# MadNLP/MadNLP.jl

Hardware: AMD Instinct MI355X
Metric: IP iterations/sec + ms per factorize!/solve!, condensed KKT n≈1e4 (higher is better)
Workload: dtype f64; 1 GPU; BASELINE config C3: case1354pegase-shaped sparse-condensed KKT, one instance; N=11192, m=16646, nnz(K)=68688; step = compress_J+compress_H+build_kkt+factorize (n_f=1) + inertia fetch + 2 solve_linear_system per instance; algorithm=BUNCHKAUFMAN (device: static-pivot LDL^T), outer_block=0, batch_per_gpu=1, batch_api=n/a (one instance), parallelism=1 GPU(s) x 1 independent instance(s)

## Files before the change

### madnlp.jl_amd/csrc/dag.hip

```cpp
#include <algorithm>
#include <atomic>
#include <cfloat>
#include <climits>
#include <vector>

#include "gemm_tile.h"
#include "ls.h"

namespace mnk {


struct DagInst {
    double* F;
    int64_t ld;
    double* V;
    const double* dinv;
    const double* dblk;
    const double* inv16;
    int* front;
    int* af;
    int* tprog;
    int* info;
    unsigned long long* vmax;
    double* zfill;
// ... 973 lines not shown
        mnk::PpDag dag{front, inst.af, ntile, 0, 0, -1, spin_limit, trace ? trace + (size_t)ls->dag_ntasks * 8 + (size_t)js_begin * 8 * 16 : nullptr,
                  mnk_ls_growth_word(ls), ls->dag_debug ? ls->dag_dbg.p : nullptr};
        int rc = mnk_launch_pchain(ls, sp, dag, js_begin, js_end, strips);
        if (rc) return rc;
        const int ph = (int)(counter - qctr), nq = ls->dag_nq[ph];
        MNK_REQUIRE(nq == 0 || (ntask >= mnk_ctx_bulk_wgs(ctx, chain_cus, 3) && bulk_xcds(ctx, chain_cus) == nq),
                    "task-DAG schedule: the bulk grid does not cover the XCDs the task list was dealt for");
        rc = mnk::launch_dag_bulk(su, ldl, inst, nullptr, ls->dag_tasks.p + 4 * (size_t)task0, ntask, ntile, counter, spin_limit,
                                  std::min(ntask, mnk_ctx_bulk_wgs(ctx, chain_cus, 3)), trace ? trace + 8 * (size_t)task0 : nullptr,
                                  trace ? trace + (size_t)ls->dag_ntasks * 8 + 4096 * 8 + (task0 > 0 ? 512 * 8 : 0) : nullptr,
                                  ls->dag_qoff.p + 16 * ph, ls->dag_qheads.p + ph * mnk::DAG_QHEAD_WORDS, nq);
        if (rc) return rc;
        if (js_begin == 0 && js_end > 0) {
            const int64_t safe = std::min<int64_t>(js_end, std::max<int64_t>(0, (ntile - ls->dag_band / 2 - 1) / 2)) & ~(int64_t)1;
            if (strips == (unsigned)ls->dag_band && safe > 0) {
                rc = mnk_ls_invert_blocks(ls, su, 0, safe);
                if (rc) return rc;
                ls->inv_done = safe;
            }
        }
        if (small) {
            rc = mnk_ls_invert_blocks(ls, s, 0, nsc);
            if (rc) return rc;
            ls->inv_done = nsc;
        } else if (js_begin == 0 && js_end == nsc && js2 == 0) {
            hipLaunchKernelGGL(mnk::dag_gate_kernel, dim3(1), dim3(1), 0, su, front + (nblk - 1), ntile, ls->info_dev.p, spin_limit);
            rc = mnk_ls_invert_blocks(ls, su, 0, nsc);
            if (rc) return rc;
            ls->inv_done = nsc;
        }
        if (!small) MNK_HIP(hipEventRecord(ctx->ev_a, sp));
        MNK_HIP(hipEventRecord(ctx->ev_b, su));
        if (!small) MNK_HIP(hipStreamWaitEvent(s, ctx->ev_a, 0));
        MNK_HIP(hipStreamWaitEvent(s, ctx->ev_b, 0));
        return 0;
    };
    if (js2 > 0) {
        int rc = phase(ctx->sp_dag, ctx->su_dag, ctx->dag_cus, 0, ls->dag_ntasks1, qctr, 0, std::min(js2, nsc),
                       (unsigned)std::min<int64_t>(ls->dag_band, Np / NBI));
        if (rc) return rc;
    }
    if (js2 < nsc) {
        const int64_t rows2 = Np - 256 * (int64_t)js2;
        MNK_REQUIRE(ctx->sp_dag2 != nullptr, "task-DAG schedule: the deep-band streams are missing");
        int rc = phase(ctx->sp_dag2, ctx->su_dag2, ctx->dag_cus2, ls->dag_ntasks1, ls->dag_ntasks - ls->dag_ntasks1,
                       qctr + 1, js2, nsc, (unsigned)(rows2 / NBI));
        if (rc) return rc;
    }
    return 0;
}

namespace {
struct BatchState {
    int depth = 0;
    bool active = false;
    std::vector<mnk_ls*> pend;
};
thread_local BatchState t_batch;

struct BatchBuffers {
    mnk::DevBuf<int> tasks;
    mnk::DevBuf<int> qctr;
    mnk::DevBuf<char> insts, pcsys, aux;
    char* stage = nullptr;
    size_t stage_bytes = 0;
    hipEvent_t stage_ev = nullptr;
    int ntile = 0, ninst = 0, period = 0, chunk = 0, taper0 = 0, band = 0, ntasks = 0;
    bool fill = false;
    hipEvent_t ev[4] = {nullptr, nullptr, nullptr, nullptr};
};
BatchBuffers g_batch[64];
}

bool mnk_batch_active() { return t_batch.active; }

bool mnk_batch_defer(mnk_ls* ls) {
    if (!t_batch.active) return false;
    const int nsc = (int)((ls->Np + 255) / 256);
    if (ls->algo_now != 5 || (ls->dag_js2 != nsc && ls->dag_js2 != 0) || ls->dag_trace_on || ls->ctx->partitioned) return false;
    if (mnk_ctx_ensure_batch_streams(ls->ctx) != 0) (void)hipGetLastError();
    if (!ls->ctx->sp_dagB) return false;
    if (!ls->ev_defer && hipEventCreateWithFlags(&ls->ev_defer, hipEventDisableTiming) != hipSuccess) { (void)hipGetLastError(); return false; }
    if (hipEventRecord(ls->ev_defer, ls->ctx->stream) != hipSuccess) { (void)hipGetLastError(); return false; }
    ls->deferred = true;
    t_batch.pend.push_back(ls);
    return true;
}

static void batch_mark_done(mnk_ls* ls) {
    ls->factorized = true;
    ls->info_valid = false;
    ls->bk_active = false;
    ls->deferred = false;
}

static int batch_run_group(std::vector<mnk_ls*>& g) {
    mnk_ls* l0 = g[0];
    mnk_ctx* c0 = l0->ctx;
    hipStream_t h = c0->stream;
    MNK_HIP(hipSetDevice(c0->device));
    const int64_t Np = l0->Np;
    const bool ldl = l0->algo == MNK_LDL;
    const int ntile = (int)(Np / 128), nsc = (int)((Np + 255) / 256), ninst = (int)g.size();
    const size_t nflags = (size_t)2 + (size_t)(Np / NBI) + 2 * (size_t)ntile * ntile;
    for (mnk_ls* ls : g)
        if (ls->ctx->stream != h) MNK_HIP(hipStreamWaitEvent(h, ls->ev_defer, 0));
    int rc = mnk_persist_begin(c0, h);
    if (rc) return rc;
    auto body = [&]() -> int {
        BatchBuffers& B = g_batch[c0->device & 63];
        const int period = std::max((ntile + 1) / 2, l0->batch_period > 0 ? l0->batch_period : 0);
        if (B.ntile != ntile || B.ninst != ninst || B.period != period || B.chunk != l0->dag_chunk || B.taper0 != l0->dag_taper0 ||
            B.band != l0->dag_band || B.fill != l0->dag_has_fill || !B.tasks.p) {
            std::vector<int> merged;
            mnk::dag_merge_tasks(l0->dag_host_tasks, l0->dag_host_ready, ninst, period, merged);
            if (B.tasks.alloc(merged.size() + 4)) return -2;
            { mnk::H2DGuard h2d; MNK_HIP(hipMemcpy(B.tasks.p, merged.data(), merged.size() * sizeof(int), hipMemcpyHostToDevice)); }
            if (!B.qctr.p && B.qctr.alloc(4)) return -2;
            if (B.insts.alloc(sizeof(mnk::DagInst) * (size_t)ninst)) return -2;
            for (hipEvent_t& e : B.ev)
                if (!e) MNK_HIP(hipEventCreateWithFlags(&e, hipEventDisableTiming));
            B.ntile = ntile; B.ninst = ninst; B.period = period; B.chunk = l0->dag_chunk; B.taper0 = l0->dag_taper0;
            B.band = l0->dag_band; B.fill = l0->dag_has_fill; B.ntasks = (int)(merged.size() / 4);
        }
        std::vector<mnk::DagInst> hin;
        mnk::DagInst* insts_dev = reinterpret_cast<mnk::DagInst*>(B.insts.p);
        for (mnk_ls* ls : g) {
            hin.push_back(dag_instance(ls));
            ls->dag_filled = hin.back().zfill != nullptr;
            ls->env_used = hin.back().env != nullptr;
            hipLaunchKernelGGL(mnk::dag_reset_kernel, dim3((unsigned)std::min<size_t>((nflags + 1023) / 1024, 64)), dim3(256), 0, h,
                               ls->dag_flags.p, (int64_t)nflags, ls->info_dev.p, hin.back(), insts_dev + (hin.size() - 1),
                               (const mnk::SmallSysRec*)nullptr, ls->env_word.p);
            ls->env_armed = false;
        }
        MNK_HIP(hipMemsetAsync(B.qctr.p, 0, 4 * sizeof(int), h));
        hipStream_t sp[2] = {c0->sp_dag, c0->sp_dagB}, su = c0->su_dagB;
        MNK_HIP(hipEventRecord(B.ev[0], h));
        MNK_HIP(hipStreamWaitEvent(sp[0], B.ev[0], 0));
        MNK_HIP(hipStreamWaitEvent(sp[1], B.ev[0], 0));
        MNK_HIP(hipStreamWaitEvent(su, B.ev[0], 0));
        const unsigned strips = (unsigned)std::min<int64_t>(l0->dag_band, Np / NBI);
        const int bulk_wgs = mnk_ctx_bulk_wgs(c0, 2 * c0->dag_cus, 3);
        auto launch_chain = [&](int i) -> int {
            mnk_ls* ls = g[i];
            mnk::PpDag dag{hin[i].front, hin[i].af, ntile, 0, 0, -1, mnk_ls_dag_spin_limit(ls), nullptr, mnk_ls_growth_word(ls)};
            return mnk_launch_pchain(ls, sp[i & 1], dag, 0, nsc, strips);
        };
        auto launch_tail = [&](int i) -> int {
            mnk_ls* ls = g[i];
            int r = mnk_ls_invert_blocks(ls, sp[i & 1], 0, nsc);
            if (r) return r;
            ls->inv_done = nsc;
            return mnk_ls_launch_finish_info(ls, sp[i & 1]);
        };
        for (int i = 0; i < std::min(2, ninst); ++i) {
            int r = launch_chain(i);
            if (r) return r;
        }
        int r = mnk::launch_dag_bulk(su, ldl, hin[0], insts_dev, B.tasks.p, B.ntasks, ntile, B.qctr.p,
                                     mnk_ls_dag_spin_limit(l0), std::min(B.ntasks, bulk_wgs), nullptr, nullptr);
        if (r) return r;
        for (int i = 0; i < ninst; ++i) {
            r = launch_tail(i);
            if (r) return r;
            if (i + 2 < ninst) {
                r = launch_chain(i + 2);
                if (r) return r;
            }
        }
        MNK_HIP(hipEventRecord(B.ev[1], sp[0]));
        MNK_HIP(hipEventRecord(B.ev[2], sp[1]));
        MNK_HIP(hipEventRecord(B.ev[3], su));
        for (int e = 1; e < 4; ++e) MNK_HIP(hipStreamWaitEvent(h, B.ev[e], 0));
        return 0;
    };
    rc = body();
    rc = mnk_persist_end(c0, h, rc);
    if (rc) return rc;
    MNK_HIP(hipEventRecord(l0->ev_defer, h));
    for (mnk_ls* ls : g) {
        if (ls->ctx->stream != h) MNK_HIP(hipStreamWaitEvent(ls->ctx->stream, l0->ev_defer, 0));
        batch_mark_done(ls);
        int r = mnk_ls_prefill_spare(ls);
        if (r) return r;
    }
    return 0;
}

static int batch_run_group_small(std::vector<mnk_ls*>& g) {
    mnk_ls* l0 = g[0];
    mnk_ctx* c0 = l0->ctx;
    hipStream_t h = c0->stream;
    MNK_HIP(hipSetDevice(c0->device));
    const int64_t Np = l0->Np;
    const bool ldl = l0->algo == MNK_LDL;
    const int ntile = (int)(Np / 128), nsc = (int)((Np + 255) / 256), strips = (int)(Np / NBI);
    const size_t nflags = (size_t)2 + (size_t)(Np / NBI) + 2 * (size_t)ntile * ntile;
    const int ntasks1 = l0->dag_ntasks;
    const int bulk_min = ntasks1 > 0 ? std::max(32, c0->num_cu / 4) : 0;
    auto chain_cus_for = [&](int k) { return std::min(c0->num_cu, (k * strips + 63) / 64 * 64); };
    int kmax = std::min(32, (c0->num_cu - bulk_min) / strips);
    while (kmax > 1 && chain_cus_for(kmax) > c0->num_cu - bulk_min) --kmax;
    if (kmax < 2) {
        for (mnk_ls* ls : g) {
            ls->deferred = false;
            int rc = mnk_ls_run_factorization_now(ls);
            if (rc) return rc;
        }
        return 0;
    }
    for (mnk_ls* ls : g)
        if (ls->ctx->stream != h) MNK_HIP(hipStreamWaitEvent(h, ls->ev_defer, 0));
    BatchBuffers& B = g_batch[c0->device & 63];
    for (size_t r0 = 0; r0 < g.size(); r0 += (size_t)kmax) {
        const int k = (int)std::min<size_t>(kmax, g.size() - r0);
        hipStream_t sp = nullptr, su = nullptr;
        int rc = mnk_masked_stream_pair(c0, chain_cus_for(k), &sp, &su);
        if (rc) return rc;
        if (ntasks1 > 0 && su == nullptr) { set_error("factorize batch: no CUs left for the bulk kernel"); return -1; }
        rc = mnk_persist_begin(c0, h);
        if (rc) return rc;
        auto body = [&]() -> int {
            if (ntasks1 > 0 && (B.ntile != ntile || B.ninst != k || B.period != 0 || B.chunk != l0->dag_chunk || B.taper0 != l0->dag_taper0 ||
                                B.band != l0->dag_band || B.fill != l0->dag_has_fill || !B.tasks.p)) {
                std::vector<int> merged;
                mnk::dag_merge_tasks(l0->dag_host_tasks, l0->dag_host_ready, k, 0, merged);
                if (B.tasks.alloc(merged.size() + 4)) return -2;
                { mnk::H2DGuard h2d; MNK_HIP(hipMemcpy(B.tasks.p, merged.data(), merged.size() * sizeof(int), hipMemcpyHostToDevice)); }
                B.ntile = ntile; B.ninst = k; B.period = 0; B.chunk = l0->dag_chunk; B.taper0 = l0->dag_taper0;
                B.band = l0->dag_band; B.fill = l0->dag_has_fill; B.ntasks = (int)(merged.size() / 4);
            }
            if (!B.qctr.p && B.qctr.alloc(4)) return -2;
            if (B.insts.n < sizeof(mnk::DagInst) * (size_t)k && B.insts.alloc(sizeof(mnk::DagInst) * (size_t)std::max(k, 32))) return -2;
            if (B.pcsys.n < mnk_pchain_sys_bytes() * (size_t)k && B.pcsys.alloc(mnk_pchain_sys_bytes() * (size_t)std::max(k, 32))) return -2;
            for (hipEvent_t& e : B.ev)
                if (!e) MNK_HIP(hipEventCreateWithFlags(&e, hipEventDisableTiming));
            std::vector<mnk::DagInst> hin;
            std::vector<int*> fronts;
            std::vector<const int*> afs;
            mnk::DagInst* insts_dev = reinterpret_cast<mnk::DagInst*>(B.insts.p);
            const size_t pc_bytes = mnk_pchain_sys_bytes();
            const size_t need = (size_t)k * (sizeof(mnk::DagInst) + pc_bytes + sizeof(mnk::SmallSysRec));
            if (B.aux.n < sizeof(mnk::SmallSysRec) * (size_t)k && B.aux.alloc(sizeof(mnk::SmallSysRec) * (size_t)std::max(k, 32))) return -2;
            if (B.stage_ev == nullptr) MNK_HIP(hipEventCreateWithFlags(&B.stage_ev, hipEventDisableTiming));
            else MNK_HIP(hipEventSynchronize(B.stage_ev));
            if (B.stage_bytes < need) {
                mnk::LaunchLock lock;
                if (B.stage) { mnk::quiesce_persistent(); (void)hipHostFree(B.stage); B.stage = nullptr; }
                const size_t cap = (size_t)std::max(k, 32) * (sizeof(mnk::DagInst) + pc_bytes + sizeof(mnk::SmallSysRec));
                MNK_HIP(hipHostMalloc((void**)&B.stage, cap, hipHostMallocDefault));
                B.stage_bytes = cap;
            }
            mnk::DagInst* st_inst = reinterpret_cast<mnk::DagInst*>(B.stage);
            char* st_pc = B.stage + (size_t)k * sizeof(mnk::DagInst);
            mnk::SmallSysRec* st_aux = reinterpret_cast<mnk::SmallSysRec*>(st_pc + (size_t)k * pc_bytes);
            const bool batch_aux = l0->linv_mfma && !l0->solve512;
            for (int i = 0; i < k; ++i) {
                mnk_ls* ls = g[r0 + i];
                hin.push_back(dag_instance(ls));
                ls->dag_filled = hin.back().zfill != nullptr;
                hin.back().env = nullptr;
                hin.back().envgate = nullptr;
                ls->env_used = false;
                fronts.push_back(hin.back().front);
                afs.push_back(hin.back().af);
                st_inst[i] = hin.back();
                mnk_pchain_fill_sys(ls, st_pc + (size_t)i * pc_bytes, hin.back().front, hin.back().af);
                mnk_ls_fill_small_rec(ls, st_aux + i);
            }
            MNK_HIP(hipMemcpyAsync(B.insts.p, st_inst, (size_t)k * sizeof(mnk::DagInst), hipMemcpyHostToDevice, h));
            MNK_HIP(hipMemcpyAsync(B.pcsys.p, st_pc, (size_t)k * pc_bytes, hipMemcpyHostToDevice, h));
            MNK_HIP(hipMemcpyAsync(B.aux.p, st_aux, (size_t)k * sizeof(mnk::SmallSysRec), hipMemcpyHostToDevice, h));
            MNK_HIP(hipEventRecord(B.stage_ev, h));
            const mnk::SmallSysRec* aux_dev = reinterpret_cast<const mnk::SmallSysRec*>(B.aux.p);
            hipLaunchKernelGGL(mnk::dag_reset_kernel, dim3((unsigned)std::min<size_t>((nflags + 1023) / 1024, 64), (unsigned)k), dim3(256), 0, h,
                               (int*)nullptr, (int64_t)0, (int*)nullptr, hin[0], (mnk::DagInst*)nullptr, aux_dev);
            MNK_HIP(hipMemsetAsync(B.qctr.p, 0, 4 * sizeof(int), h));
            MNK_HIP(hipEventRecord(B.ev[0], h));
            MNK_HIP(hipStreamWaitEvent(sp, B.ev[0], 0));
            if (su != nullptr) MNK_HIP(hipStreamWaitEvent(su, B.ev[0], 0));
            int r = mnk_launch_pchain_multi(g.data() + r0, k, sp, nullptr, B.pcsys.p, fronts.data(), afs.data());
            if (r) return r;
            if (ntasks1 > 0) {
                const int bulk_wgs = mnk_ctx_bulk_wgs(c0, chain_cus_for(k), 3);
                r = mnk::launch_dag_bulk(su, ldl, hin[0], insts_dev, B.tasks.p, B.ntasks, ntile, B.qctr.p, mnk_ls_dag_spin_limit(l0),
                                         std::min(B.ntasks, bulk_wgs), nullptr, nullptr);
                if (r) return r;
                MNK_HIP(hipEventRecord(B.ev[2], su));
                MNK_HIP(hipStreamWaitEvent(h, B.ev[2], 0));
            }
            MNK_HIP(hipEventRecord(B.ev[1], sp));
            MNK_HIP(hipStreamWaitEvent(h, B.ev[1], 0));
            if (su != nullptr) MNK_HIP(hipStreamWaitEvent(su, B.ev[1], 0));
            if (su != nullptr) MNK_HIP(hipStreamWaitEvent(sp, B.ev[2], 0));
            if (batch_aux) {
                r = mnk_ls_invert_blocks_batch(h, ldl, aux_dev, k, Np);
                if (r) return r;
                r = mnk_ls_finish_info_batch(h, aux_dev, k, ldl ? (l0->N >= 4096 ? 1024 : 256) : 64);
                if (r) return r;
                for (int i = 0; i < k; ++i) {
                    mnk_ls* ls = g[r0 + i];
                    ls->inv_done = nsc;
                    if (!ls->ev_info) MNK_HIP(hipEventCreateWithFlags(&ls->ev_info, hipEventDisableTiming));
                    MNK_HIP(hipEventRecord(ls->ev_info, h));
                    ls->ev_info_recorded = true;
                }
                return 0;
            }
            hipStream_t inv_s[3] = {h, sp, su != nullptr ? su : sp};
            for (int i = 0; i < k; ++i) {
                mnk_ls* ls = g[r0 + i];
                hipStream_t si = inv_s[i % 3];
                r = mnk_ls_invert_blocks(ls, si, 0, nsc);
                if (r) return r;
                ls->inv_done = nsc;
                r = mnk_ls_launch_finish_info(ls, si);
                if (r) return r;
            }
            MNK_HIP(hipEventRecord(B.ev[1], sp));
            MNK_HIP(hipStreamWaitEvent(h, B.ev[1], 0));
            if (su != nullptr) {
                MNK_HIP(hipEventRecord(B.ev[2], su));
                MNK_HIP(hipStreamWaitEvent(h, B.ev[2], 0));
            }
            return 0;
        };
        rc = body();
        rc = mnk_persist_end(c0, h, rc);
        if (rc) return rc;
    }
    MNK_HIP(hipEventRecord(l0->ev_defer, h));
    for (mnk_ls* ls : g) {
        if (ls->ctx->stream != h) MNK_HIP(hipStreamWaitEvent(ls->ctx->stream, l0->ev_defer, 0));
        batch_mark_done(ls);
        int r = mnk_ls_prefill_spare(ls);
        if (r) return r;
    }
    return 0;
}

static int batch_flush() {
    std::vector<mnk_ls*> pend;
    pend.swap(t_batch.pend);
    int rc_all = 0;
    while (!pend.empty()) {
        mnk_ls* l0 = pend.front();
        std::vector<mnk_ls*> g, rest;
        for (mnk_ls* ls : pend) {
            const bool same = ls->ctx->device == l0->ctx->device && ls->Np == l0->Np && ls->algo == l0->algo && ls->dag_js2 == l0->dag_js2 && ls->dag_chunk == l0->dag_chunk &&
                              ls->dag_taper0 == l0->dag_taper0 && ls->dag_band == l0->dag_band && ls->dag_has_fill == l0->dag_has_fill;
            (same && std::find(g.begin(), g.end(), ls) == g.end() ? g : rest).push_back(ls);
        }
        pend.swap(rest);
        int rc;
        if (g.size() >= 2) {
            rc = l0->dag_js2 == 0 ? batch_run_group_small(g) : batch_run_group(g);
            if (rc)
                for (mnk_ls* ls : g) { ls->deferred = false; ls->factorized = false; ls->info_valid = false; }
        } else {
            g[0]->deferred = false;
            if (g[0]->Np < g[0]->dag_min_rows) g[0]->algo_now = 4;
            rc = mnk_ls_run_factorization_now(g[0]);
            if (rc) { g[0]->factorized = false; g[0]->info_valid = false; }
        }
        if (rc && !rc_all) rc_all = rc;
    }
    return rc_all;
}

int mnk_ls_sync_deferred(mnk_ls* ls) {
    {
        int rc_s = mnk_solve_sync_deferred(ls);
        if (rc_s) return rc_s;
    }
    return mnk_ls_sync_deferred_fact(ls);
}

bool mnk_ls_pending_elsewhere(const mnk_ls* ls) {
    return ls->deferred && std::find(t_batch.pend.begin(), t_batch.pend.end(), ls) == t_batch.pend.end();
}

int mnk_ls_sync_deferred_fact(mnk_ls* ls) {
    if (!ls->deferred) return 0;
    if (std::find(t_batch.pend.begin(), t_batch.pend.end(), ls) == t_batch.pend.end()) {
        set_error("a factorize! call of this solver is pending in a batch that another thread opened (mnk_factorize_batch_end must come first)");
        return -1;
    }
    return batch_flush();
}

extern "C" int mnk_factorize_batch_begin(void) {
    ++t_batch.depth;
    t_batch.active = true;
    return 0;
}

extern "C" int mnk_factorize_batch_end(void) {
    if (t_batch.depth <= 0) { set_error("mnk_factorize_batch_end: no batch is open on this thread"); return -1; }
    if (--t_batch.depth > 0) return 0;
    t_batch.active = false;
    return batch_flush();
}

extern "C" int mnk_debug_dag_tasks(int ntile, int chunk, int band_tiles, int js2, int taper0, int* out, int cap, int* first_phase) {
    if (ntile <= 0 || chunk <= 0 || band_tiles <= 0 || taper0 <= 0) return -1;
    std::vector<int> h;
    const int n1 = mnk::dag_build_tasks(ntile, chunk, band_tiles, js2, h, taper0, nullptr);
    const int n = (int)(h.size() / 4);
    if (first_phase != nullptr) *first_phase = n1;
    if (out != nullptr)
        for (int i = 0; i < std::min(n, cap) * 4; ++i) out[i] = h[i];
    return n;
}

extern "C" int mnk_debug_dag_merged_tasks(int ntile, int chunk, int band_tiles, int js2, int taper0, int fill, int ninst, int period,
                                          int* out, int cap) {
    if (ntile <= 0 || chunk <= 0 || band_tiles <= 0 || taper0 <= 0 || ninst <= 0 || period < 0) return -1;
    std::vector<int> h, ready, merged;
    int n1 = mnk::dag_build_tasks(ntile, chunk, band_tiles, js2, h, taper0, &ready);
    if (fill) n1 = mnk::dag_add_fill_tasks(ntile, h, ready, n1);
    mnk::dag_merge_tasks(h, ready, ninst, period, merged);
    const int n = (int)(merged.size() / 4);
    if (out != nullptr)
        for (int i = 0; i < std::min(n, cap) * 4; ++i) out[i] = merged[i];
    return n;
}

extern "C" int mnk_debug_dag_deal(int ntile, int chunk, int band_tiles, int js2, int taper0, int fill, int ninst, int period, int nq,
                                  int gang, int* tasks_out, int* order, int cap, int* off, int* first_phase) {
    if (ntile <= 0 || chunk <= 0 || band_tiles <= 0 || taper0 <= 0 || ninst <= 0 || period < 0 || nq <= 0 || nq > 64 || gang == 0) return -1;
    std::vector<int> h, ready;
    int n1 = mnk::dag_build_tasks(ntile, chunk, band_tiles, js2, h, taper0, &ready);
    if (fill) n1 = mnk::dag_add_fill_tasks(ntile, h, ready, n1);
    if (ninst > 1) {
        std::vector<int> merged, mready, pos(ninst, 0);
        mnk::dag_merge_tasks(h, ready, ninst, period, merged);
        for (size_t t = 0; t < merged.size() / 4; ++t) { const int i = merged[4 * t + 1] >> 16; mready.push_back(i * period + ready[pos[i]++]); }
        h.swap(merged);
        ready.swap(mready);
        n1 = (int)ready.size();
    }
    const int n = (int)ready.size();
    if (first_phase != nullptr) *first_phase = n1;
    const int part[3] = {0, n1, n};
    int written = 0;
    for (int ph = 0; ph < 2; ++ph) {
        std::vector<int> ord, o;
        mnk::dag_deal_tasks(h, ready, part[ph], part[ph + 1], nq, gang, ord, o);
        for (int x = 0; x <= nq; ++x)
            if (off != nullptr) off[ph * (nq + 1) + x] = part[ph] + o[x];
        for (int v : ord) {
            if (order != nullptr && written < cap) order[written] = v;
            ++written;
        }
    }
    if (tasks_out != nullptr)
        for (int i = 0; i < std::min(n, cap) * 4; ++i) tasks_out[i] = h[i];
    return n;
}
```

### madnlp.jl_amd/csrc/factor.hip

```cpp
#include <atomic>
#include <type_traits>
#include <atomic>
#include <cfloat>
#include <chrono>
#include <cmath>
#include <cstdlib>

#include "ls.h"
#include "leaf64.h"

namespace mnk {

template <bool LDL, int NS>
__device__ __forceinline__ void trsm64_mfma_body(double* __restrict__ F, int64_t ld, int64_t j0, int64_t Np,
                                                 const double* __restrict__ Dblk, const double* __restrict__ inv16,
                                                 const double* __restrict__ dinv, double* __restrict__ W, int64_t ldw,
                                                 int64_t wcol, const int* __restrict__ info,
                                                 unsigned long long* __restrict__ vmax) {
    if (*info != 0) return;
    const int lane = threadIdx.x & 63, wave = threadIdx.x >> 6;
    const int l15 = lane & 15, l4 = lane >> 4;
    const int64_t r0 = j0 + 64 + ((int64_t)blockIdx.x * 4 + wave) * (16 * NS);
    if (r0 >= Np) return;
    double Ln[6][4];
// ... 894 lines not shown
        hipLaunchKernelGGL(linv64_kernel<true>, dim3((unsigned)(b1 - b0)), dim3(256), 0, s, ls->fact.p, ls->ld, ls->dblk.p,
                           ls->linv.p, ls->info_dev.p, (int)b0);
    else
        hipLaunchKernelGGL(linv64_kernel<false>, dim3((unsigned)(b1 - b0)), dim3(256), 0, s, ls->fact.p, ls->ld, ls->dblk.p,
                           ls->linv.p, ls->info_dev.p, (int)b0);
    MNK_HIP(hipGetLastError());
    return mnk_ls_build_inverses(ls, s, sc0, sc1);
}

int mnk_launch_pchain(mnk_ls* ls, hipStream_t sp, const mnk::PpDag& dag, int js_begin, int js_end, unsigned strips) {
    {
        static std::atomic<uint64_t> attr_devs{0};
        int dev = 0;
        MNK_HIP(hipGetDevice(&dev));
        if (!(attr_devs.load(std::memory_order_relaxed) >> (dev & 63) & 1)) {
            MNK_HIP(hipFuncSetAttribute((const void*)pchain_kernel<true>, hipFuncAttributeMaxDynamicSharedMemorySize, PC_LDS_BYTES));
            MNK_HIP(hipFuncSetAttribute((const void*)pchain_kernel<false>, hipFuncAttributeMaxDynamicSharedMemorySize, PC_LDS_BYTES));
            attr_devs.fetch_or(1ull << (dev & 63), std::memory_order_relaxed);
        }
    }
    const bool ldl = ls->algo == MNK_LDL;
    const int epoch16 = ls->epoch * 16;
    double* V = ldl ? ls->vfull.p : nullptr;
    if (ldl)
        hipLaunchKernelGGL(pchain_kernel<true>, dim3(strips), dim3(256), PC_LDS_BYTES, sp, ls->fact.p, ls->ld, ls->Np, ls->dblk.p,
                           ls->inv16.p, ls->dvec.p, ls->dinv.p, V, ls->info_dev.p, ls->pivot_tol, ls->flag_p.p, epoch16,
                           ls->debug_pp_missing, dag, js_begin, js_end);
    else
        hipLaunchKernelGGL(pchain_kernel<false>, dim3(strips), dim3(256), PC_LDS_BYTES, sp, ls->fact.p, ls->ld, ls->Np, ls->dblk.p,
                           ls->inv16.p, ls->dvec.p, ls->dinv.p, V, ls->info_dev.p, ls->pivot_tol, ls->flag_p.p, epoch16,
                           ls->debug_pp_missing, dag, js_begin, js_end);
    MNK_HIP(hipGetLastError());
    return 0;
}

static int run_factorization_body(mnk_ls* ls);

size_t mnk_pchain_sys_bytes() { return sizeof(mnk::PcSys); }
void mnk_pchain_fill_sys(mnk_ls* ls, void* rec_host, int* front, const int* af) {
    const bool ldl = ls->algo == MNK_LDL;
    *static_cast<mnk::PcSys*>(rec_host) = mnk::PcSys{ls->fact.p, ls->ld, ls->Np, ls->dblk.p, ls->inv16.p, ls->dvec.p, ls->dinv.p,
                                                       ldl ? ls->vfull.p : nullptr, ls->info_dev.p, ls->pivot_tol, ls->flag_p.p,
                                                       ls->epoch * 16, front, af, (int)(ls->Np / 128), mnk_ls_dag_spin_limit(ls),
                                                       mnk_ls_growth_word(ls)};
}

int mnk_launch_pchain_multi(mnk_ls* const* v, int n, hipStream_t sp, hipStream_t fill_stream, void* table, int* const* front,
                            const int* const* af) {
    {
        static std::atomic<uint64_t> attr_devs{0};
        int dev = 0;
        MNK_HIP(hipGetDevice(&dev));
        if (!(attr_devs.load(std::memory_order_relaxed) >> (dev & 63) & 1)) {
            MNK_HIP(hipFuncSetAttribute((const void*)pchain_multi_kernel<true>, hipFuncAttributeMaxDynamicSharedMemorySize, PC_LDS_BYTES));
            MNK_HIP(hipFuncSetAttribute((const void*)pchain_multi_kernel<false>, hipFuncAttributeMaxDynamicSharedMemorySize, PC_LDS_BYTES));
            attr_devs.fetch_or(1ull << (dev & 63), std::memory_order_relaxed);
        }
    }
    mnk::PcSys* dst = static_cast<mnk::PcSys*>(table);
    const bool ldl = v[0]->algo == MNK_LDL;
    const int strips = (int)(v[0]->Np / NBI);
    for (int i = 0; i < n && fill_stream != nullptr; ++i) {
        mnk_ls* ls = v[i];
        mnk::PcSys rec{ls->fact.p, ls->ld, ls->Np, ls->dblk.p, ls->inv16.p, ls->dvec.p, ls->dinv.p, ldl ? ls->vfull.p : nullptr,
                       ls->info_dev.p, ls->pivot_tol, ls->flag_p.p, ls->epoch * 16, front[i], af[i], (int)(ls->Np / 128),
                       mnk_ls_dag_spin_limit(ls), mnk_ls_growth_word(ls)};
        hipLaunchKernelGGL(pc_set_sys_kernel, dim3(1), dim3(1), 0, fill_stream, rec, dst + i);
    }
    MNK_HIP(hipGetLastError());
    if (ldl)
        hipLaunchKernelGGL(pchain_multi_kernel<true>, dim3((unsigned)(n * strips)), dim3(256), PC_LDS_BYTES, sp, dst, strips);
    else
        hipLaunchKernelGGL(pchain_multi_kernel<false>, dim3((unsigned)(n * strips)), dim3(256), PC_LDS_BYTES, sp, dst, strips);
    MNK_HIP(hipGetLastError());
    return 0;
}

int mnk_ls_run_factorization(mnk_ls* ls) {
    if (ls->algo == MNK_QR) return mnk_qr_factor(ls);
    if (ls->algo == MNK_LU) return mnk_lu_factor(ls);
    if (ls->algo == MNK_EVD) return mnk_evd_factor(ls);
    mnk_ctx* ctx = ls->ctx;
    hipStream_t s = ctx->stream;
    const int64_t Np = ls->Np;
    if (ls->panel_algo >= 4 && !ls->flag_p.p) {
        if (ls->flag_p.alloc(Np / NBI + 1)) return -2;
        MNK_HIP(hipMemsetAsync(ls->flag_p.p, 0, (Np / NBI + 1) * sizeof(int), s));
    }
    ++ls->epoch;
    ls->inv_done = 0;
    ls->factor_invalid = false;
    ls->t_fact_launch_ms = mnk_host_ms();
    {
        const int want = (ls->early_reject && ls->accept_only_pd && ls->algo == MNK_LDL && ls->src_persistent) ? 1 : 0;
        if (want != ls->reject_on_device) {
            MNK_HIP(hipMemsetAsync(ls->info_dev.p + 2, want, sizeof(int), s));
            ls->reject_on_device = want;
        }
    }
    ls->algo_now = ls->panel_algo;
    ls->env_used = false;
    const int64_t min_rows = mnk_batch_active() ? std::min<int64_t>(ls->dag_min_rows, 256) : ls->dag_min_rows;
    if (ls->algo_now == 5 && (ctx->dag_cus < ls->dag_band || !ls->lookahead || Np < min_rows || Np > ls->dag_max_rows)) ls->algo_now = 4;
    if (ls->algo_now == 5 && ctx->sp_dag == nullptr && mnk_ctx_ensure_dag(ctx) != 0) { (void)hipGetLastError(); ls->algo_now = 4; }
    if (ls->algo_now == 5 && ctx->sp_dag == nullptr) ls->algo_now = 4;
    ++ls->fact_count;
    if (ls->pp_blocked && ls->fact_count >= ls->pp_retry_at) ls->pp_blocked = false;
    if (ls->algo_now >= 4 && ls->pp_blocked) ls->algo_now = 1;
    if (ls->algo_now == 5 && mnk_ls_dag_prepare(ls) != 0) ls->algo_now = 4;
    if (ls->algo_now == 5 && ls->dag_js2 < (Np + 255) / 256) {
        if (mnk_ctx_ensure_dag2(ctx) != 0) (void)hipGetLastError();
        if (ctx->sp_dag2 == nullptr) ls->algo_now = 4;
    }
    if (ls->algo_now == 5 && mnk_batch_defer(ls)) return 0;
    return mnk_ls_run_factorization_now(ls);
}

int mnk_ls_run_factorization_now(mnk_ls* ls) {
    mnk_ctx* ctx = ls->ctx;
    hipStream_t s = ctx->stream;
    const bool persistent = ls->algo_now >= 4;
    if (persistent) {
        int rc0 = mnk_persist_begin(ctx, s);
        if (rc0) return rc0;
    }
    const int rc_run = run_factorization_body(ls);
    return persistent ? mnk_persist_end(ctx, s, rc_run) : rc_run;
}

static int run_factorization_body(mnk_ls* ls) {
    mnk_ctx* ctx = ls->ctx;
    hipStream_t s = ctx->stream;
    const int64_t Np = ls->Np, ld = ls->ld;
    const bool ldl = ls->algo == MNK_LDL;
    double* F = ls->fact.p;
    const int64_t NBO = mnk_ls_effective_nbo(ls);
    if (ls->algo_now != 5) MNK_HIP(hipMemsetAsync(ls->info_dev.p, 0, 2 * sizeof(int), s));
    std::vector<int64_t> bnd{0};
    for (int64_t pos = 0; pos < Np;) {
        const bool tail = ls->lookahead && NBO < Np && ls->tail_rows > 0 && Np - pos <= ls->tail_rows && ls->tail_nbo < NBO;
        pos = std::min<int64_t>(pos + (tail ? ls->tail_nbo : NBO), Np);
        bnd.push_back(pos);
    }
    const int64_t npanel = (int64_t)bnd.size() - 1;
    const bool la = ls->lookahead && npanel > 1;

    if (ls->algo_now == 5) {
        int rc = mnk_ls_run_factorization_dag(ls);
        if (rc) return rc;
    } else if (!la) {
        for (int64_t ko = 0; ko < Np; ko += NBO) {
            const int64_t kend = std::min<int64_t>(ko + NBO, Np);
            int rc = factor_outer_panel(ls, s, ko, kend, ls->wbuf[0].p);
            if (rc) return rc;
            const int64_t Mt = Np - kend;
            if (Mt > 0) {
                const double* Wsrc = ldl ? ls->wbuf[0].p + kend : F + kend + ko * ld;
                rc = launch_gemm_nt(s, 2, Mt, Mt, kend - ko, Wsrc, ldl ? ls->ldw : ld, F + kend + ko * ld, ld,
                                    F + kend + kend * ld, ld, nullptr, nullptr, 0, ls->info_dev.p);
                if (rc) return rc;
            }
        }
    } else {
        { int rc_s = mnk_ctx_ensure_panel_streams(ctx); if (rc_s) return rc_s; }
        hipStream_t sp = ctx->sp, su = ctx->su;
        if ((int64_t)ctx->ev_panel.size() < npanel + 1) {
            const size_t old = ctx->ev_panel.size();
            ctx->ev_panel.resize(npanel + 1);
            ctx->ev_next.resize(npanel + 1);
            ctx->ev_next2.resize(npanel + 1);
            ctx->ev_bdone.resize(npanel + 1);
            for (size_t e = old; e < ctx->ev_panel.size(); ++e) {
                MNK_HIP(hipEventCreateWithFlags(&ctx->ev_panel[e], hipEventDisableTiming));
                MNK_HIP(hipEventCreateWithFlags(&ctx->ev_next[e], hipEventDisableTiming));
                MNK_HIP(hipEventCreateWithFlags(&ctx->ev_next2[e], hipEventDisableTiming));
                MNK_HIP(hipEventCreateWithFlags(&ctx->ev_bdone[e], hipEventDisableTiming));
            }
        }
        const int pcus = ctx->panel_cus;
        const int ucus = pcus > 0 ? ctx->num_cu - pcus : ctx->num_cu;
        const bool share = ls->share != 0;
        if (share) {
            if (ls->tile_ctr.n < 8 * ((size_t)npanel + 1)) {
                int rc0 = ls->tile_ctr.alloc(8 * ((size_t)npanel + 1));
                if (rc0) return rc0;
            }
            MNK_HIP(hipMemsetAsync(ls->tile_ctr.p, 0, 8 * ((size_t)npanel + 1) * sizeof(int), s));
        }
        int rc = 0;
        if (ls->panel0_whole) rc = factor_outer_panel(ls, s, 0, bnd[1], ls->wbuf[0].p);
        if (rc) return rc;
        MNK_HIP(hipEventRecord(ctx->ev_a, s));
        MNK_HIP(hipStreamWaitEvent(sp, ctx->ev_a, 0));
        MNK_HIP(hipStreamWaitEvent(su, ctx->ev_a, 0));
        if (!ls->panel0_whole) rc = factor_outer_panel(ls, sp, 0, bnd[1], ls->wbuf[0].p);
        if (rc) return rc;
        MNK_HIP(hipEventRecord(ctx->ev_panel[0], sp));
        for (int64_t k = 0; k + 1 < npanel; ++k) {
            const int64_t ko = bnd[k], kend = bnd[k + 1];
            const int64_t Mt = Np - kend;
            if (Mt <= 0) break;
            const int64_t nnext = bnd[k + 2] - kend;
            double* wk = ls->wbuf[k & 1].p;
            const double* Wsrc = ldl ? wk + kend : F + kend + ko * ld;
            const int64_t ldws = ldl ? ls->ldw : ld;
            const int64_t Kw = kend - ko;
            MNK_HIP(hipStreamWaitEvent(su, ctx->ev_panel[k], 0));
            auto update_a = [&](hipStream_t st, int64_t c0, int64_t c1) -> int {
                const int64_t Mp = Mt - c0, Nn = c1 - c0;
                double* Cp = F + (kend + c0) + (kend + c0) * ld;
                if (gemm_nt_lower_tiles(Mp, Nn) < ls->small_tiles)
                    return launch_gemm_nt_lower_small(st, Mp, Nn, Kw, Wsrc + c0, ldws, F + kend + c0 + ko * ld, ld, Cp,
                                                      ld, ls->info_dev.p);
                return launch_gemm_nt(st, 2, Mp, Nn, Kw, Wsrc + c0, ldws, F + kend + c0 + ko * ld, ld, Cp, ld, nullptr,
                                      nullptr, 0, ls->info_dev.p);
            };
            const bool fuse_a = ls->algo_now == 4 && ls->pp_fuse_rows > 0 && Mt <= ls->pp_fuse_rows && Kw <= 512;
            const bool own_first = !fuse_a && ls->split_a == 2 && nnext > NBI;
            const int64_t n1 = own_first ? std::min<int64_t>(ls->own_cols, nnext - NBI) : std::min<int64_t>(256, nnext);
            const bool split_a = (ls->split_a || fuse_a) && nnext > n1;
            if (fuse_a) {
                if (k > 0) MNK_HIP(hipStreamWaitEvent(sp, ctx->ev_bdone[k - 1], 0));
                if (split_a) {
                    rc = update_a(su, n1, nnext);
                    if (rc) return rc;
                    MNK_HIP(hipEventRecord(ctx->ev_next2[k], su));
                }
            } else if (own_first) {
                if (k > 0) MNK_HIP(hipStreamWaitEvent(sp, ctx->ev_bdone[k - 1], 0));
                rc = update_a(sp, 0, n1);
                if (rc) return rc;
                rc = update_a(su, n1, nnext);
                if (rc) return rc;
                MNK_HIP(hipEventRecord(ctx->ev_next2[k], su));
            } else {
                rc = update_a(su, 0, split_a ? n1 : nnext);
                if (rc) return rc;
                MNK_HIP(hipEventRecord(ctx->ev_next[k], su));
                if (split_a) {
                    rc = update_a(su, n1, nnext);
                    if (rc) return rc;
                    MNK_HIP(hipEventRecord(ctx->ev_next2[k], su));
                }
            }
            const int64_t Mb = Mt - nnext;
            const int64_t Nb = Mb;
            bool shared_b = false;
            if (Mb > 0 && Nb > 0) {
                const int ntiles = gemm_nt_lower_tiles(Mb, Nb);
                const double t_upd = ntiles * (68.0 * (double)Kw / 512.0) / ucus;
                const double t_pan = 55.0 * (double)nnext / 64.0 * (pcus > 0 ? 64.0 / pcus : 1.0);
                shared_b = share && pcus > 0 && (t_upd > t_pan || ls->share == 2);
                if (shared_b)
                    rc = launch_gemm_nt_queue(su, Mb, Nb, Kw, Wsrc + nnext, ldws, F + kend + nnext + ko * ld, ld,
                                              F + (kend + nnext) + (kend + nnext) * ld, ld, ls->tile_ctr.p + 8 * k,
                                              ucus, ls->info_dev.p);
                else
                    rc = launch_gemm_nt(su, 2, Mb, Nb, Kw, Wsrc + nnext, ldws, F + kend + nnext + ko * ld, ld,
                                        F + (kend + nnext) + (kend + nnext) * ld, ld, nullptr, nullptr, 0,
                                        ls->info_dev.p);
                if (rc) return rc;
            }
            MNK_HIP(hipEventRecord(ctx->ev_bdone[k], su));
            if (!own_first && !fuse_a) MNK_HIP(hipStreamWaitEvent(sp, ctx->ev_next[k], 0));
            rc = factor_outer_panel(ls, sp, kend, kend + nnext, ls->wbuf[(k + 1) & 1].p,
                                    split_a ? ctx->ev_next2[k] : nullptr, own_first ? n1 : 256,
                                    fuse_a ? (ldl ? wk : F + ko * ld) : nullptr, ldws, fuse_a ? Kw : 0);
            if (rc) return rc;
            if (shared_b) {
                rc = launch_gemm_nt_queue(sp, Mb, Nb, Kw, Wsrc + nnext, ldws, F + kend + nnext + ko * ld, ld,
                                          F + (kend + nnext) + (kend + nnext) * ld, ld, ls->tile_ctr.p + 8 * k,
                                          pcus, ls->info_dev.p);
                if (rc) return rc;
            }
            MNK_HIP(hipEventRecord(ctx->ev_panel[k + 1], sp));
        }
        MNK_HIP(hipEventRecord(ctx->ev_a, sp));
        MNK_HIP(hipEventRecord(ctx->ev_b, su));
        MNK_HIP(hipStreamWaitEvent(s, ctx->ev_a, 0));
        MNK_HIP(hipStreamWaitEvent(s, ctx->ev_b, 0));
    }
    {
        int rc = mnk_ls_invert_blocks(ls, s, ls->inv_done, (Np + 255) / 256);
        if (rc) return rc;
    }
    ls->factorized = true;
    ls->info_valid = false;
    ls->bk_active = false;
    {
        int rc = mnk_ls_launch_finish_info(ls, s);
        if (rc) return rc;
    }
    return mnk_ls_prefill_spare(ls);
}

void mnk_ls_fill_small_rec(mnk_ls* ls, mnk::SmallSysRec* rec) {
    const bool lmode = ls->algo == MNK_LDL;
    const int64_t ntile = ls->Np / 128;
    rec->flags = ls->dag_flags.p;
    rec->nflags = 2 + ls->Np / NBI + 2 * ntile * ntile;
    rec->info = ls->info_dev.p;
    rec->F = ls->fact.p; rec->ld = ls->ld; rec->dblk = ls->dblk.p; rec->linv = ls->linv.p;
    rec->linv256 = ls->linv256.p; rec->linv256t = ls->linv256t.p; rec->Np = ls->Np;
    rec->dvec = ls->dvec.p; rec->ninertia = lmode ? ls->N : 0; rec->pin_dev = ls->pin_dev;
    rec->amax = mnk_ls_growth_word(ls) != nullptr ? ls->amax_dev.p : nullptr;
}

int mnk_ls_invert_blocks_batch(hipStream_t s, bool ldl, const mnk::SmallSysRec* recs_dev, int n, int64_t Np) {
    const unsigned nb = (unsigned)(Np / NBI);
    if (ldl) hipLaunchKernelGGL(linv64_kernel<true>, dim3(nb, 1, (unsigned)n), dim3(256), 0, s, (double*)nullptr, (int64_t)0, (const double*)nullptr,
                                (double*)nullptr, (const int*)nullptr, 0, recs_dev);
    else hipLaunchKernelGGL(linv64_kernel<false>, dim3(nb, 1, (unsigned)n), dim3(256), 0, s, (double*)nullptr, (int64_t)0, (const double*)nullptr,
                            (double*)nullptr, (const int*)nullptr, 0, recs_dev);
    MNK_HIP(hipGetLastError());
    return mnk_ls_build_inverses_batch(s, recs_dev, n, Np);
}

int mnk_ls_finish_info_batch(hipStream_t s, const mnk::SmallSysRec* recs_dev, int n, int threads) {
    hipLaunchKernelGGL(finish_info_kernel, dim3((unsigned)n), dim3(threads), 0, s, (const double*)nullptr, (int64_t)0, (const int*)nullptr,
                       (unsigned long long*)nullptr, (const unsigned long long*)nullptr, recs_dev);
    MNK_HIP(hipGetLastError());
    return 0;
}

int mnk_ls_launch_finish_info(mnk_ls* ls, hipStream_t s) {
    const bool lmode = ls->algo == MNK_LDL;
    const int threads = lmode ? (ls->N >= 4096 ? 1024 : 256) : 64;
    hipLaunchKernelGGL(finish_info_kernel, dim3(1), dim3(threads), 0, s, ls->dvec.p, lmode ? ls->N : (int64_t)0, ls->info_dev.p, ls->pin_dev,
                       mnk_ls_growth_word(ls) != nullptr ? ls->amax_dev.p : (const unsigned long long*)nullptr);
    MNK_HIP(hipGetLastError());
    if (!ls->ev_info) MNK_HIP(hipEventCreateWithFlags(&ls->ev_info, hipEventDisableTiming));
    MNK_HIP(hipEventRecord(ls->ev_info, s));
    ls->ev_info_recorded = true;
    return 0;
}

int mnk_ls_right_trsm_rows(mnk_ls* ls, hipStream_t s, int64_t j0, double* Xrows, double* Vrows, int64_t ldr, int64_t nrows) {
    MNK_REQUIRE(ls->factorized && !ls->bk_active && nrows % 16 == 0 && j0 % NBI == 0 && j0 < ls->Np,
                "mnk_ls_right_trsm_rows: needs a static-pivot factor, 16-row multiples and a block-aligned column");
    double* Fp = Xrows - (j0 + NBI);
    double* Wp = Vrows ? Vrows - (j0 + NBI) : nullptr;
    const unsigned grid = (unsigned)((nrows / 16 + 3) / 4);
    const double* dblk = ls->dblk.p + (j0 / NBI) * 4096;
    const double* inv16 = ls->inv16.p + (j0 / NBI) * 1024;
    if (ls->algo == MNK_LDL)
        hipLaunchKernelGGL((trsm64_mfma_kernel<true, 1>), dim3(grid), dim3(256), 0, s, Fp, ldr, j0, j0 + NBI + nrows, dblk,
                           inv16, ls->dinv.p, Wp, ldr, (int64_t)j0, ls->info_dev.p);
    else
        hipLaunchKernelGGL((trsm64_mfma_kernel<false, 1>), dim3(grid), dim3(256), 0, s, Fp, ldr, j0, j0 + NBI + nrows, dblk,
                           inv16, ls->dinv.p, (double*)nullptr, (int64_t)0, (int64_t)0, ls->info_dev.p);
    MNK_HIP(hipGetLastError());
    return 0;
}

int mnk_launch_trsm64_batch(hipStream_t s, bool ldl, const mnk::TrsmBatchRec* recs_dev, int nbatch, int64_t j0, int64_t nrows,
                            int64_t ldr) {
    if (nbatch <= 0 || nrows <= 0) return 0;
    MNK_REQUIRE(nrows % 16 == 0 && j0 % NBI == 0, "mnk_launch_trsm64_batch: 16-row multiples and a block-aligned column");
    const dim3 grid((unsigned)((nrows / 16 + 3) / 4), (unsigned)nbatch);
    if (ldl) hipLaunchKernelGGL(trsm64_mfma_batch_kernel<true>, grid, dim3(256), 0, s, recs_dev, ldr, j0, nrows);
    else hipLaunchKernelGGL(trsm64_mfma_batch_kernel<false>, grid, dim3(256), 0, s, recs_dev, ldr, j0, nrows);
    MNK_HIP(hipGetLastError());
    return 0;
}

static int bk_fallback(mnk_ls* ls) {
    hipStream_t s = ls->ctx->stream;
    int rc = ls->retransfer();
    if (rc) return rc;
    rc = mnk_ls_run_bunchkaufman(ls);
    if (rc) return rc;
    rc = mnk_ls_invert_blocks(ls, s, 0, (ls->Np + 255) / 256);
    if (rc) return rc;
    ++ls->bk_count;
    return mnk_ls_prefill_spare(ls);
}

int mnk_ls_fetch_info(mnk_ls* ls) {
    { int rc_d = mnk_ls_sync_deferred(ls); if (rc_d) return rc_d; }
    if (ls->info_valid) return 0;
    if (ls->algo == MNK_QR) {
        MNK_HIP(mnk::stream_wait(ls->ctx->stream));
        ls->info = 0;
        ls->info_valid = true;
        return 0;
    }
    if (ls->algo == MNK_LU) return mnk_lu_fetch_info(ls);
    if (ls->algo == MNK_EVD) return mnk_evd_fetch_info(ls);
    hipStream_t s = ls->ctx->stream;
    if (ls->bk_active) {
        MNK_HIP(hipMemsetAsync(ls->inertia_dev.p, 0, 3 * sizeof(unsigned long long), s));
        int rc = mnk_ls_bk_inertia(ls, ls->inertia_dev.p);
        if (rc) return rc;
        hipLaunchKernelGGL(publish_info_kernel, dim3(1), dim3(64), 0, s, ls->inertia_dev.p, ls->info_dev.p, ls->pin_dev);
        MNK_HIP(hipGetLastError());
        MNK_HIP(mnk::stream_wait(s));
        volatile unsigned long long* pw = ls->pin;
        unsigned long long h[3] = {pw[0], pw[1], pw[2]};
        int hinfo = (int)(long long)pw[3];
        ls->info = hinfo;
        ls->nneg = h[1] > 0 ? -1 : (int64_t)h[0];
        ls->nzero = hinfo > 0 ? 1 : 0;
        ls->npos = ls->N - ls->nneg - ls->nzero;
        ls->info_valid = true;
        return 0;
    }
    const bool guard = ls->algo == MNK_LDL && ls->bk_requested && ls->bk_fallback && ls->retransfer && ls->amax_dev.p != nullptr;
    if (ls->ev_info_recorded) MNK_HIP(hipEventSynchronize(ls->ev_info));
    else MNK_HIP(mnk::stream_wait(s));
    volatile unsigned long long* pw = ls->pin;
    unsigned long long h[3] = {pw[0], pw[1], pw[2]};
    int hinfo = (int)(long long)pw[3];
    if (guard) {
        double am, dm;
        const unsigned long long wa = pw[4], wd = pw[5];
        memcpy(&am, &wa, sizeof am);
        memcpy(&dm, &wd, sizeof dm);
        ls->last_growth = am > 0.0 ? dm / am : (dm > 0.0 ? HUGE_VAL : 0.0);
        ls->last_sign_changes = (int64_t)pw[6];
    }
    if (hinfo == -7) ls->last_timeout_site = (int)(long long)pw[7];
    if (hinfo == -7 && ls->dag_debug && ls->dag_flags.p && ls->dag_dbg.p) {
        MNK_HIP(mnk::stream_wait(s));
        const int64_t ntile = ls->Np / 128;
        ls->dbg_flags.resize((size_t)(2 + ls->Np / NBI + 2 * ntile * ntile));
        ls->dbg_chain.resize(ls->dag_dbg.n);
        MNK_HIP(mnk::d2h_copy(ls->dbg_flags.data(), ls->dag_flags.p, ls->dbg_flags.size() * sizeof(int), s));
        MNK_HIP(mnk::d2h_copy(ls->dbg_chain.data(), ls->dag_dbg.p, ls->dbg_chain.size() * sizeof(int), s));
    }
    if (hinfo != 0 && ls->spare_by_dag) {
        ls->spare_zeroed = false;
        ls->spare_by_dag = false;
    }
    if (hinfo == -7 && ls->algo_now >= 4 && ls->retransfer) {
        ls->pp_blocked = true;
        ls->pp_retry_at = ls->fact_count + ls->pp_backoff + 1;
        ls->pp_backoff *= 4;
        ++ls->pp_fallbacks;
        {
            const double lost = std::max(0.0, mnk_host_ms() - ls->t_fact_launch_ms);
            ls->stall_ms_total += lost;
            mnk_add_process_stall_ms(lost);
        }
        int rc = ls->retransfer();
        if (rc) return rc;
        rc = mnk_ls_run_factorization(ls);
        if (rc) return rc;
        return mnk_ls_fetch_info(ls);
    }
    ls->factor_invalid = false;
    if (hinfo == -9) {
        ls->info = 1;
        ls->npos = (int64_t)h[0];
        ls->nzero = (int64_t)h[1];
        ls->nneg = ls->N - ls->npos - ls->nzero;
        ls->factor_invalid = true;
        ++ls->early_rejects;
        ls->early_reject_col = (int64_t)(long long)pw[7];
        ls->info_valid = true;
        ls->probe_last_rejected = true;
        if (2 * ls->early_reject_col < ls->N) { ls->probe_hint_col = ls->early_reject_col; ls->probe_since_hint = 0; }
        else if (ls->probe_since_hint < (1 << 20)) ++ls->probe_since_hint;
        return 0;
    }
    if (hinfo < 0) {
        set_error("factorize!: a device-side hand-off timed out (info = %d) and the matrix cannot be transferred again; the "
                  "factor is invalid -- set panel_algo = 1", hinfo);
        return -4;
    }
    ls->info = hinfo;
    if (ls->algo == MNK_LDL) {
        ls->npos = (int64_t)h[0];
        ls->nzero = (int64_t)h[1];
        ls->nneg = (int64_t)h[2];
        if (ls->nzero > 0 && ls->info == 0) ls->info = 1;
        const double gtol = ls->last_sign_changes <= 1 ? ls->bk_growth_tol_qd : ls->bk_growth_tol;
        const bool verdict_final = ls->accept_only_pd && (ls->nzero > 0 || ls->nneg > 0);
        if (!verdict_final && (ls->nzero > 0 || (guard && !(ls->last_growth <= gtol))) && ls->bk_requested && ls->bk_fallback && ls->retransfer) {
            int rc = bk_fallback(ls);
            if (rc) return rc;
            return mnk_ls_fetch_info(ls);
        }
    } else {
        if (hinfo == 0) { ls->npos = ls->N; ls->nzero = 0; ls->nneg = 0; }
        else { ls->npos = 0; ls->nzero = ls->N; ls->nneg = 0; }
    }
    ls->probe_last_rejected = false;
    if (ls->probe_since_hint < (1 << 20)) ++ls->probe_since_hint;
    ls->info_valid = true;
    return 0;
}
```

### madnlp.jl_amd/csrc/ls.h

```cpp
#pragma once
#include <algorithm>
#include <functional>
#include <memory>
#include <string>
#include <vector>

#include "common.h"

struct mnk_sc {
    mnk_ctx* ctx = nullptr;
    int64_t n = 0, m = 0, nnzj = 0, nnzh = 0;
    int64_t nnz_jt = 0, nnz_hess = 0, nnz_aug = 0, len_jptr = 0;
    std::vector<int32_t> jt_colptr, jt_rowval, h_colptr, h_rowval, aug_colptr, aug_rowval;
    std::vector<int32_t> tile_env;
    mnk::DevBuf<int32_t> d_tile_env;
    std::vector<int64_t> jt_map, h_map;
    std::vector<int32_t> d_dst, d_src, hp_dst, hp_src, j_dst, j_c, j_k, j_l;
    mnk::DevBuf<int32_t> jt_seg_ptr, jt_seg_src, h_seg_ptr, h_seg_src;
    mnk::DevBuf<int32_t> aug_hptr, aug_hsrc;
    mnk::DevBuf<int32_t> aug_dsrc;
    mnk::DevBuf<int32_t> aug_jptr, aug_jc, aug_jk, aug_jl;
    mnk::DevBuf<int32_t> aug_row, aug_col;
    mnk::DevBuf<int32_t> d_jt_colptr, d_jt_rowval, d_jt_colidx, d_h_colptr, d_h_rowval, d_h_colidx;
    mnk::DevBuf<double> jac_coo, hess_coo, jt_nz, h_nz, aug_nz, diag_buffer, pr_diag, du_diag;
    void* extra = nullptr;
    std::shared_ptr<int> alive = std::make_shared<int>(0);
};

inline std::vector<int32_t> mnk_tile_envelope(int64_t n, const int32_t* row, const int32_t* col, int64_t nnz) {
    std::vector<int32_t> fnz(n);
    for (int64_t i = 0; i < n; ++i) fnz[i] = (int32_t)i;
    for (int64_t k = 0; k < nnz; ++k)
        if (row[k] >= 0 && row[k] < n && col[k] < fnz[row[k]]) fnz[row[k]] = col[k];
    const int64_t ntile = (n + 127) / 128;
    std::vector<int32_t> env(ntile);
    for (int64_t I = 0; I < ntile; ++I) {
        int32_t f = (int32_t)(128 * I);
        for (int64_t i = 128 * I; i < std::min<int64_t>(n, 128 * I + 128); ++i) f = std::min(f, fnz[i]);
        env[I] = f / 128;
    }
    return env;
}

struct mnk_dc {
    mnk_ctx* ctx = nullptr;
    int condensed = 1;
    bool mirror_pending = false;
    int64_t n = 0, m = 0, ns = 0, n_eq = 0, order = 0;
    std::vector<int64_t> ind_ineq, ind_eq;
    mnk::DevBuf<int64_t> d_ind_ineq, d_ind_eq;
    mnk::DevBuf<double> hess, jac, aug, pr_diag, du_diag, diag_buffer;
    mnk::DevBuf<double> jis;
    int64_t ld_jis = 0, kpad = 0, npad = 0;
    void* extra = nullptr;
    void* qn = nullptr;
    std::shared_ptr<int> alive = std::make_shared<int>(0);
};
void mnk_dc_qn_release(mnk_dc* dc);

constexpr int EVD_BLOCK = 32;

struct mnk_ls {
    mnk_ctx* ctx = nullptr;
    int64_t N = 0, Np = 0, ld = 0, ldw = 0, nbo = 512;
    bool nbo_auto = true;
    int algo = MNK_LDL;
    double pivot_tol = 0.0;
    int lookahead = 1;
    int share = 1;
    int small_tiles = 400;
    int split_a = 2;
    int64_t single_rows = 2560;
    int64_t tail_rows = 4096;
    int64_t tail_nbo = 256;
    int small_tiles_mid = 1000;
    mnk::DevBuf<int> tile_ctr;
    mnk::DevBuf<double> fact, wbuf[2], linv, dblk, inv16, linv256, linv256t, dvec, dinv, xwork;
    mnk::DevBuf<double> fact_spare;
    hipEvent_t ev_spare = nullptr, ev_free = nullptr;
    bool spare_zeroed = false, spare_pending = false;
    int prefill = 1;
    int64_t prefill_max_rows = 24576;
    int epoch = 0;
    mnk::DevBuf<int> flag_p;
    int panel0_whole = 1;
    int algo_now = 1;
    bool pp_blocked = false;
    int64_t fact_count = 0, pp_retry_at = 0, pp_backoff = 16;
    int pp_fallbacks = 0;
    int last_timeout_site = 0;
    double stall_ms_total = 0.0;
    double t_fact_launch_ms = 0.0;
    int64_t pp_fuse_rows = 4096;
    int64_t own_cols = 128;
    mnk::DevBuf<int> dag_tasks;
    int dag_ntasks = 0, dag_ntasks1 = 0, dag_js2 = 0;
    std::vector<int> dag_host_tasks, dag_host_ready;
    int dag_fill = 1;
    bool dag_has_fill = false;
    bool dag_filled = false;
    int batch_period = 0;
    hipEvent_t ev_info = nullptr;
    bool ev_info_recorded = false;
    hipEvent_t ev_defer = nullptr;
    bool deferred = false;
    int dag_xcd_queues = 1;
    int dag_gang = 4;
    int dag_nq[2] = {0, 0};
    mnk::DevBuf<int> dag_qoff;
    mnk::DevBuf<int> dag_qheads;
    mnk::DevBuf<int> dag_flags;
    mnk::DevBuf<double> vfull;
    mnk::DevBuf<unsigned long long> dag_trace;
    bool dag_trace_on = false;
    int64_t inv_done = 0;
    int dag_band = 16;
    int dag_taper0 = 2;
    long dag_spin_limit = 0;
    int dag_chunk = 64;
    int64_t dag_min_rows = 1280;
    int64_t dag_deep_rows = 5376;
    int envelope = 1;
    const int32_t* env_dev = nullptr;
    std::vector<int32_t> env_host;
    mnk::DevBuf<int32_t> env_own;
    mnk::DevBuf<int> env_word;
    bool env_used = false;
    bool env_armed = false;
    int64_t dag_max_rows = 30720;
    int panel_algo = 5;
    int persistent_solve = 1;
    int solve512 = 0;
    int64_t solve512_min_rows = 4096;
    int dag_chain_inline = 1;
    std::vector<std::string> env_keys;
    int dag_js2_override = -1;
    int linv_mfma = 1;
    mnk::DevBuf<double> linv512, linv512t, linv512tmp;
    int pub_next = 0;
    bool pub_clean[2] = {false, false};
    int* solve_abort = nullptr;
    long ps_spin_limit = 6000000;
    int debug_pp_missing = -1;
    int debug_ps_missing = -1;
    mnk::DevBuf<unsigned long long> solve_trace;
    mnk::DevBuf<int> info_dev;
    mnk::DevBuf<unsigned long long> inertia_dev;
    unsigned long long* pin = nullptr;
    unsigned long long* pin_dev = nullptr;
    bool bk_requested = false;
    int bk_fallback = 1;
    int early_reject = 0;
    int reject_on_device = -1;
    bool src_persistent = false;
    bool factor_invalid = false;
    int64_t early_rejects = 0, early_reject_col = -1, early_reject_redone = 0;
    int probe = 1;
    mnk_ls* probe_ls = nullptr;
    int64_t probe_order = 0;
    int64_t probe_hint_col = -1;
    int probe_since_hint = 1 << 20;
    bool probe_last_rejected = false;
    int64_t probe_hits = 0, probe_misses = 0;
    int accept_only_pd = 0;
    double bk_growth_tol = 64.0, bk_growth_tol_qd = 1e8;
    double last_growth = 0.0;
    int64_t last_sign_changes = 0;
    mnk::DevBuf<unsigned long long> amax_dev;
    bool bk_active = false;
    int bk_count = 0;
    std::function<int()> retransfer;
    mnk::DevBuf<int> bk_perm, bk_ptype;
    mnk::DevBuf<double> bk_doff, bk_dcoup, bk_work;
    mnk::DevBuf<char> bk_state;
    mnk::DevBuf<double> bk_wv, bk_tmp;
    mnk::DevBuf<unsigned long long> bk_msg;
    mnk::DevBuf<int> bk_aux;
    int bk_panel_wgs = 0;
    int bk_max_wgs = 0;
    long bk_spin_limit = 1L << 21;
    int debug_bk_missing = -1;
    bool bk_multi_last = false, bk_mw_blocked = false;
    int bk_mw_fallbacks = 0;
    bool factorized = false, info_valid = false;
    int dag_debug = 0;
    mnk::DevBuf<int> dag_dbg;
    std::vector<int> dbg_flags, dbg_chain;
    bool spare_by_dag = false;
    int info = 0;
    int64_t npos = 0, nzero = 0, nneg = 0;
    mnk::DevBuf<double> qr_v, qr_t, qr_w, qr_p;
    mnk::DevBuf<double> lu_ut, lu_p;
    mnk::DevBuf<int> lu_cand, lu_ipiv, lu_perm, lu_info;
    mnk::DevBuf<double> evd_a, evd_v, evd_rt, evd_colsum, evd_lam, evd_part;
    mnk::DevBuf<int> evd_ident, evd_rank;
    int evd_sweep_cap = 60;
    int evd_sweeps = 0;
};

int64_t mnk_ls_effective_nbo(const mnk_ls* ls);
int mnk_qr_alloc(mnk_ls* ls);
int mnk_qr_factor(mnk_ls* ls);
int mnk_qr_solve(mnk_ls* ls, double* x, int64_t nrhs, int64_t ldx, int loc);
int mnk_launch_tril_to_full(hipStream_t s, double* F, int64_t ld, int64_t N, int64_t Np);
int mnk_launch_upper_bsolve(hipStream_t s, const double* F, int64_t ld, int64_t Np, double* y, double* x);
int mnk_lu_alloc(mnk_ls* ls);
int mnk_lu_factor(mnk_ls* ls);
int mnk_lu_fetch_info(mnk_ls* ls);
int mnk_lu_solve(mnk_ls* ls, double* x, int64_t nrhs, int64_t ldx, int loc);
int mnk_evd_alloc(mnk_ls* ls);
int mnk_evd_factor(mnk_ls* ls);
int mnk_evd_fetch_info(mnk_ls* ls);
int mnk_evd_solve(mnk_ls* ls, double* x, int64_t nrhs, int64_t ldx, int loc);
int mnk_ls_run_factorization(mnk_ls* ls);
int mnk_ls_run_factorization_now(mnk_ls* ls);
int mnk_ls_launch_finish_info(mnk_ls* ls, hipStream_t s);
bool mnk_solve_defer(mnk_ls* ls, double* xuser);
int mnk_solve_sync_deferred(mnk_ls* ls);
int mnk_solve_batch_flush_pending(void);
int mnk_ls_factorize_dense_dev_async(mnk_ls* ls, const double* Adev, int64_t lda);
double mnk_host_ms();
void mnk_add_process_stall_ms(double ms);
double mnk_process_stall_ms();
bool mnk_ls_pending_elsewhere(const mnk_ls* ls);
bool mnk_batch_active();
size_t mnk_pchain_sys_bytes();
int mnk_launch_pchain_multi(mnk_ls* const* v, int n, hipStream_t sp, hipStream_t fill_stream, void* table, int* const* front,
                            const int* const* af);
bool mnk_batch_defer(mnk_ls* ls);
int mnk_ls_sync_deferred(mnk_ls* ls);
int mnk_ls_sync_deferred_fact(mnk_ls* ls);
int mnk_ls_prefill_spare(mnk_ls* ls);
int mnk_ls_fetch_info(mnk_ls* ls);
int mnk_ls_run_factorization_dag(mnk_ls* ls);
int mnk_ls_dag_prepare(mnk_ls* ls);
int mnk_launch_pchain(mnk_ls* ls, hipStream_t sp, const mnk::PpDag& dag, int js_begin, int js_end, unsigned strips);
unsigned long long* mnk_ls_growth_word(mnk_ls* ls);
int mnk_ls_run_solve(mnk_ls* ls, double* xdev , double* xuser = nullptr );
int mnk_ls_build_inverses(mnk_ls* ls, hipStream_t s, int64_t sc0, int64_t sc1);
int mnk_ls_invert_blocks(mnk_ls* ls, hipStream_t s, int64_t sc0, int64_t sc1);
int mnk_ls_right_trsm_rows(mnk_ls* ls, hipStream_t s, int64_t j0, double* Xrows, double* Vrows, int64_t ldr, int64_t nrows);
int mnk_ls_run_bunchkaufman(mnk_ls* ls);
long mnk_ls_dag_spin_limit(const mnk_ls* ls);
namespace mnk {
struct SmallSysRec {
    int* flags; int64_t nflags; int* info;
    double* F; int64_t ld; const double* dblk; double* linv; double* linv256; double* linv256t; int64_t Np;
    const double* dvec; int64_t ninertia; unsigned long long* pin_dev; const unsigned long long* amax;
};
}
int mnk_ls_invert_blocks_batch(hipStream_t s, bool ldl, const mnk::SmallSysRec* recs_dev, int n, int64_t Np);
int mnk_ls_build_inverses_batch(hipStream_t s, const mnk::SmallSysRec* recs_dev, int n, int64_t Np);
int mnk_ls_finish_info_batch(hipStream_t s, const mnk::SmallSysRec* recs_dev, int n, int threads);
void mnk_ls_fill_small_rec(mnk_ls* ls, mnk::SmallSysRec* rec);
void mnk_pchain_fill_sys(mnk_ls* ls, void* rec_host, int* front, const int* af);
int mnk_launch_trsm64_batch(hipStream_t s, bool ldl, const mnk::TrsmBatchRec* recs_dev, int nbatch, int64_t j0, int64_t nrows,
                            int64_t ldr);
int mnk_ls_bk_permute(mnk_ls* ls, double* x, double* tmp, bool forward);
int mnk_ls_bk_dsolve(mnk_ls* ls, double* y);
int mnk_ls_bk_inertia(mnk_ls* ls, unsigned long long* out_dev);
bool mnk_ls_take_solve_abort(mnk_ls* ls);
```

### madnlp.jl_amd/csrc/ls.hip

```cpp
#include <cstdarg>
#include <cstdlib>
#include <atomic>
#include <map>
#include <mutex>

#include <cfloat>
#include "ls.h"

namespace mnk {

static thread_local std::string g_err;
void set_error(const char* fmt, ...) {
    char buf[1024];
    va_list ap;
    va_start(ap, fmt);
    vsnprintf(buf, sizeof(buf), fmt, ap);
    va_end(ap);
    g_err = buf;
}

__global__ __launch_bounds__(256) void fill_lower_kernel(double* __restrict__ F, int64_t ld, int64_t N, int64_t Np) {
    const int64_t col = blockIdx.x;
    const int64_t first = (col / PAD) * PAD;
    const int64_t r = first + ((int64_t)blockIdx.y * 256 + threadIdx.x) * 2;
// ... 431 lines not shown
        }
        if (!part) g_ctx_list[device & 63].push_back(c);
        c->sp_dag = d.sp; c->su_dag = d.su; c->dag_cus = d.cus;
        c->dag_cus2 = d.cus > 0 ? (getenv("MNK_DAG_CUS2") ? atoi(getenv("MNK_DAG_CUS2")) : 96) : 0;
        if (c->dag_cus2 <= 0 || c->dag_cus2 >= c->num_cu) c->dag_cus2 = 0;
        c->shared_dag_streams = !part;
        if (part) {
            if (c->dag_cus2 > 0 && !make_pair(c->dag_cus2, c->sp_dag2, c->su_dag2)) c->dag_cus2 = 0;
        }
    }
    MNK_HIP(hipEventCreateWithFlags(&c->ev_a, hipEventDisableTiming));
    MNK_HIP(hipEventCreateWithFlags(&c->ev_b, hipEventDisableTiming));
    if (mnk_solve_warmup(c->stream) != 0) (void)hipGetLastError();
    g_live_ctx[device & 63].fetch_add(1, std::memory_order_relaxed);
    *out = c;
    return 0;
}

int mnk_ctx_create(int device, void* stream, mnk_ctx** out) { return ctx_create_common(device, stream, 0, 0, out); }

}
int mnk_masked_stream_pair(mnk_ctx* ctx, int chain_cus, hipStream_t* sp, hipStream_t* su) {
    mnk::LaunchLock lock;
    MNK_REQUIRE(!ctx->partitioned && chain_cus > 0 && chain_cus <= ctx->total_cu, "mnk_masked_stream_pair: bad size");
    MaskedPair& p = g_pair_cache[{ctx->device, chain_cus}];
    if (p.sp == nullptr) {
        std::vector<int> bits;
        for (int b = 0; b < ctx->total_cu; ++b) bits.push_back(b);
        if (!make_masked_stream(ctx->total_cu, bits.data(), chain_cus, p.sp)) { set_error("mnk_masked_stream_pair: CU-masked streams are not available"); return -2; }
        if (chain_cus < ctx->total_cu && !make_masked_stream(ctx->total_cu, bits.data() + chain_cus, ctx->total_cu - chain_cus, p.su)) {
            (void)hipStreamDestroy(p.sp);
            p.sp = nullptr;
            set_error("mnk_masked_stream_pair: CU-masked streams are not available");
            return -2;
        }
        if (p.su != nullptr) {
            hipStream_t w[1] = {p.su};
            if (mnk_dag_warmup(w, 1, 3 * ctx->num_cu) != 0) (void)hipGetLastError();
        }
    }
    *sp = p.sp;
    *su = p.su;
    return 0;
}
extern "C" {

int mnk_ctx_destroy(mnk_ctx* c) {
    if (!c) return 0;
    {
        std::lock_guard<std::mutex> lock(g_ctx_mutex);
        if (c->children > 0) {
            c->released = true;
            return 0;
        }
    }
    ctx_free(c);
    return 0;
}


int mnk_ctx_synchronize(mnk_ctx* c) {
    MNK_REQUIRE(c != nullptr, "ctx is NULL");
    MNK_HIP(mnk::stream_wait(c->stream));
    return 0;
}

void* mnk_ctx_stream(mnk_ctx* c) { return c ? (void*)c->stream : nullptr; }

int mnk_ls_create(mnk_ctx* ctx, int64_t N, int algo, mnk_ls** out) {
    MNK_REQUIRE(ctx && out, "mnk_ls_create: NULL argument");
    mnk::LaunchLock lock;
    MNK_REQUIRE(N > 0, "mnk_ls_create: N must be positive");
    const bool bk_requested = algo == MNK_BUNCHKAUFMAN;
    if (bk_requested) algo = MNK_LDL;
    MNK_REQUIRE(algo == MNK_CHOLESKY || algo == MNK_LDL || algo == MNK_QR || algo == MNK_LU || algo == MNK_EVD,
                "mnk_ls_create: unknown algorithm (BUNCHKAUFMAN, LU, QR, CHOLESKY, LDL and EVD are implemented on device)");
    MNK_HIP(hipSetDevice(ctx->device));
    mnk_ls* ls = new mnk_ls();
    ls->ctx = ctx;
    ls->N = N;
    ls->algo = algo;
    ls->bk_requested = bk_requested;
    {
        auto from_env = [&](const std::string& key, double v) {
            if (mnk_ls_set_option(ls, key.c_str(), v) == 0) ls->env_keys.push_back(key);
            else fprintf(stderr, "madnlp_hip: ignoring environment override '%s': %s\n", key.c_str(), mnk_last_error_string());
        };
        if (const char* e = getenv("MNK_PANEL_ALGO")) from_env("panel_algo", atof(e));
        if (const char* e = getenv("MNK_PERSISTENT_SOLVE")) from_env("persistent_solve", atof(e));
        if (const char* e = getenv("MNK_OPTIONS")) {
            std::string all(e);
            size_t pos = 0;
            while (pos < all.size()) {
                size_t end = all.find(',', pos);
                if (end == std::string::npos) end = all.size();
                const std::string item = all.substr(pos, end - pos);
                const size_t eq = item.find('=');
                if (eq != std::string::npos && eq > 0) from_env(item.substr(0, eq), atof(item.c_str() + eq + 1));
                pos = end + 1;
            }
        }
    }
    ls->Np = round_up(N, PAD);
    ls->ld = ls->Np;
    ls->ldw = ls->Np;
    int rc = 0;
    rc |= ls->fact.alloc((size_t)ls->ld * ls->Np + SLACK);
    rc |= ls->linv.alloc((size_t)(ls->Np / NBI) * NBI * NBI);
    rc |= ls->dblk.alloc((size_t)(ls->Np / NBI) * NBI * NBI);
    rc |= ls->inv16.alloc((size_t)(ls->Np / NBI) * 1024);
    rc |= ls->linv256.alloc((size_t)((ls->Np + 255) / 256) * 65536);
    rc |= ls->linv256t.alloc((size_t)((ls->Np + 255) / 256) * 65536);
    rc |= ls->dvec.alloc(ls->Np);
    rc |= ls->dinv.alloc(ls->Np);
    rc |= ls->xwork.alloc(10 * ls->Np);
    if (hipHostMalloc((void**)&ls->solve_abort, sizeof(int), hipHostMallocDefault) != hipSuccess) {
        (void)hipGetLastError();
        ls->solve_abort = nullptr;
        rc |= -2;
    } else {
        *ls->solve_abort = 0;
    }
    if (hipHostMalloc((void**)&ls->pin, 8 * sizeof(unsigned long long), hipHostMallocMapped) != hipSuccess ||
        hipHostGetDevicePointer((void**)&ls->pin_dev, ls->pin, 0) != hipSuccess) {
        (void)hipGetLastError();
        rc |= -2;
    }
    rc |= ls->info_dev.alloc(4);
    rc |= ls->inertia_dev.alloc(3);
    if (algo == MNK_QR) {
        rc |= mnk_qr_alloc(ls);
        ls->prefill = 0;
    }
    if (algo == MNK_LU) {
        rc |= mnk_lu_alloc(ls);
        ls->prefill = 0;
    }
    if (algo == MNK_EVD) {
        rc |= mnk_evd_alloc(ls);
        ls->prefill = 0;
    }
    if (rc) { delete ls; return -2; }
    MNK_HIP(hipMemsetAsync(ls->fact.p, 0, ((size_t)ls->ld * ls->Np + SLACK) * sizeof(double), ctx->stream));
    mnk_ctx_child_added(ctx);
    *out = ls;
    return 0;
}

int mnk_ls_destroy(mnk_ls* ls) {
    if (!ls) return 0;
    (void)hipSetDevice(ls->ctx->device);
    if (mnk_ls_pending_elsewhere(ls)) {
        set_error("mnk_ls_destroy: a factorize! call of this solver is pending in a batch that another thread opened "
                  "(that thread's mnk_factorize_batch_end must come first); the solver was NOT destroyed");
        return -1;
    }
    (void)mnk_ls_sync_deferred(ls);
    (void)mnk::stream_wait(ls->ctx->stream);
    if (ls->probe_ls) { (void)mnk_ls_destroy(ls->probe_ls); ls->probe_ls = nullptr; }
    mnk::LaunchLock lock;
    mnk::quiesce_persistent();
    if (ls->solve_abort) (void)hipHostFree(ls->solve_abort);
    if (ls->pin) (void)hipHostFree(ls->pin);
    if (ls->ctx->s_fill) (void)mnk::stream_wait(ls->ctx->s_fill);
    if (ls->ev_spare) (void)hipEventDestroy(ls->ev_spare);
    if (ls->ev_free) (void)hipEventDestroy(ls->ev_free);
    if (ls->ev_defer) (void)hipEventDestroy(ls->ev_defer);
    if (ls->ev_info) (void)hipEventDestroy(ls->ev_info);
    mnk_ctx* ctx = ls->ctx;
    delete ls;
    mnk_ctx_child_gone(ctx);
    return 0;
}

int mnk_ls_set_option(mnk_ls* ls, const char* key, double value) {
    MNK_REQUIRE(ls && key, "mnk_ls_set_option: NULL argument");
    { int rc_d = mnk_ls_sync_deferred(ls); if (rc_d) return rc_d; }
    for (const std::string& k : ls->env_keys)
        if (k == key) {
            static std::mutex warn_mutex;
            static std::vector<std::string> warned;
            std::lock_guard<std::mutex> lock(warn_mutex);
            if (std::find(warned.begin(), warned.end(), k) == warned.end()) {
                warned.push_back(k);
                fprintf(stderr, "madnlp_hip: set_option('%s', %g) ignored: the option is pinned by MNK_OPTIONS / MNK_PANEL_ALGO / "
                                "MNK_PERSISTENT_SOLVE for this process (query: get_stat(\"pinned:%s\"))\n", key, value, key);
            }
            return 0;
        }
    if (!strcmp(key, "pivot_tol")) { ls->pivot_tol = value; return 0; }
    if (!strcmp(key, "envelope")) { ls->envelope = value != 0.0; return 0; }
    if (!strcmp(key, "split_a")) { ls->split_a = (int)value; return 0; }
    if (!strcmp(key, "tail_rows")) { ls->tail_rows = (int64_t)value; return 0; }
    if (!strcmp(key, "tail_nbo")) { ls->tail_nbo = (int64_t)value; return 0; }
    if (!strcmp(key, "own_cols")) { ls->own_cols = std::max<long>(64, (long)value / 64 * 64); return 0; }
    if (!strcmp(key, "panel0_whole")) { ls->panel0_whole = (int)value; return 0; }
    if (!strcmp(key, "dag_js2")) { ls->dag_js2_override = (int)value; return 0; }
    if (!strcmp(key, "outer_block")) {
        int64_t v = (int64_t)value;
        MNK_REQUIRE(v == 0 || (v >= NBI && v % NBI == 0), "outer_block must be 0 (by size) or a positive multiple of 64");
        ls->nbo_auto = v == 0;
        if (v > 0) ls->nbo = v;
        ls->wbuf[0].release();
        ls->wbuf[1].release();
        return 0;
    }
    if (!strcmp(key, "solve512")) { ls->solve512 = value != 0; return 0; }
    if (!strcmp(key, "solve512_min_rows")) { ls->solve512_min_rows = (int64_t)value; return 0; }
    if (!strcmp(key, "linv_mfma")) { ls->linv_mfma = value != 0.0; return 0; }
    if (!strcmp(key, "dag_chain_inline")) { ls->dag_chain_inline = value != 0.0; return 0; }
    if (!strcmp(key, "prefill")) { ls->prefill = value != 0; return 0; }
    if (!strcmp(key, "prefill_max_rows")) { ls->prefill_max_rows = (int64_t)value; return 0; }
    if (!strcmp(key, "single_rows")) {
        ls->single_rows = (int64_t)value;
        ls->wbuf[0].release();
        ls->wbuf[1].release();
        return 0;
    }
    if (!strcmp(key, "lookahead")) { ls->lookahead = value != 0.0; return 0; }
    if (!strcmp(key, "share")) { ls->share = (int)value; return 0; }
    if (!strcmp(key, "small_tiles")) { ls->small_tiles = (int)value; return 0; }
    if (!strcmp(key, "small_tiles_mid")) { ls->small_tiles_mid = (int)value; return 0; }
    if (!strcmp(key, "panel_algo")) {
        MNK_REQUIRE((int)value == 1 || (int)value == 4 || (int)value == 5, "panel_algo must be 1, 4 or 5");
        ls->panel_algo = (int)value;
        return 0;
    }
    if (!strcmp(key, "pp_fuse_rows")) { ls->pp_fuse_rows = (int64_t)value; return 0; }
    if (!strcmp(key, "dag_min_rows")) { ls->dag_min_rows = (int64_t)value; return 0; }
    if (!strcmp(key, "dag_taper0")) {
        MNK_REQUIRE(value >= 1.0 && value <= 16.0, "dag_taper0 must be in 1..16");
        ls->dag_taper0 = (int)value;
        ls->dag_tasks.release();
        return 0;
    }
    if (!strcmp(key, "dag_chunk")) {
        MNK_REQUIRE(value >= 1.0 && value <= 64.0, "dag_chunk must be in 1..64");
        ls->dag_chunk = (int)value;
        ls->dag_tasks.release();
        return 0;
    }
    if (!strcmp(key, "dag_band")) {
        MNK_REQUIRE(value >= 8.0 && value <= 64.0 && (int)value % 4 == 0 && (double)(int)value == value, "dag_band must be a multiple of 4 in 8..64");
        ls->dag_band = (int)value;
        ls->dag_tasks.release();
        return 0;
    }
    if (!strcmp(key, "dag_spin_limit")) {
        MNK_REQUIRE(value >= 1024.0, "dag_spin_limit must be at least 1024");
        ls->dag_spin_limit = (long)value;
        return 0;
    }
    if (!strcmp(key, "dag_fill")) { ls->dag_fill = value != 0.0; ls->dag_tasks.release(); return 0; }
    if (!strcmp(key, "dag_xcd_queues")) { ls->dag_xcd_queues = value != 0.0; ls->dag_tasks.release(); return 0; }
    if (!strcmp(key, "dag_gang")) {
        MNK_REQUIRE(value <= 64.0 && value != 0.0 && (double)(int)value == value, "dag_gang must be an integer in 1..64 (or negative)");
        ls->dag_gang = (int)value;
        ls->dag_tasks.release();
        return 0;
    }
    if (!strcmp(key, "batch_period")) { ls->batch_period = (int)value; return 0; }
    if (!strcmp(key, "dag_trace")) { ls->dag_trace_on = value != 0.0; return 0; }
    if (!strcmp(key, "dag_max_rows")) { ls->dag_max_rows = (int64_t)value; return 0; }
    if (!strcmp(key, "dag_deep_rows")) { ls->dag_deep_rows = (int64_t)value; ls->dag_tasks.release(); return 0; }
    if (!strcmp(key, "bk_fallback")) { ls->bk_fallback = (int)value; return 0; }
    if (!strcmp(key, "bk_panel_wgs")) {
        MNK_REQUIRE(value == 0.0 || value == 1.0, "bk_panel_wgs must be 0 or 1");
        ls->bk_panel_wgs = (int)value;
        return 0;
    }
    if (!strcmp(key, "accept_only_pd")) { ls->accept_only_pd = value != 0; return 0; }
    if (!strcmp(key, "probe")) { ls->probe = value != 0; return 0; }
    if (!strcmp(key, "early_reject")) { ls->early_reject = value != 0; return 0; }
    if (!strcmp(key, "dag_debug")) {
        ls->dag_debug = value != 0.0;
        if (ls->dag_debug && !ls->dag_dbg.p) {
            if (ls->dag_dbg.alloc(8 * 128 + 16 * 1024)) return -2;
            MNK_HIP(hipMemset(ls->dag_dbg.p, 0, (8 * 128 + 16 * 1024) * sizeof(int)));
        }
        return 0;
    }
    if (!strcmp(key, "bk_max_wgs")) {
        MNK_REQUIRE(value >= 0.0 && value <= 256.0, "bk_max_wgs must be in 0..256");
        ls->bk_max_wgs = (int)value;
        return 0;
    }
    if (!strcmp(key, "bk_spin_limit")) {
        MNK_REQUIRE(value >= 1024.0, "bk_spin_limit must be at least 1024");
        ls->bk_spin_limit = (long)value;
        return 0;
    }
    if (!strcmp(key, "debug_bk_missing")) { ls->debug_bk_missing = (int)value; return 0; }
    if (!strcmp(key, "bk_growth_tol")) {
        MNK_REQUIRE(value > 1.0, "bk_growth_tol must be > 1");
        ls->bk_growth_tol = value;
        return 0;
    }
    if (!strcmp(key, "bk_growth_tol_qd")) {
        MNK_REQUIRE(value > 1.0, "bk_growth_tol_qd must be > 1");
        ls->bk_growth_tol_qd = value;
        return 0;
    }
    if (!strcmp(key, "persistent_solve")) { ls->persistent_solve = value != 0.0; return 0; }
    if (!strcmp(key, "ps_spin_limit")) {
        MNK_REQUIRE(value >= 1024.0, "ps_spin_limit must be at least 1024");
        ls->ps_spin_limit = (long)value;
        return 0;
    }
    if (!strcmp(key, "debug_pp_missing")) { ls->debug_pp_missing = (int)value; return 0; }
    if (!strcmp(key, "debug_ps_missing")) { ls->debug_ps_missing = (int)value; return 0; }
    if (!strcmp(key, "solve_trace")) {
        if (value != 0.0) {
            int rc = ls->solve_trace.alloc((size_t)(ls->Np / 64) * 8);
            if (rc) return rc;
            MNK_HIP(hipMemset(ls->solve_trace.p, 0, (size_t)(ls->Np / 64) * 8 * sizeof(unsigned long long)));
        } else {
            ls->solve_trace.release();
        }
        return 0;
    }
    set_error("mnk_ls_set_option: unknown option '%s'", key);
    return -1;
}

static int ensure_wbuf(mnk_ls* ls) {
    if (ls->algo != MNK_LDL || ls->wbuf[0].p) return 0;
    const size_t cnt = (size_t)ls->ldw * std::min<int64_t>(mnk_ls_effective_nbo(ls), ls->Np) + SLACK;
    int rc = ls->wbuf[0].alloc(cnt);
    if (!rc && mnk_ls_effective_nbo(ls) < ls->Np) rc = ls->wbuf[1].alloc(cnt);
    return rc;
}

static unsigned long long* amax_word(mnk_ls* ls) {
    if (!(ls->bk_requested && ls->bk_fallback && ls->algo == MNK_LDL)) return nullptr;
    if (!ls->amax_dev.p && ls->amax_dev.alloc(AMAX_WORDS)) return nullptr;
    (void)hipMemsetAsync(ls->amax_dev.p, 0, AMAX_WORDS * sizeof(unsigned long long), ls->ctx->stream);
    return ls->amax_dev.p;
}

static int prepare_fill(mnk_ls* ls) {
    mnk_ctx* ctx = ls->ctx;
    hipStream_t s = ctx->stream;
    dim3 grid((unsigned)ls->Np, (unsigned)((ls->Np / 2 + 255) / 256));
    bool pre = ls->prefill && ls->Np <= ls->prefill_max_rows;
    if (pre && !ls->fact_spare.p) {
        if (ls->fact_spare.alloc(ls->fact.n) != 0) { (void)hipGetLastError(); ls->prefill = 0; pre = false; }
        if (pre && !ctx->s_fill && hipStreamCreateWithFlags(&ctx->s_fill, hipStreamNonBlocking) != hipSuccess) { ls->prefill = 0; pre = false; }
        if (pre && (hipEventCreateWithFlags(&ls->ev_spare, hipEventDisableTiming) != hipSuccess ||
                    hipEventCreateWithFlags(&ls->ev_free, hipEventDisableTiming) != hipSuccess)) { ls->prefill = 0; pre = false; }
        if (pre) MNK_HIP(hipMemsetAsync(ls->fact_spare.p, 0, ls->fact_spare.n * sizeof(double), s));
    }
    if (pre && ls->spare_zeroed && ls->spare_by_dag && !ls->info_valid) {
        ls->spare_zeroed = false;
        ls->spare_by_dag = false;
    }
    if (pre && ls->spare_zeroed) {
        std::swap(ls->fact.p, ls->fact_spare.p);
        MNK_HIP(hipStreamWaitEvent(s, ls->ev_spare, 0));
        ls->spare_zeroed = false;
    } else {
        hipLaunchKernelGGL(fill_lower_kernel, grid, dim3(256), 0, s, ls->fact.p, ls->ld, ls->N, ls->Np);
    }
    ls->spare_pending = pre;
    MNK_HIP(hipGetLastError());
    return 0;
}

}
int mnk_ls_prefill_spare(mnk_ls* ls) {
    if (!ls->spare_pending) return 0;
    ls->spare_pending = false;
    if (ls->dag_filled) {
        ls->dag_filled = false;
        MNK_HIP(hipEventRecord(ls->ev_spare, ls->ctx->stream));
        ls->spare_zeroed = true;
        ls->spare_by_dag = true;
        return 0;
    }
    ls->spare_by_dag = false;
    mnk_ctx* ctx = ls->ctx;
    dim3 grid((unsigned)ls->Np, (unsigned)((ls->Np / 2 + 255) / 256));
    MNK_HIP(hipEventRecord(ls->ev_free, ctx->stream));
    MNK_HIP(hipStreamWaitEvent(ctx->s_fill, ls->ev_free, 0));
    hipLaunchKernelGGL(fill_lower_kernel, grid, dim3(256), 0, ctx->s_fill, ls->fact_spare.p, ls->ld, ls->N, ls->Np);
    MNK_HIP(hipGetLastError());
    MNK_HIP(hipEventRecord(ls->ev_spare, ctx->s_fill));
    ls->spare_zeroed = true;
    return 0;
}
extern "C" {

static int* set_envelope(mnk_ls* ls, const int32_t* env_dev, const std::vector<int32_t>& env_host) {
    ls->env_dev = nullptr;
    if (!ls->envelope || env_dev == nullptr || ls->algo == MNK_QR || ls->algo == MNK_LU || ls->algo == MNK_EVD) return nullptr;
    if (!ls->env_word.p) {
        if (ls->env_word.alloc(2) || hipMemsetAsync(ls->env_word.p, 0, 2 * sizeof(int), ls->ctx->stream) != hipSuccess) {
            (void)hipGetLastError();
            ls->env_word.release();
            return nullptr;
        }
    }
    if (ls->env_armed && hipMemsetAsync(ls->env_word.p, 0, sizeof(int), ls->ctx->stream) != hipSuccess) { (void)hipGetLastError(); return nullptr; }
    ls->env_armed = true;
    ls->env_dev = env_dev;
    ls->env_host.assign(env_host.begin(), env_host.begin() + std::min<size_t>(env_host.size(), (size_t)(ls->Np / 128)));
    return ls->env_word.p;
}

static int transfer_sc(mnk_ls* ls, mnk_sc* sc) {
    int rc = prepare_fill(ls);
    if (rc) return rc;
    const int64_t nnz = sc->nnz_aug;
    int* nonfinite = set_envelope(ls, sc->d_tile_env.p, sc->tile_env);
    hipLaunchKernelGGL(scatter_csc_kernel, dim3((unsigned)((nnz + 255) / 256)), dim3(256), 0, ls->ctx->stream,
                       ls->fact.p, ls->ld, sc->aug_row.p, sc->aug_col.p, sc->aug_nz.p, nnz, amax_word(ls),
                       ls->N < sc->n ? (int32_t)ls->N : INT32_MAX, nonfinite);
    MNK_HIP(hipGetLastError());
    return 0;
}

static int probe_leading_block(mnk_ls* ls, mnk_sc* sc, bool* rejected) {
    *rejected = false;
    if (!(ls->probe && ls->early_reject && ls->accept_only_pd && ls->algo == MNK_LDL && ls->N == sc->n && !mnk_batch_active())) return 0;
    if (ls->probe_last_rejected || ls->probe_hint_col < 0 || ls->probe_since_hint > 3) return 0;
    const int64_t m = (ls->probe_hint_col + 256) / 256 * 256;
    if (m < 512 || 2 * m > ls->N) return 0;
    if (ls->probe_ls == nullptr || ls->probe_order != m) {
        if (ls->probe_ls) { (void)mnk_ls_destroy(ls->probe_ls); ls->probe_ls = nullptr; }
        mnk_ls* child = nullptr;
        if (mnk_ls_create(ls->ctx, m, ls->algo, &child) != 0) { (void)hipGetLastError(); return 0; }
        child->probe = 0;
        child->accept_only_pd = 1;
        child->early_reject = 1;
        ls->probe_ls = child;
        ls->probe_order = m;
    }
    mnk_ls* c = ls->probe_ls;
    c->pivot_tol = ls->pivot_tol;
    c->envelope = ls->envelope;
    if (c->dag_xcd_queues != ls->dag_xcd_queues || c->dag_gang != ls->dag_gang) {
        c->dag_xcd_queues = ls->dag_xcd_queues;
        c->dag_gang = ls->dag_gang;
        c->dag_tasks.release();
    }
    int rc = mnk_ls_factorize_sc_async(c, sc);
    if (!rc) rc = mnk_ls_fetch_info(c);
    if (rc) return rc;
    if (c->npos == m && c->nzero == 0 && c->nneg == 0) { ++ls->probe_misses; return 0; }
    ++ls->probe_hits;
    ++ls->early_rejects;
    ls->early_reject_col = c->factor_invalid ? c->early_reject_col : m - 1;
    ls->info = 1;
    ls->npos = c->npos;
    ls->nzero = c->nzero;
    ls->nneg = ls->N - ls->npos - ls->nzero;
    ls->factor_invalid = true;
    ls->info_valid = true;
    ls->factorized = true;
    ls->bk_active = false;
    ls->probe_last_rejected = true;
    if (2 * ls->early_reject_col < ls->N) { ls->probe_hint_col = ls->early_reject_col; ls->probe_since_hint = 0; }
    *rejected = true;
    return 0;
}

int mnk_ls_factorize_sc_async(mnk_ls* ls, mnk_sc* sc) {
    MNK_REQUIRE(ls && sc && sc->ctx, "mnk_ls_factorize_sc: NULL argument or host-only handle");
    MNK_REQUIRE(sc->n >= ls->N, "mnk_ls_factorize_sc: the solver's order exceeds the KKT system's");
    MNK_HIP(hipSetDevice(ls->ctx->device));
    { int rc_d = mnk_ls_sync_deferred(ls); if (rc_d) return rc_d; }
    int rc = ensure_wbuf(ls);
    if (rc) return rc;
    bool probe_rejected = false;
    rc = probe_leading_block(ls, sc, &probe_rejected);
    if (rc) return rc;
    if (!probe_rejected) {
        rc = transfer_sc(ls, sc);
        if (rc) return rc;
    }
    ls->src_persistent = true;
    ls->retransfer = [ls, sc, w = std::weak_ptr<int>(sc->alive)]() {
        if (w.expired()) {
            set_error("factorize!: the KKT handle of the last factorize! call was destroyed before its inertia was fetched; the "
                      "matrix cannot be transferred again for the fall-back tier");
            return -5;
        }
        return transfer_sc(ls, sc);
    };
    if (probe_rejected) return 0;
    return mnk_ls_run_factorization(ls);
}

static int transfer_dense(mnk_ls* ls, const double* Adev, int64_t lda) {
    ls->env_dev = nullptr;
    dim3 grid((unsigned)ls->Np, (unsigned)((ls->Np + 1023) / 1024));
    hipLaunchKernelGGL(copy_lower_kernel, grid, dim3(256), 0, ls->ctx->stream, ls->fact.p, ls->ld, Adev, lda,
                       ls->N, ls->Np, amax_word(ls));
    MNK_HIP(hipGetLastError());
    return 0;
}

static int factorize_dense_dev(mnk_ls* ls, const double* Adev, int64_t lda, bool src_persistent = false) {
    int rc = ensure_wbuf(ls);
    if (rc) return rc;
    rc = transfer_dense(ls, Adev, lda);
    if (rc) return rc;
    ls->src_persistent = src_persistent;
    ls->retransfer = [ls, Adev, lda]() { return transfer_dense(ls, Adev, lda); };
    return mnk_ls_run_factorization(ls);
}

}
int mnk_ls_factorize_dense_dev_async(mnk_ls* ls, const double* Adev, int64_t lda) {
    MNK_REQUIRE(ls && Adev && lda >= ls->N, "mnk_ls_factorize_dense_dev_async: bad argument");
    MNK_HIP(hipSetDevice(ls->ctx->device));
    { int rc_d = mnk_ls_sync_deferred(ls); if (rc_d) return rc_d; }
    return factorize_dense_dev(ls, Adev, lda);
}
extern "C" {

int mnk_ls_factorize_dc_async(mnk_ls* ls, mnk_dc* dc) {
    MNK_REQUIRE(ls && dc, "mnk_ls_factorize_dc: NULL argument");
    MNK_REQUIRE(dc->order == ls->N, "mnk_ls_factorize_dc: order mismatch");
    MNK_HIP(hipSetDevice(ls->ctx->device));
    { int rc_d = mnk_ls_sync_deferred(ls); if (rc_d) return rc_d; }
    int rc = factorize_dense_dev(ls, dc->aug.p, round_up(dc->order, PAD), true);
    ls->retransfer = [ls, dc, w = std::weak_ptr<int>(dc->alive)]() {
        if (w.expired()) {
            set_error("factorize!: the KKT handle of the last factorize! call was destroyed before its inertia was fetched; the "
                      "matrix cannot be transferred again for the fall-back tier");
            return -5;
        }
        return transfer_dense(ls, dc->aug.p, round_up(dc->order, PAD));
    };
    return rc;
}

static int finish_info(mnk_ls* ls, int* info) {
    int rc = mnk_ls_fetch_info(ls);
    if (rc) return rc;
    if (info) *info = ls->info;
    return 0;
}

int mnk_ls_factorize_sc(mnk_ls* ls, mnk_sc* sc, int* info) {
    int rc = mnk_ls_factorize_sc_async(ls, sc);
    return rc ? rc : finish_info(ls, info);
}

int mnk_ls_factorize_dc(mnk_ls* ls, mnk_dc* dc, int* info) {
    int rc = mnk_ls_factorize_dc_async(ls, dc);
    return rc ? rc : finish_info(ls, info);
}

int mnk_ls_factorize_dense(mnk_ls* ls, const double* A, int64_t lda, int loc, int* info) {
    MNK_REQUIRE(ls && A, "mnk_ls_factorize_dense: NULL argument");
    MNK_REQUIRE(lda >= ls->N, "mnk_ls_factorize_dense: lda < N");
    MNK_HIP(hipSetDevice(ls->ctx->device));
    { int rc_d = mnk_ls_sync_deferred(ls); if (rc_d) return rc_d; }
    int rc;
    if (loc == MNK_DEVICE) {
        rc = factorize_dense_dev(ls, A, lda);
    } else {
        DevBuf<double> tmp;
        rc = tmp.alloc((size_t)ls->N * ls->N);
        if (rc) return rc;
        MNK_HIP(mnk::h2d_copy_2d(tmp.p, ls->N * sizeof(double), A, lda * sizeof(double), ls->N * sizeof(double), ls->N,
                                 ls->ctx->stream));
        rc = factorize_dense_dev(ls, tmp.p, ls->N);
        MNK_HIP(mnk::stream_wait(ls->ctx->stream));
        if (!rc) rc = finish_info(ls, info);
        ls->retransfer = nullptr;
        return rc;
    }
    rc = rc ? rc : finish_info(ls, info);
    ls->retransfer = nullptr;
    return rc;
}

int mnk_ls_factorize_csc(mnk_ls* ls, const int32_t* colptr, const int32_t* rowval, const double* nzval,
                         int index_base, int* info) {
    MNK_REQUIRE(ls && colptr && rowval && nzval, "mnk_ls_factorize_csc: NULL argument");
    MNK_HIP(hipSetDevice(ls->ctx->device));
    { int rc_d = mnk_ls_sync_deferred(ls); if (rc_d) return rc_d; }
    const int64_t N = ls->N;
    const int64_t nnz = colptr[N] - index_base;
    std::vector<int32_t> row(nnz), col(nnz);
    for (int64_t c = 0; c < N; ++c)
        for (int64_t k = colptr[c] - index_base; k < colptr[c + 1] - index_base; ++k) {
            row[k] = rowval[k] - index_base;
            col[k] = (int32_t)c;
            MNK_REQUIRE(row[k] >= c && row[k] < N, "mnk_ls_factorize_csc: matrix must be lower triangular");
        }
    DevBuf<int32_t> drow, dcol;
    DevBuf<double> dnz;
    std::vector<double> nzv(nzval, nzval + nnz);
    int rc = drow.upload(row, ls->ctx->stream);
    rc |= dcol.upload(col, ls->ctx->stream);
    rc |= dnz.upload(nzv, ls->ctx->stream);
    const std::vector<int32_t> env = ls->envelope ? mnk_tile_envelope(N, row.data(), col.data(), nnz) : std::vector<int32_t>();
    if (ls->envelope) rc |= ls->env_own.upload(env, ls->ctx->stream);
    if (rc) return -2;
    rc = ensure_wbuf(ls);
    if (rc) return rc;
    auto transfer = [ls, nnz, &drow, &dcol, &dnz, &env]() -> int {
        int r = prepare_fill(ls);
// ... 387 lines not shown
```

### madnlp.jl_amd/csrc/solve.hip

```cpp
#include <mutex>

#include <atomic>

#include "gemm_tile.h"
#include "ls.h"

namespace mnk {

constexpr int SB = 256;
typedef double v2d __attribute__((ext_vector_type(2)));

__device__ __forceinline__ void mm64x16_acc(const double* As, const double* Bs, double (&c)[4], int ty, int tx) {
#pragma unroll 8
    for (int k = 0; k < 64; ++k) {
        const double b = Bs[tx * 64 + k];
#pragma unroll
        for (int i = 0; i < 4; ++i) c[i] = fma(As[k * 64 + 4 * ty + i], b, c[i]);
    }
}

template <int S>
__global__ __launch_bounds__(256) void linv_tri_kernel(const double* __restrict__ F, int64_t ld,
                                                      const double* __restrict__ Linv64, double* __restrict__ Inv,
                                                      double* __restrict__ InvT, int64_t Np,
                                                      const int* __restrict__ info, int blk0) {
    __shared__ double As[64 * 64];
    __shared__ double Bs[16 * 64];
    if (*info != 0) return;
    const int64_t blk = (int64_t)blockIdx.x + blk0;
    const int q = blockIdx.y;
    const int cs = blockIdx.z;
    const int64_t j0 = blk * S;
    const int nb = (int)((Np - j0 < S ? Np - j0 : S) / 64);
    double* out = Inv + blk * (int64_t)(S * S);
    double* outT = InvT + blk * (int64_t)(S * S);
    const int t = threadIdx.x, ty = t & 15, tx = t >> 4;
    const int col = 64 * q + 16 * cs + tx;
    for (int e = t; e < 64 * q * 16; e += 256) {
        const int r = e % (64 * q), c = 64 * q + 16 * cs + e / (64 * q);
        out[r + (int64_t)c * S] = 0.0;
        outT[c + (int64_t)r * S] = 0.0;
    }
    if (q >= nb) {
        for (int e = t; e < 16 * S; e += 256) {
            const int r = e % S, c = 64 * q + 16 * cs + e / S;
            out[r + (int64_t)c * S] = 0.0;
            outT[c + (int64_t)r * S] = 0.0;
        }
        return;
    }
    for (int b = q; b < S / 64; ++b) {
        double c[4] = {0.0, 0.0, 0.0, 0.0};
        if (b < nb) {
            if (b == q) {
                const double* Li = Linv64 + ((j0 >> 6) + q) * 4096;
#pragma unroll
                for (int i = 0; i < 4; ++i) c[i] = Li[(4 * ty + i) + 64 * (16 * cs + tx)];
            } else {
                for (int bp = q; bp < b; ++bp) {
                    __syncthreads();
                    for (int e = t; e < 4096; e += 256) {
                        const int r = e & 63, k = e >> 6;
                        As[k * 64 + r] = F[(j0 + 64 * b + r) + (j0 + 64 * bp + k) * ld];
                    }
                    for (int e = t; e < 1024; e += 256) {
                        const int k = e & 63, j = e >> 6;
                        Bs[j * 64 + k] = out[(64 * bp + k) + (int64_t)(64 * q + 16 * cs + j) * S];
                    }
                    __syncthreads();
                    mm64x16_acc(As, Bs, c, ty, tx);
                }
                __syncthreads();
#pragma unroll
                for (int i = 0; i < 4; ++i) Bs[tx * 64 + 4 * ty + i] = c[i];
                const double* Li = Linv64 + ((j0 >> 6) + b) * 4096;
                for (int e = t; e < 4096; e += 256) As[e] = Li[e];
                __syncthreads();
#pragma unroll
                for (int i = 0; i < 4; ++i) c[i] = 0.0;
                mm64x16_acc(As, Bs, c, ty, tx);
#pragma unroll
                for (int i = 0; i < 4; ++i) c[i] = -c[i];
            }
        }
#pragma unroll
        for (int i = 0; i < 4; ++i) {
            const int r = 64 * b + 4 * ty + i;
            out[r + (int64_t)col * S] = c[i];
            outT[col + (int64_t)r * S] = c[i];
        }
        __threadfence_block();
        __syncthreads();
    }
}

__global__ __launch_bounds__(256) void linv256_mfma_kernel(const double* __restrict__ F, int64_t ld, const double* __restrict__ Linv64,
                                                           double* __restrict__ Inv,
                                                           double* __restrict__ InvT, int64_t Np, const int* __restrict__ info,
                                                           int blk0, const mnk::SmallSysRec* __restrict__ recs = nullptr) {
    __shared__ v4f64 tile[1024];
    if (recs != nullptr) {
        const mnk::SmallSysRec r = recs[blockIdx.z];
        F = r.F; ld = r.ld; Linv64 = r.linv; Inv = r.linv256; InvT = r.linv256t; Np = r.Np; info = r.info;
    }
    if (*info != 0) return;
    const int64_t blk = (int64_t)blockIdx.x + blk0;
    const int q = blockIdx.y;
    const int64_t j0 = blk * SB;
    const int nb = (int)((Np - j0 < SB ? Np - j0 : SB) / 64);
    double* out = Inv + blk * (int64_t)(SB * SB);
    double* outT = InvT + blk * (int64_t)(SB * SB);
    const int tid = threadIdx.x, lane = tid & 63, w = __builtin_amdgcn_readfirstlane(tid >> 6);
    const int l15 = lane & 15, l4 = lane >> 4;
    const int row = 64 * q + 16 * w + l15;
    v4f64 X[16];
#pragma unroll
    for (int g = 0; g < 16; ++g)
#pragma unroll
        for (int r = 0; r < 4; ++r) X[g][r] = (q < nb && 16 * g + l4 + 4 * r == row) ? 1.0 : 0.0;
    auto step = [&](auto Jc) __attribute__((always_inline)) {
        constexpr int j = decltype(Jc)::value;
        if (j >= q && j < nb && q < nb) {
            const double* Li = Linv64 + ((j0 >> 6) + j) * 4096;
#pragma unroll
            for (int cb = 3; cb >= 0; --cb) {
                v4f64 x = {0.0, 0.0, 0.0, 0.0};
#pragma unroll
                for (int ib = 0; ib <= cb; ++ib)
#pragma unroll
                    for (int s = 0; s < 4; ++s)
                        x = __builtin_amdgcn_mfma_f64_16x16x4f64(Li[(16 * cb + l15) + 64 * (16 * ib + 4 * s + l4)], X[4 * j + ib][s], x, 0, 0, 0);
                X[4 * j + cb] = x;
            }
#pragma unroll
            for (int c = j + 1; c < 4; ++c) {
                if (c >= nb) break;
                __syncthreads();
                {
                    const double* src = F + (j0 + 64 * c + lane) + (j0 + 64 * j + w) * ld;
#pragma unroll
                    for (int ib = 0; ib < 4; ++ib) {
                        v4f64 pre;
#pragma unroll
                        for (int s = 0; s < 4; ++s) pre[s] = src[(16 * ib + 4 * s) * ld];
                        tile[((lane >> 4) * 4 + ib) * 64 + (lane & 15) + 16 * w] = pre;
                    }
                }
                __syncthreads();
#pragma unroll
                for (int cb2 = 0; cb2 < 4; ++cb2)
#pragma unroll
                    for (int ib = 0; ib < 4; ++ib) {
                        const v4f64 a = tile[(cb2 * 4 + ib) * 64 + lane];
#pragma unroll
                        for (int s = 0; s < 4; ++s)
                            X[4 * c + cb2] = __builtin_amdgcn_mfma_f64_16x16x4f64(-a[s], X[4 * j + ib][s], X[4 * c + cb2], 0, 0, 0);
                    }
            }
        }
    };
    step(std::integral_constant<int, 0>{});
    step(std::integral_constant<int, 1>{});
    step(std::integral_constant<int, 2>{});
    step(std::integral_constant<int, 3>{});
#pragma unroll
    for (int g = 0; g < 16; ++g)
#pragma unroll
        for (int r = 0; r < 4; ++r) {
            const int c = 16 * g + l4 + 4 * r;
            const double v = (c >= row && c < 64 * nb) ? X[g][r] : 0.0;
            outT[row + (int64_t)c * SB] = v;
            out[c + (int64_t)row * SB] = v;
        }
}

__global__ __launch_bounds__(1024) void diag256_kernel(const double* __restrict__ M, const double* __restrict__ b,
                                                       double* __restrict__ x, int upper, int nrow) {
    __shared__ double bs[SB];
    __shared__ double part[4][SB];
    const int t = threadIdx.x, r = t & 255, p = t >> 8;
    if (t < SB) bs[t] = t < nrow ? b[t] : 0.0;
    __syncthreads();
    double a0 = 0.0, a1 = 0.0, a2 = 0.0, a3 = 0.0;
    const int rb = r >> 6;
    if (upper ? p >= rb : p <= rb) {
        const double* Mr = M + r + (int64_t)(64 * p) * SB;
        const double* bp = bs + 64 * p;
#pragma unroll 8
        for (int c = 0; c < 64; c += 4) {
            a0 += Mr[(int64_t)(c + 0) * SB] * bp[c + 0];
            a1 += Mr[(int64_t)(c + 1) * SB] * bp[c + 1];
            a2 += Mr[(int64_t)(c + 2) * SB] * bp[c + 2];
            a3 += Mr[(int64_t)(c + 3) * SB] * bp[c + 3];
        }
    }
    part[p][r] = (a0 + a1) + (a2 + a3);
    __syncthreads();
    if (p == 0 && r < nrow) x[r] = (part[0][r] + part[1][r]) + (part[2][r] + part[3][r]);
}

__global__ void scale_vec_kernel(double* __restrict__ y, const double* __restrict__ dinv, int64_t n) {
    const int64_t i = blockIdx.x * (int64_t)blockDim.x + threadIdx.x;
    if (i < n) y[i] *= dinv[i];
}

__global__ __launch_bounds__(256) void fwd_panel_kernel(const double* __restrict__ F, int64_t ld,
                                                        const double* __restrict__ x, double* __restrict__ b,
                                                        int64_t j0, int ncol, int64_t Np) {
    __shared__ double xs[SB];
    __shared__ double part[4][64];
    const int t = threadIdx.x, row = t & 63, p = t >> 6;
    xs[t] = t < ncol ? x[j0 + t] : 0.0;
    __syncthreads();
    const int64_t r = j0 + ncol + (int64_t)blockIdx.x * 64 + row;
    double s0 = 0.0, s1 = 0.0;
    if (r < Np) {
        const int c0 = p * (ncol / 4), c1 = c0 + ncol / 4;
        const double* Fr = F + r + j0 * ld;
#pragma unroll 8
        for (int c = c0; c < c1; c += 2) {
            s0 += Fr[(int64_t)c * ld] * xs[c];
            s1 += Fr[(int64_t)(c + 1) * ld] * xs[c + 1];
        }
    }
    part[p][row] = s0 + s1;
    __syncthreads();
    if (p == 0 && r < Np) b[r] -= (part[0][row] + part[1][row]) + (part[2][row] + part[3][row]);
}

__global__ __launch_bounds__(256) void bwd_panel_kernel(const double* __restrict__ F, int64_t ld,
                                                        const double* __restrict__ x, double* __restrict__ z,
                                                        int64_t j0, int nrow) {
    __shared__ double xs[SB];
    const int t = threadIdx.x;
    xs[t] = t < nrow ? x[j0 + t] : 0.0;
    __syncthreads();
    const int64_t cb = (int64_t)blockIdx.x * 64;
    const int lane = t & 63, w = t >> 6;
    const int sub = lane & 15, colq = lane >> 4;
    double acc[4] = {0.0, 0.0, 0.0, 0.0};
    for (int rb = 0; rb < nrow; rb += 64) {
        const double x0 = xs[rb + 4 * sub], x1 = xs[rb + 4 * sub + 1], x2 = xs[rb + 4 * sub + 2],
                     x3 = xs[rb + 4 * sub + 3];
#pragma unroll
        for (int pass = 0; pass < 4; ++pass) {
            const int64_t col = cb + pass * 16 + w * 4 + colq;
            const double* Fp = F + j0 + rb + 4 * sub + col * ld;
            acc[pass] += (Fp[0] * x0 + Fp[1] * x1) + (Fp[2] * x2 + Fp[3] * x3);
        }
    }
#pragma unroll
    for (int pass = 0; pass < 4; ++pass) {
        double s = acc[pass];
        s += __shfl_xor(s, 1);
        s += __shfl_xor(s, 2);
        s += __shfl_xor(s, 4);
        s += __shfl_xor(s, 8);
        const int64_t col = cb + pass * 16 + w * 4 + colq;
        if (sub == 0) z[col] -= s;
    }
}


constexpr int PS_MAXOWN = 12;
constexpr int PS_NEAR = 3;
constexpr int PS_DAHEAD = 3;

__device__ __forceinline__ void ps_publish(double* p, double v) {
    __hip_atomic_store(reinterpret_cast<unsigned long long*>(p), (unsigned long long)__double_as_longlong(v),
                       __ATOMIC_RELAXED, __HIP_MEMORY_SCOPE_AGENT);
}

__device__ __forceinline__ void ps_barrier() { asm volatile("s_waitcnt lgkmcnt(0)\n\ts_barrier" ::: "memory"); }

__device__ __forceinline__ bool ps_gather(const double* src, int n, double* dst, int* abort_flag, long spin_limit,
                                          bool relaxed = false, int nap = 6, int* s_bad = nullptr) {
    const int t = threadIdx.x;
    int bad = 0;
    if (t < n) {
        const unsigned long long* p = reinterpret_cast<const unsigned long long*>(src + t);
        unsigned long long u = __hip_atomic_load(p, __ATOMIC_RELAXED, __HIP_MEMORY_SCOPE_AGENT);
        long spins = 0;
        while (u == ~0ull) {
            if (relaxed) { for (int z = 0; z < nap; ++z) __builtin_amdgcn_s_sleep(8); }
            else if (spins < 256) __builtin_amdgcn_s_sleep(1);
            else __builtin_amdgcn_s_sleep(24);
            if ((++spins & 1023) == 0) {
                if (__hip_atomic_load(abort_flag, __ATOMIC_RELAXED, __HIP_MEMORY_SCOPE_AGENT) != 0) { bad = 1; break; }
                if (spins > spin_limit) {
                    __hip_atomic_store(abort_flag, 1, __ATOMIC_RELAXED, __HIP_MEMORY_SCOPE_AGENT);
                    bad = 1;
                    break;
                }
            }
            u = __hip_atomic_load(p, __ATOMIC_RELAXED, __HIP_MEMORY_SCOPE_AGENT);
        }
        dst[t] = __longlong_as_double((long long)u);
    }
    if (s_bad != nullptr) {
        if (bad) *s_bad = 1;
        ps_barrier();
        return *s_bad == 0;
    }
    return __syncthreads_or(bad) == 0;
}

__global__ void pad_copy_kernel(double* __restrict__ dst, const double* __restrict__ src, int64_t N, int64_t Np) {
    const int64_t k = blockIdx.x * (int64_t)blockDim.x + threadIdx.x;
    if (k < Np) dst[k] = k < N ? src[k] : 0.0;
}

__global__ void ps_reset_kernel(unsigned long long* pub, int64_t n) {
    const int64_t i = blockIdx.x * (int64_t)blockDim.x + threadIdx.x;
    if (i < n) pub[i] = ~0ull;
}

constexpr int PS_NT = 1024;
constexpr int PS_NQ = PS_NT / 64;
constexpr int PS_CW = 256 / PS_NQ;

template <bool LDL>
__device__ __forceinline__ void persistent_solve_body(
    const double* __restrict__ F, int64_t ld, const double* __restrict__ Inv, const double* __restrict__ InvT,
    const double* __restrict__ dinv, const double* xin ,
    double* xout , int64_t N,
    double* __restrict__ pub ,
    double* __restrict__ pub_other ,
    int64_t Np, int* abort_flag,
    const int* __restrict__ info, unsigned long long* __restrict__ trace ,
    int near_steps, int nap, long spin_limit, int missing_wg, const int G, const int g) {
#define PS_STAMP(blk, slot) do { if (trace != nullptr && t == 0) trace[(int64_t)(blk) * 8 + (slot)] = wall_clock64(); } while (0)
    __shared__ double run[PS_MAXOWN][64];
    __shared__ double ysol[PS_MAXOWN][64];
    __shared__ double xs[256];
    __shared__ double part[PS_NQ][64];
    __shared__ int s_bad;
    const int t = threadIdx.x, r = t & 63, q = t >> 6;
    const int nb = (int)(Np / 64);
    const int nsteps = (nb + 3) / 4;
    const int nown = g < nb ? (nb - g + G - 1) / G : 0;
    if (pub_other != nullptr)
        for (int e = t; e < nown * 256; e += PS_NT) {
            const int m = e >> 8, arr = (e >> 6) & 3;
            reinterpret_cast<unsigned long long*>(pub_other)[(int64_t)arr * Np + (int64_t)(g + m * G) * 64 + (e & 63)] = ~0ull;
        }
    if (*info != 0) return;
    if (nown == 0) return;
    if (g == missing_wg) return;
    double* bfin = pub;
    double* ypub = pub + Np;
    double* zfin = pub + 2 * Np;
    double* xpub = pub + 3 * Np;
    for (int e = t; e < nown * 64; e += PS_NT) {
        const int64_t row = (int64_t)(g + (e >> 6) * G) * 64 + (e & 63);
        run[e >> 6][e & 63] = row < N ? xin[row] : 0.0;
    }
    if (t == 0) s_bad = 0;
    __syncthreads();

    double a[PS_CW];
    double d[PS_CW];
    auto dot_chunk = [&](const double (&v)[PS_CW], bool active) {
        double s0 = 0.0, s1 = 0.0, s2 = 0.0, s3 = 0.0;
        if (active) {
            const double* xq = xs + q * PS_CW;
#pragma unroll
            for (int j = 0; j < PS_CW; j += 4) {
                s0 = fma(v[j], xq[j], s0);
                s1 = fma(v[j + 1], xq[j + 1], s1);
                s2 = fma(v[j + 2], xq[j + 2], s2);
                s3 = fma(v[j + 3], xq[j + 3], s3);
            }
        }
        part[q][r] = (s0 + s1) + (s2 + s3);
    };
    auto reduce_parts = [&](int c) {
        double sm = 0.0;
#pragma unroll
        for (int u = 0; u < PS_NQ; ++u) sm += part[u][c];
        return sm;
    };
    const int qb = (q * PS_CW) >> 6;

    int m0 = 0;
    bool have_d = false;
    bool pub_b = false;
    for (int k = 0; k < nsteps && m0 < nown; ++k) {
        const int b0 = 4 * k, nbk = nb - b0 < 4 ? nb - b0 : 4;
        int i = g + m0 * G;
        if (i < b0 + nbk) {
            const int li = i - b0;
            if (!have_d) {
                const double* Mk = Inv + (int64_t)k * (SB * SB) + (li * 64 + r) + (int64_t)(q * PS_CW) * SB;
                if (qb <= li) {
#pragma unroll
                    for (int j = 0; j < PS_CW; ++j) d[j] = Mk[(int64_t)j * SB];
                }
            }
            if (!pub_b && t < 64) ps_publish(bfin + (int64_t)i * 64 + t, run[m0][t]);
            if (t < 64) xs[li * 64 + t] = run[m0][t];
            if (!ps_gather(bfin + (int64_t)b0 * 64, li * 64, xs, abort_flag, spin_limit, false, 6, &s_bad)) return;
            PS_STAMP(i, 3);
            dot_chunk(d, qb <= li);
            ps_barrier();
            if (t < 64) {
                const double v = reduce_parts(t);
                ps_publish(ypub + (int64_t)i * 64 + t, v);
                ysol[m0][t] = v;
            }
            PS_STAMP(i, 4);
            have_d = false;
            pub_b = false;
            ++m0;
            if (m0 >= nown) break;
            i = g + m0 * G;
        }
        const bool diag_next = i < b0 + nbk + 4;
        {
            const double* Fs = F + ((int64_t)i * 64 + r) + ((int64_t)b0 * 64 + q * PS_CW) * ld;
            if (qb < nbk) {
#pragma unroll
                for (int j = 0; j < PS_CW; ++j) a[j] = Fs[(int64_t)j * ld];
            }
            if (!have_d && i < b0 + nbk + 4 * PS_DAHEAD) {
                const int li = i & 3;
                const double* Mk = Inv + (int64_t)(i >> 2) * (SB * SB) + (li * 64 + r) + (int64_t)(q * PS_CW) * SB;
                if (qb <= li) {
#pragma unroll
                    for (int j = 0; j < PS_CW; ++j) d[j] = Mk[(int64_t)j * SB];
                }
                have_d = true;
            }
        }
        if (diag_next) PS_STAMP(i, 0);
        if (!ps_gather(ypub + (int64_t)b0 * 64, nbk * 64, xs, abort_flag, spin_limit, i >= b0 + nbk + 4 * near_steps, nap, &s_bad)) return;
        if (diag_next) PS_STAMP(i, 1);
        for (int m = m0; m < nown; ++m) {
            const int im = g + m * G;
            if (m > m0 && qb < nbk) {
                const double* Fs = F + ((int64_t)im * 64 + r) + ((int64_t)b0 * 64 + q * PS_CW) * ld;
#pragma unroll
                for (int j = 0; j < PS_CW; ++j) a[j] = Fs[(int64_t)j * ld];
            }
            dot_chunk(a, qb < nbk);
            ps_barrier();
            if (t < 64) {
                const double v = run[m][t] - reduce_parts(t);
                run[m][t] = v;
                if (m == m0 && diag_next) ps_publish(bfin + (int64_t)im * 64 + t, v);
            }
            if (m == m0 && diag_next) PS_STAMP(im, 2);
            if (m + 1 < nown) ps_barrier();
        }
        pub_b = diag_next;
    }

    __syncthreads();
    for (int e = t; e < nown * 64; e += PS_NT) {
        const int m = e >> 6, c = e & 63;
        const double y = ysol[m][c];
        run[m][c] = LDL ? y * dinv[(int64_t)(g + m * G) * 64 + c] : y;
    }
    __syncthreads();
    const int lane = t & 63, sub = lane & 15, colq = lane >> 4, rc = q & 3, cg = q >> 2;
    int m1 = nown - 1;
    have_d = false;
    pub_b = false;
    for (int k = nsteps - 1; k >= 0 && m1 >= 0; --k) {
        const int b0 = 4 * k, nbk = nb - b0 < 4 ? nb - b0 : 4;
        int i = g + m1 * G;
        if (i >= b0) {
            const int li = i - b0;
            const bool act = qb >= li && qb < nbk;
            if (!have_d) {
                const double* Mk = InvT + (int64_t)k * (SB * SB) + (li * 64 + r) + (int64_t)(q * PS_CW) * SB;
                if (act) {
#pragma unroll
                    for (int j = 0; j < PS_CW; ++j) d[j] = Mk[(int64_t)j * SB];
                }
            }
            if (!pub_b && t < 64) ps_publish(zfin + (int64_t)i * 64 + t, run[m1][t]);
            if (t < 64) xs[li * 64 + t] = run[m1][t];
            if (!ps_gather(zfin + (int64_t)(i + 1) * 64, (nbk - 1 - li) * 64, xs + (li + 1) * 64, abort_flag, spin_limit, false, 6, &s_bad)) return;
            dot_chunk(d, act);
            ps_barrier();
            if (t < 64) {
                const double v = reduce_parts(t);
                ps_publish(xpub + (int64_t)i * 64 + t, v);
                if ((int64_t)i * 64 + t < N) xout[(int64_t)i * 64 + t] = v;
            }
            have_d = false;
            pub_b = false;
            --m1;
            if (m1 < 0) break;
            i = g + m1 * G;
        }
        auto load_slice = [&](int im, double (&dst)[PS_CW], int bs) {
            const double* Fs = F + ((int64_t)bs * 64 + 64 * rc + 4 * sub) + ((int64_t)im * 64 + cg * 16 + colq) * ld;
#pragma unroll
            for (int p = 0; p < 4; ++p) {
                const v2d lo = *reinterpret_cast<const v2d*>(Fs + (int64_t)(4 * p) * ld);
                const v2d hi = *reinterpret_cast<const v2d*>(Fs + (int64_t)(4 * p) * ld + 2);
                dst[4 * p] = lo[0];
                dst[4 * p + 1] = lo[1];
                dst[4 * p + 2] = hi[0];
                dst[4 * p + 3] = hi[1];
            }
        };
        const bool diag_next = i >= b0 - 4;
        if (rc < nbk) load_slice(i, a, b0);
        if (!have_d && i >= b0 - 4 * PS_DAHEAD) {
            const int li = i & 3;
            const double* Mk = InvT + (int64_t)(i >> 2) * (SB * SB) + (li * 64 + r) + (int64_t)(q * PS_CW) * SB;
            if (qb >= li) {
#pragma unroll
                for (int j = 0; j < PS_CW; ++j) d[j] = Mk[(int64_t)j * SB];
            }
            have_d = true;
        }
        if (!ps_gather(xpub + (int64_t)b0 * 64, nbk * 64, xs, abort_flag, spin_limit, i < b0 - 4 * near_steps, nap, &s_bad)) return;
        for (int m = m1; m >= 0; --m) {
            const int im = g + m * G;
            if (m < m1 && rc < nbk) load_slice(im, a, b0);
            if (rc < nbk) {
                const double x0 = xs[64 * rc + 4 * sub], x1 = xs[64 * rc + 4 * sub + 1],
                             x2 = xs[64 * rc + 4 * sub + 2], x3 = xs[64 * rc + 4 * sub + 3];
#pragma unroll
                for (int p = 0; p < 4; ++p) {
                    double sp = (a[4 * p] * x0 + a[4 * p + 1] * x1) + (a[4 * p + 2] * x2 + a[4 * p + 3] * x3);
                    sp += __shfl_xor(sp, 1);
                    sp += __shfl_xor(sp, 2);
                    if ((sub & 3) == 0) part[rc * 4 + (sub >> 2)][cg * 16 + 4 * p + colq] = sp;
                }
            } else if (lane < 16) {
#pragma unroll
                for (int u = 0; u < 4; ++u) part[rc * 4 + u][cg * 16 + lane] = 0.0;
            }
            ps_barrier();
            if (t < 64) {
                const double v = run[m][t] - reduce_parts(t);
                run[m][t] = v;
                if (m == m1 && diag_next) ps_publish(zfin + (int64_t)im * 64 + t, v);
            }
            if (m > 0) ps_barrier();
        }
        pub_b = diag_next;
    }
#undef PS_STAMP
}

template <bool LDL>
__global__ __launch_bounds__(PS_NT) void persistent_solve_kernel(
    const double* __restrict__ F, int64_t ld, const double* __restrict__ Inv, const double* __restrict__ InvT,
    const double* __restrict__ dinv, const double* xin, double* xout, int64_t N, double* __restrict__ pub,
    double* __restrict__ pub_other, int64_t Np, int* abort_flag, const int* __restrict__ info,
    unsigned long long* __restrict__ trace, int near_steps, int nap, long spin_limit, int missing_wg) {
    persistent_solve_body<LDL>(F, ld, Inv, InvT, dinv, xin, xout, N, pub, pub_other, Np, abort_flag, info, trace, near_steps, nap,
                               spin_limit, missing_wg, (int)gridDim.x, (int)blockIdx.x);
}

struct PsSys {
    const double* F;
    int64_t ld;
    const double* Inv;
    const double* InvT;
    const double* dinv;
    const double* xin;
    double* xout;
    int64_t N;
    double* pub;
    double* pub_other;
    int* abort_flag;
    const int* info;
};
typedef const PsSys __attribute__((address_space(4))) * PsSysP;

template <bool LDL>
__global__ __launch_bounds__(PS_NT) void persistent_solve_multi_kernel(const PsSys* __restrict__ sys, int G, int64_t Np, int near_steps,
                                                                      int nap, long spin_limit) {
    const int isys = (int)blockIdx.x / G, g = (int)blockIdx.x % G;
    const PsSysP y = (PsSysP)(uintptr_t)(sys + isys);
    persistent_solve_body<LDL>(y->F, y->ld, y->Inv, y->InvT, y->dinv, y->xin, y->xout, y->N, y->pub, y->pub_other, Np, y->abort_flag,
                               y->info, nullptr, near_steps, nap, spin_limit, -1, G, g);
}

__global__ void ps_set_sys_kernel(PsSys rec, PsSys* __restrict__ dst) { *dst = rec; }


constexpr int P5_RB = 32, P5_NBS = 16, P5_STEP = 512, P5_NQ = 32, P5_CW = 16;

template <bool LDL>
__global__ __launch_bounds__(PS_NT) void persistent_solve512_kernel(
    const double* __restrict__ F, int64_t ld, const double* __restrict__ Inv, const double* __restrict__ InvT,
    const double* __restrict__ dinv, double* __restrict__ xio, double* __restrict__ pub, int64_t Np, int* abort_flag,
    const int* __restrict__ info, int near_steps, int nap, long spin_limit, int missing_wg) {
    __shared__ double run[PS_MAXOWN][P5_RB];
    __shared__ double ysol[PS_MAXOWN][P5_RB];
    __shared__ double xs[P5_STEP];
    __shared__ double part[P5_NQ][P5_RB];
    if (*info != 0) return;
    const int t = threadIdx.x, r = t & 31, q = t >> 5;
    const int G = gridDim.x, g = blockIdx.x;
    const int nb = (int)(Np / P5_RB);
    const int nsteps = (nb + P5_NBS - 1) / P5_NBS;
    const int nown = g < nb ? (nb - g + G - 1) / G : 0;
    if (nown == 0) return;
    if (g == missing_wg) return;
    double* bfin = pub;
    double* ypub = pub + Np;
    double* zfin = pub + 2 * Np;
    double* xpub = pub + 3 * Np;
    for (int e = t; e < nown * P5_RB; e += PS_NT) run[e >> 5][e & 31] = xio[(int64_t)(g + (e >> 5) * G) * P5_RB + (e & 31)];
    __syncthreads();

    double a[P5_CW], d[P5_CW];
    auto dot_chunk = [&](const double (&v)[P5_CW], bool active) {
        double s0 = 0.0, s1 = 0.0, s2 = 0.0, s3 = 0.0;
        if (active) {
            const double* xq = xs + q * P5_CW;
#pragma unroll
            for (int j = 0; j < P5_CW; j += 4) {
                s0 = fma(v[j], xq[j], s0);
                s1 = fma(v[j + 1], xq[j + 1], s1);
                s2 = fma(v[j + 2], xq[j + 2], s2);
                s3 = fma(v[j + 3], xq[j + 3], s3);
            }
        }
        part[q][r] = (s0 + s1) + (s2 + s3);
    };
    auto reduce_parts = [&](int c, int n) {
        double sm = 0.0;
        for (int u = 0; u < n; ++u) sm += part[u][c];
        return sm;
    };
    const int qb = q >> 1;

    int m0 = 0;
    bool have_d = false;
    for (int k = 0; k < nsteps && m0 < nown; ++k) {
        const int b0 = P5_NBS * k, nbk = nb - b0 < P5_NBS ? nb - b0 : P5_NBS;
        int i = g + m0 * G;
        if (i < b0 + nbk) {
            const int li = i - b0;
            if (!have_d) {
                const double* Mk = Inv + (int64_t)k * (P5_STEP * P5_STEP) + (li * P5_RB + r) + (int64_t)(q * P5_CW) * P5_STEP;
                if (qb <= li) {
#pragma unroll
                    for (int j = 0; j < P5_CW; ++j) d[j] = Mk[(int64_t)j * P5_STEP];
                }
                if (t < P5_RB) ps_publish(bfin + (int64_t)i * P5_RB + t, run[m0][t]);
            }
            if (t < P5_RB) xs[li * P5_RB + t] = run[m0][t];
            if (!ps_gather(bfin + (int64_t)b0 * P5_RB, li * P5_RB, xs, abort_flag, spin_limit)) return;
            dot_chunk(d, qb <= li);
            __syncthreads();
            if (t < P5_RB) {
                const double v = reduce_parts(t, P5_NQ);
                ps_publish(ypub + (int64_t)i * P5_RB + t, v);
                ysol[m0][t] = v;
            }
            have_d = false;
            ++m0;
            if (m0 >= nown) break;
            i = g + m0 * G;
        }
        const bool diag_next = i < b0 + nbk + P5_NBS;
        {
            const double* Fs = F + ((int64_t)i * P5_RB + r) + ((int64_t)b0 * P5_RB + q * P5_CW) * ld;
            if (qb < nbk) {
#pragma unroll
                for (int j = 0; j < P5_CW; ++j) a[j] = Fs[(int64_t)j * ld];
            }
            if (diag_next) {
                const int li = i - (b0 + nbk);
                const double* Mk = Inv + (int64_t)(k + 1) * (P5_STEP * P5_STEP) + (li * P5_RB + r) + (int64_t)(q * P5_CW) * P5_STEP;
                if (qb <= li) {
#pragma unroll
                    for (int j = 0; j < P5_CW; ++j) d[j] = Mk[(int64_t)j * P5_STEP];
                }
            }
        }
        if (!ps_gather(ypub + (int64_t)b0 * P5_RB, nbk * P5_RB, xs, abort_flag, spin_limit, i >= b0 + nbk + P5_NBS * near_steps, nap)) return;
        for (int m = m0; m < nown; ++m) {
            const int im = g + m * G;
            if (m > m0 && qb < nbk) {
                const double* Fs = F + ((int64_t)im * P5_RB + r) + ((int64_t)b0 * P5_RB + q * P5_CW) * ld;
#pragma unroll
                for (int j = 0; j < P5_CW; ++j) a[j] = Fs[(int64_t)j * ld];
            }
            dot_chunk(a, qb < nbk);
            __syncthreads();
            if (t < P5_RB) {
                const double v = run[m][t] - reduce_parts(t, P5_NQ);
                run[m][t] = v;
                if (m == m0 && diag_next) ps_publish(bfin + (int64_t)im * P5_RB + t, v);
            }
            if (m + 1 < nown) __syncthreads();
        }
        have_d = diag_next;
    }

    __syncthreads();
    for (int e = t; e < nown * P5_RB; e += PS_NT) {
        const int m = e >> 5, c = e & 31;
        const double y = ysol[m][c];
        run[m][c] = LDL ? y * dinv[(int64_t)(g + m * G) * P5_RB + c] : y;
    }
    __syncthreads();
    const int lane = t & 63, sub = lane & 7, colq = lane >> 3, rc = t >> 6;
    int m1 = nown - 1;
    have_d = false;
    for (int k = nsteps - 1; k >= 0 && m1 >= 0; --k) {
        const int b0 = P5_NBS * k, nbk = nb - b0 < P5_NBS ? nb - b0 : P5_NBS;
        int i = g + m1 * G;
        if (i >= b0) {
            const int li = i - b0;
            const bool act = qb >= li && qb < nbk;
            if (!have_d) {
                const double* Mk = InvT + (int64_t)k * (P5_STEP * P5_STEP) + (li * P5_RB + r) + (int64_t)(q * P5_CW) * P5_STEP;
                if (act) {
#pragma unroll
                    for (int j = 0; j < P5_CW; ++j) d[j] = Mk[(int64_t)j * P5_STEP];
                }
                if (t < P5_RB) ps_publish(zfin + (int64_t)i * P5_RB + t, run[m1][t]);
            }
            if (t < P5_RB) xs[li * P5_RB + t] = run[m1][t];
            if (!ps_gather(zfin + (int64_t)(i + 1) * P5_RB, (nbk - 1 - li) * P5_RB, xs + (li + 1) * P5_RB, abort_flag, spin_limit)) return;
            dot_chunk(d, act);
            __syncthreads();
            if (t < P5_RB) {
                const double v = reduce_parts(t, P5_NQ);
                ps_publish(xpub + (int64_t)i * P5_RB + t, v);
                xio[(int64_t)i * P5_RB + t] = v;
            }
            have_d = false;
            --m1;
            if (m1 < 0) break;
            i = g + m1 * G;
        }
        auto load_slice = [&](int im) {
            const double* Fs = F + ((int64_t)b0 * P5_RB + 32 * rc + 4 * sub) + ((int64_t)im * P5_RB + colq) * ld;
#pragma unroll
            for (int p = 0; p < 4; ++p) {
                const v2d lo = *reinterpret_cast<const v2d*>(Fs + (int64_t)(8 * p) * ld);
                const v2d hi = *reinterpret_cast<const v2d*>(Fs + (int64_t)(8 * p) * ld + 2);
                a[4 * p] = lo[0];
                a[4 * p + 1] = lo[1];
                a[4 * p + 2] = hi[0];
                a[4 * p + 3] = hi[1];
            }
        };
        const bool diag_next = i >= b0 - P5_NBS;
        if (rc < nbk) load_slice(i);
        if (diag_next) {
            const int li = i - (b0 - P5_NBS);
            const double* Mk = InvT + (int64_t)(k - 1) * (P5_STEP * P5_STEP) + (li * P5_RB + r) + (int64_t)(q * P5_CW) * P5_STEP;
            if (qb >= li) {
#pragma unroll
                for (int j = 0; j < P5_CW; ++j) d[j] = Mk[(int64_t)j * P5_STEP];
            }
        }
        if (!ps_gather(xpub + (int64_t)b0 * P5_RB, nbk * P5_RB, xs, abort_flag, spin_limit, i < b0 - P5_NBS * near_steps, nap)) return;
        for (int m = m1; m >= 0; --m) {
            const int im = g + m * G;
            if (m < m1 && rc < nbk) load_slice(im);
            if (rc < nbk) {
                const double x0 = xs[32 * rc + 4 * sub], x1 = xs[32 * rc + 4 * sub + 1], x2 = xs[32 * rc + 4 * sub + 2],
                             x3 = xs[32 * rc + 4 * sub + 3];
#pragma unroll
                for (int p = 0; p < 4; ++p) {
                    double sp = (a[4 * p] * x0 + a[4 * p + 1] * x1) + (a[4 * p + 2] * x2 + a[4 * p + 3] * x3);
                    sp += __shfl_xor(sp, 1);
                    sp += __shfl_xor(sp, 2);
                    sp += __shfl_xor(sp, 4);
                    if (sub == 0) part[rc][colq + 8 * p] = sp;
                }
            } else if (lane < P5_RB) {
                part[rc][lane] = 0.0;
            }
            __syncthreads();
            if (t < P5_RB) {
                const double v = run[m][t] - reduce_parts(t, P5_NBS);
                run[m][t] = v;
                if (m == m1 && diag_next) ps_publish(zfin + (int64_t)im * P5_RB + t, v);
            }
            if (m > 0) __syncthreads();
        }
        have_d = diag_next;
    }
}


__global__ __launch_bounds__(512) void inv512_assemble_kernel(const double* __restrict__ Inv256, const double* __restrict__ InvT256,
                                                              double* __restrict__ Inv512, double* __restrict__ InvT512, int64_t Np,
                                                              int t0, const int* __restrict__ info) {
    if (*info != 0) return;
    const int64_t t = (int64_t)blockIdx.x + t0;
    const int col = blockIdx.y, row = threadIdx.x;
    const int64_t nblk256 = (Np + 255) / 256;
    double v = 0.0, vt = 0.0;
    const int qr = row >> 8, qc = col >> 8;
    if (qr == qc && 2 * t + qr < nblk256) {
        const int64_t off = (2 * t + qr) * 65536 + (row & 255) + (int64_t)(col & 255) * 256;
        v = Inv256[off];
        vt = InvT256[off];
    }
    Inv512[t * 262144 + row + (int64_t)col * 512] = v;
    InvT512[t * 262144 + row + (int64_t)col * 512] = vt;
}
template <int STAGE>
__global__ __launch_bounds__(256, 3) void inv512_gemm_kernel(const double* __restrict__ F, int64_t ld, const double* __restrict__ Inv256,
                                                             const double* __restrict__ InvT256, double* __restrict__ Tt,
                                                             double* __restrict__ Inv512, double* __restrict__ InvT512, int64_t Np,
                                                             int t0, const int* __restrict__ info) {
    extern __shared__ __attribute__((aligned(16))) char smem_raw[];
    if (*info != 0) return;
    const int64_t t = (int64_t)blockIdx.x + t0;
    if ((2 * t + 1) * 256 >= Np) return;
    const int tm = blockIdx.y & 1, tn = blockIdx.y >> 1;
    const double* IA_t = InvT256 + (2 * t) * 65536;
    const double* ID = Inv256 + (2 * t + 1) * 65536;
    double* T = Tt + t * 65536;
    if (STAGE == 1) {
        const double* C = F + (512 * t + 256) + (512 * t) * ld;
        gemm_nt_tile<2, 2, 4, 1, false, 0, 8>(tm, tn, 256, 256, 256, IA_t, 256, C, ld, T, 256, nullptr, nullptr, 0, smem_raw);
    } else if (blockIdx.z == 0) {
        gemm_nt_tile<2, 2, 4, 0, false, 0, 8>(tm, tn, 256, 256, 256, ID, 256, T, 256, Inv512 + t * 262144 + 256, 512, nullptr, nullptr, 0, smem_raw);
    } else {
        gemm_nt_tile<2, 2, 4, 0, false, 0, 8>(tm, tn, 256, 256, 256, T, 256, ID, 256, InvT512 + t * 262144 + (int64_t)256 * 512, 512, nullptr, nullptr, 0, smem_raw);
    }
}

}

using namespace mnk;

int mnk_ls_build_inverses(mnk_ls* ls, hipStream_t s, int64_t sc0, int64_t sc1) {
    const int64_t nblk = std::min<int64_t>(sc1, (ls->Np + SB - 1) / SB) - sc0;
    if (nblk <= 0) return 0;
    if (!ls->linv_mfma)
        hipLaunchKernelGGL(linv_tri_kernel<256>, dim3((unsigned)nblk, 4, 4), dim3(256), 0, s, ls->fact.p, ls->ld, ls->linv.p,
                           ls->linv256.p, ls->linv256t.p, ls->Np, ls->info_dev.p, (int)sc0);
    else
        hipLaunchKernelGGL(linv256_mfma_kernel, dim3((unsigned)nblk, 4), dim3(256), 0, s, ls->fact.p, ls->ld, ls->linv.p,
                           ls->linv256.p, ls->linv256t.p, ls->Np, ls->info_dev.p, (int)sc0);
    if (ls->solve512 && ls->Np >= ls->solve512_min_rows && ls->Np % 512 != 384 && !ls->linv512.p) {
        const size_t ntri = (size_t)((ls->Np + 511) / 512);
        if (ls->linv512.alloc(ntri * 512 * 512) || ls->linv512t.alloc(ntri * 512 * 512) || ls->linv512tmp.alloc(ntri * 256 * 256)) {
            (void)hipGetLastError();
            ls->linv512.release(); ls->linv512t.release(); ls->linv512tmp.release();
            ls->solve512 = 0;
        }
    }
    if (ls->solve512 && ls->linv512.p) {
        const int64_t nsc = (ls->Np + SB - 1) / SB;
        const int64_t t0 = (sc0 + 1) / 2, t1 = std::min<int64_t>(sc1, nsc) == nsc ? (ls->Np + 511) / 512 : sc1 / 2;
        if (t1 > t0) {
            const unsigned nt = (unsigned)(t1 - t0);
            static std::atomic<uint64_t> attr_devs{0};
            int dev = 0;
            MNK_HIP(hipGetDevice(&dev));
            const int smem = 2 * 8 * ((128 + 16) + (128 + 16)) * (int)sizeof(double);
            if (!(attr_devs.load(std::memory_order_relaxed) >> (dev & 63) & 1)) {
                MNK_HIP(hipFuncSetAttribute((const void*)inv512_gemm_kernel<1>, hipFuncAttributeMaxDynamicSharedMemorySize, smem));
                MNK_HIP(hipFuncSetAttribute((const void*)inv512_gemm_kernel<2>, hipFuncAttributeMaxDynamicSharedMemorySize, smem));
                attr_devs.fetch_or(1ull << (dev & 63), std::memory_order_relaxed);
            }
            hipLaunchKernelGGL(inv512_assemble_kernel, dim3(nt, 512), dim3(512), 0, s, ls->linv256.p, ls->linv256t.p, ls->linv512.p,
                               ls->linv512t.p, ls->Np, (int)t0, ls->info_dev.p);
            hipLaunchKernelGGL(inv512_gemm_kernel<1>, dim3(nt, 4, 1), dim3(256), smem, s, ls->fact.p, ls->ld, ls->linv256.p, ls->linv256t.p,
                               ls->linv512tmp.p, ls->linv512.p, ls->linv512t.p, ls->Np, (int)t0, ls->info_dev.p);
            hipLaunchKernelGGL(inv512_gemm_kernel<2>, dim3(nt, 4, 2), dim3(256), smem, s, ls->fact.p, ls->ld, ls->linv256.p, ls->linv256t.p,
                               ls->linv512tmp.p, ls->linv512.p, ls->linv512t.p, ls->Np, (int)t0, ls->info_dev.p);
        }
    }
    MNK_HIP(hipGetLastError());
    return 0;
}

int mnk_ls_build_inverses_batch(hipStream_t s, const mnk::SmallSysRec* recs_dev, int n, int64_t Np) {
    const unsigned nblk = (unsigned)((Np + SB - 1) / SB);
    hipLaunchKernelGGL(linv256_mfma_kernel, dim3(nblk, 4, (unsigned)n), dim3(256), 0, s, (const double*)nullptr, (int64_t)0,
                       (const double*)nullptr, (double*)nullptr, (double*)nullptr, (int64_t)0, (const int*)nullptr, 0, recs_dev);
    MNK_HIP(hipGetLastError());
    return 0;
}

int mnk_solve_warmup(hipStream_t s) {
    static mnk::DevBuf<int> one;
    if (!one.p) {
        if (one.alloc(1)) return -2;
        const int v = 1;
        { mnk::H2DGuard h2d; MNK_HIP(hipMemcpy(one.p, &v, sizeof(int), hipMemcpyHostToDevice)); }
    }
    hipLaunchKernelGGL(linv256_mfma_kernel, dim3(1, 4), dim3(256), 0, s, (const double*)nullptr, (int64_t)0, (const double*)nullptr,
                       (double*)nullptr, (double*)nullptr, (int64_t)256, one.p, 0);
    MNK_HIP(hipGetLastError());
    return 0;
}

int mnk_ls_run_solve(mnk_ls* ls, double* xdev, double* xuser) {
    hipStream_t s = ls->ctx->stream;
    const int64_t Np = ls->Np, ld = ls->ld, N = ls->N;
    const int ldl = ls->algo == MNK_LDL;
    const int64_t nb64 = Np / 64;
    const int G = (int)std::min<int64_t>(nb64, ls->ctx->num_cu);
    const bool bk = ls->bk_active;
    const bool persistent = !bk && ls->persistent_solve && G >= 1 && (nb64 + G - 1) / G <= PS_MAXOWN && (G >= 4 || nb64 <= G);
    const int64_t nb32 = Np / P5_RB;
    const int G5 = (int)std::min<int64_t>(nb32, ls->ctx->num_cu);
    const bool use512 = persistent && ls->solve512 && ls->linv512.p && (nb32 + G5 - 1) / G5 <= PS_MAXOWN && (G5 >= P5_NBS || nb32 <= G5);
    const bool direct = persistent && !use512;
    auto stage_in = [&]() -> int {
        if (xuser != nullptr) hipLaunchKernelGGL(pad_copy_kernel, dim3((unsigned)((Np + 255) / 256)), dim3(256), 0, s, xdev, xuser, N, Np);
        MNK_HIP(hipGetLastError());
        return 0;
    };
    auto stage_out = [&]() -> int {
        if (xuser != nullptr) MNK_HIP(hipMemcpyAsync(xuser, xdev, N * sizeof(double), hipMemcpyDeviceToDevice, s));
        return 0;
    };
    if (!direct) {
        int rc = stage_in();
        if (rc) return rc;
    }
    if (bk) {
        ls->pub_clean[0] = false;
        int rc = mnk_ls_bk_permute(ls, xdev, xdev + 2 * Np, true);
        if (rc) return rc;
    }
    if (persistent) {
        int rc = mnk_persist_begin(ls->ctx, s);
        if (rc) return rc;
        const int ps_near = PS_NEAR, ps_nap = 6;
        double* pubs[2] = {xdev + 2 * Np, xdev + 6 * Np};
        auto ensure_clean = [&](int b) {
            if (!ls->pub_clean[b])
                hipLaunchKernelGGL(ps_reset_kernel, dim3((unsigned)((4 * Np + 255) / 256)), dim3(256), 0, s,
                                   reinterpret_cast<unsigned long long*>(pubs[b]), 4 * Np);
            ls->pub_clean[b] = true;
        };
        if (use512) {
            ls->pub_clean[0] = false;
            ensure_clean(0);
            double* pub = pubs[0];
            if (ldl)
                hipLaunchKernelGGL(persistent_solve512_kernel<true>, dim3(G5), dim3(PS_NT), 0, s, ls->fact.p, ld, ls->linv512.p,
                                   ls->linv512t.p, ls->dinv.p, xdev, pub, Np, ls->solve_abort, ls->info_dev.p, ps_near, ps_nap,
                                   ls->ps_spin_limit, ls->debug_ps_missing);
            else
                hipLaunchKernelGGL(persistent_solve512_kernel<false>, dim3(G5), dim3(PS_NT), 0, s, ls->fact.p, ld, ls->linv512.p,
                                   ls->linv512t.p, ls->dinv.p, xdev, pub, Np, ls->solve_abort, ls->info_dev.p, ps_near, ps_nap,
                                   ls->ps_spin_limit, ls->debug_ps_missing);
            ls->pub_clean[0] = false;
            rc = hipGetLastError() == hipSuccess ? 0 : -2;
            rc = mnk_persist_end(ls->ctx, s, rc);
            return rc ? rc : stage_out();
        }
        const int cur = ls->pub_next, oth = cur ^ 1;
        ensure_clean(cur);
        const double* xin = xuser != nullptr ? xuser : xdev;
        double* xout = xuser != nullptr ? xuser : xdev;
        const int64_t nio = xuser != nullptr ? N : Np;
        if (ldl)
            hipLaunchKernelGGL(persistent_solve_kernel<true>, dim3(G), dim3(PS_NT), 0, s, ls->fact.p, ld, ls->linv256.p,
                               ls->linv256t.p, ls->dinv.p, xin, xout, nio, pubs[cur], pubs[oth], Np, ls->solve_abort, ls->info_dev.p,
                               ls->solve_trace.p, ps_near, ps_nap, ls->ps_spin_limit, ls->debug_ps_missing);
        else
            hipLaunchKernelGGL(persistent_solve_kernel<false>, dim3(G), dim3(PS_NT), 0, s, ls->fact.p, ld,
                               ls->linv256.p, ls->linv256t.p, ls->dinv.p, xin, xout, nio, pubs[cur], pubs[oth], Np, ls->solve_abort,
                               ls->info_dev.p, ls->solve_trace.p, ps_near, ps_nap, ls->ps_spin_limit,
                               ls->debug_ps_missing);
        ls->pub_clean[cur] = false;
        ls->pub_clean[oth] = ls->debug_ps_missing < 0;
        ls->pub_next = oth;
        rc = hipGetLastError() == hipSuccess ? 0 : -2;
        return mnk_persist_end(ls->ctx, s, rc);
    }
    double* b = xdev;
    double* y = xdev + Np;
    const int64_t nsteps = (Np + SB - 1) / SB;
    for (int64_t k = 0; k < nsteps; ++k) {
        const int64_t j0 = k * SB;
        const int ncol = (int)std::min<int64_t>(SB, Np - j0);
        hipLaunchKernelGGL(diag256_kernel, dim3(1), dim3(1024), 0, s, ls->linv256.p + k * (int64_t)(SB * SB), b + j0,
                           y + j0, 0, ncol);
        const int64_t below = Np - j0 - ncol;
        if (below > 0)
            hipLaunchKernelGGL(fwd_panel_kernel, dim3((unsigned)((below + 63) / 64)), dim3(256), 0, s, ls->fact.p, ld,
                               y, b, j0, ncol, Np);
    }
    if (bk) {
        int rc = mnk_ls_bk_dsolve(ls, y);
        if (rc) return rc;
    } else if (ldl)
        hipLaunchKernelGGL(scale_vec_kernel, dim3((unsigned)((Np + 255) / 256)), dim3(256), 0, s, y, ls->dinv.p, Np);
    for (int64_t k = nsteps - 1; k >= 0; --k) {
        const int64_t j0 = k * SB;
        const int nrow = (int)std::min<int64_t>(SB, Np - j0);
        hipLaunchKernelGGL(diag256_kernel, dim3(1), dim3(1024), 0, s, ls->linv256t.p + k * (int64_t)(SB * SB), y + j0,
                           b + j0, 1, nrow);
        if (j0 > 0)
            hipLaunchKernelGGL(bwd_panel_kernel, dim3((unsigned)(j0 / 64)), dim3(256), 0, s, ls->fact.p, ld, b, y, j0,
                               nrow);
    }
    MNK_HIP(hipGetLastError());
    if (bk) {
        ls->pub_clean[0] = false;
        int rc = mnk_ls_bk_permute(ls, xdev, xdev + 2 * Np, false);
        if (rc) return rc;
    }
    return stage_out();
}

namespace {
struct SolveReq { mnk_ls* ls; double* x; };
struct SolveBatchState { int depth = 0; bool active = false; std::vector<SolveReq> pend; };
thread_local SolveBatchState t_sbatch;
struct SolveBatchBuffers { mnk::DevBuf<char> sys; hipEvent_t ev = nullptr; };
SolveBatchBuffers g_sbatch[64];
constexpr int PS_BATCH_MAXQ = 32;
}

static bool solve_eligible(const mnk_ls* ls) {
    const int64_t nb64 = ls->Np / 64;
    const int G = (int)std::min<int64_t>(nb64, ls->ctx->num_cu);
    return !ls->bk_active && ls->persistent_solve && !(ls->solve512 && ls->linv512.p) && !ls->ctx->partitioned &&
           (nb64 + G - 1) / G <= PS_MAXOWN && (G >= 4 || nb64 <= G) && !(ls->solve_abort && *ls->solve_abort != 0) &&
           ls->debug_ps_missing < 0 && !ls->solve_trace.p;
}

bool mnk_solve_defer(mnk_ls* ls, double* xuser) {
    if (!t_sbatch.active || !solve_eligible(ls)) return false;
    if (!ls->ev_defer && hipEventCreateWithFlags(&ls->ev_defer, hipEventDisableTiming) != hipSuccess) { (void)hipGetLastError(); return false; }
    if (hipEventRecord(ls->ev_defer, ls->ctx->stream) != hipSuccess) { (void)hipGetLastError(); return false; }
    t_sbatch.pend.push_back({ls, xuser});
    return true;
}

static int solve_batch_launch(const std::vector<SolveReq>& v) {
    const int q = (int)v.size();
    mnk_ls* l0 = v[0].ls;
    mnk_ctx* c0 = l0->ctx;
    hipStream_t h = c0->stream;
    MNK_HIP(hipSetDevice(c0->device));
    const int64_t Np = l0->Np, nb64 = Np / 64;
    const int G = (int)std::min<int64_t>(nb64, c0->num_cu / q);
    SolveBatchBuffers& B = g_sbatch[c0->device & 63];
    for (const SolveReq& r : v)
        if (r.ls->ctx->stream != h) MNK_HIP(hipStreamWaitEvent(h, r.ls->ev_defer, 0));
    int rc = mnk_persist_begin(c0, h);
    if (rc) return rc;
    auto body = [&]() -> int {
        if (B.sys.n < sizeof(PsSys) * PS_BATCH_MAXQ && B.sys.alloc(sizeof(PsSys) * PS_BATCH_MAXQ)) return -2;
        if (!B.ev) MNK_HIP(hipEventCreateWithFlags(&B.ev, hipEventDisableTiming));
        PsSys* dsys = reinterpret_cast<PsSys*>(B.sys.p);
        for (int i = 0; i < q; ++i) {
            mnk_ls* ls = v[i].ls;
            double* pubs[2] = {ls->xwork.p + 2 * Np, ls->xwork.p + 6 * Np};
            const int cur = ls->pub_next, oth = cur ^ 1;
            if (!ls->pub_clean[cur])
                hipLaunchKernelGGL(ps_reset_kernel, dim3((unsigned)((4 * Np + 255) / 256)), dim3(256), 0, h,
                                   reinterpret_cast<unsigned long long*>(pubs[cur]), 4 * Np);
            PsSys rec{ls->fact.p, ls->ld, ls->linv256.p, ls->linv256t.p, ls->dinv.p, v[i].x, v[i].x, ls->N, pubs[cur], pubs[oth],
                      ls->solve_abort, ls->info_dev.p};
            hipLaunchKernelGGL(ps_set_sys_kernel, dim3(1), dim3(1), 0, h, rec, dsys + i);
            ls->pub_clean[cur] = false;
            ls->pub_clean[oth] = true;
            ls->pub_next = oth;
        }
        const bool ldl = l0->algo == MNK_LDL;
        if (ldl)
            hipLaunchKernelGGL(persistent_solve_multi_kernel<true>, dim3((unsigned)(q * G)), dim3(PS_NT), 0, h, dsys, G, Np, PS_NEAR, 6, l0->ps_spin_limit);
        else
            hipLaunchKernelGGL(persistent_solve_multi_kernel<false>, dim3((unsigned)(q * G)), dim3(PS_NT), 0, h, dsys, G, Np, PS_NEAR, 6, l0->ps_spin_limit);
        MNK_HIP(hipGetLastError());
        return 0;
    };
    rc = body();
    rc = mnk_persist_end(c0, h, rc);
    if (rc) return rc;
    bool other = false;
    for (const SolveReq& r : v) other = other || r.ls->ctx->stream != h;
    if (other) {
        MNK_HIP(hipEventRecord(B.ev, h));
        for (const SolveReq& r : v)
            if (r.ls->ctx->stream != h) MNK_HIP(hipStreamWaitEvent(r.ls->ctx->stream, B.ev, 0));
    }
    return 0;
}

static int solve_batch_flush() {
    std::vector<SolveReq> pend;
    pend.swap(t_sbatch.pend);
    static const int envq = []() { const char* e = getenv("MNK_SOLVE_BATCH_Q"); return e ? std::max(1, std::min(PS_BATCH_MAXQ, atoi(e))) : 0; }();
    int rc_all = 0;
    while (!pend.empty()) {
        mnk_ls* l0 = pend.front().ls;
        const int64_t nb64 = l0->Np / 64;
        const int g4 = (int)std::max<int64_t>(1, std::min<int64_t>(nb64, l0->ctx->num_cu / 4));
        const int maxq = envq > 0 ? envq : std::max(1, std::min(PS_BATCH_MAXQ, l0->ctx->num_cu / g4));
        std::vector<SolveReq> g, rest;
        for (const SolveReq& r : pend) {
            bool take = (int)g.size() < maxq && r.ls->ctx->device == l0->ctx->device && r.ls->Np == l0->Np && r.ls->algo == l0->algo;
            for (const SolveReq& t : g) take = take && t.ls != r.ls;
            for (const SolveReq& t : rest) take = take && t.ls != r.ls;
            if (take) {
                const int Gq = (int)std::min<int64_t>(nb64, l0->ctx->num_cu / ((int)g.size() + 1));
                take = (Gq >= 4 || nb64 <= Gq) && (nb64 + Gq - 1) / Gq <= PS_MAXOWN;
                take = take || g.empty();
            }
            (take ? g : rest).push_back(r);
        }
        pend.swap(rest);
        int rc;
        if (g.size() >= 2) rc = solve_batch_launch(g);
        else rc = mnk_ls_run_solve(g[0].ls, g[0].ls->xwork.p, g[0].x);
        if (rc && !rc_all) rc_all = rc;
    }
    return rc_all;
}

extern "C" int mnk_solve_batch_begin(void) {
    ++t_sbatch.depth;
    t_sbatch.active = true;
    return 0;
}

extern "C" int mnk_solve_batch_end(void) {
    if (t_sbatch.depth <= 0) { mnk::set_error("mnk_solve_batch_end: no batch is open on this thread"); return -1; }
    if (--t_sbatch.depth > 0) return 0;
    t_sbatch.active = false;
    return solve_batch_flush();
}

int mnk_solve_batch_flush_pending(void) { return t_sbatch.pend.empty() ? 0 : solve_batch_flush(); }

int mnk_solve_sync_deferred(mnk_ls* ls) {
    for (const SolveReq& r : t_sbatch.pend)
        if (r.ls == ls) return solve_batch_flush();
    return 0;
}
```

### madnlp.jl_amd/linear_solver.py

```python
from __future__ import annotations

import atexit
import ctypes as C
import weakref
from dataclasses import dataclass

import numpy as np

from . import _lib as L

BUNCHKAUFMAN, LU, QR, CHOLESKY, LDL, EVD = "BUNCHKAUFMAN", "LU", "QR", "CHOLESKY", "LDL", "EVD"
_ALGO = {BUNCHKAUFMAN: L.MNK_BUNCHKAUFMAN, CHOLESKY: L.MNK_CHOLESKY, LDL: L.MNK_LDL, QR: L.MNK_QR, LU: L.MNK_LU, EVD: L.MNK_EVD}
_NO_INERTIA = (QR, LU)
_HIP_LINEAR_SOLVER_ALGOS = (BUNCHKAUFMAN, CHOLESKY, LDL, QR, EVD)


class LinearSolverException(Exception):
    """reference `src/LinearSolvers/linearsolvers.jl:133`."""


class SymbolicException(LinearSolverException):
    pass


class FactorizationException(LinearSolverException):
    pass


class SolveException(LinearSolverException):
    pass


class InertiaException(LinearSolverException):
    pass


_LIVE_OBJECTS = weakref.WeakSet()
_LIVE_CONTEXTS = weakref.WeakSet()


@atexit.register
def _close_all():
    for obj in list(_LIVE_OBJECTS):
        try:
            obj.close()
        except Exception:
            pass
    for ctx in list(_LIVE_CONTEXTS):
        try:
            ctx.close()
        except Exception:
            pass


class HipContext:

    def __init__(self, device: int = 0, stream: int | None = None):
        self._h = C.c_void_p()
        L.check(L.lib().mnk_ctx_create(device, C.c_void_p(stream) if stream else None, C.byref(self._h)),
                "mnk_ctx_create")
        self.device = device
        _LIVE_CONTEXTS.add(self)

    @property
    def handle(self):
        return self._h

    def synchronize(self):
        L.check(L.lib().mnk_ctx_synchronize(self._h), "mnk_ctx_synchronize")

    def stream(self) -> int:
        return L.lib().mnk_ctx_stream(self._h) or 0

    def close(self):
        if self._h:
            L.lib().mnk_ctx_destroy(self._h)
            self._h = C.c_void_p()

    def __del__(self):
        try:
            self.close()
        except Exception:
            pass


class factorize_batch:

    def __enter__(self):
        L.check(L.lib().mnk_factorize_batch_begin(), "mnk_factorize_batch_begin")
        return self

    def __exit__(self, et, ev, tb):
        rc = L.lib().mnk_factorize_batch_end()
        if rc and et is None:
            raise FactorizationException(L.lib().mnk_last_error_string().decode())
        return False


def release_idle_streams(device: int = 0):
    L.check(L.lib().mnk_release_idle_streams(int(device)), "mnk_release_idle_streams")


class solve_batch:

    def __enter__(self):
        L.check(L.lib().mnk_solve_batch_begin(), "mnk_solve_batch_begin")
        return self

    def __exit__(self, et, ev, tb):
        rc = L.lib().mnk_solve_batch_end()
        if rc and et is None:
            raise SolveException(L.lib().mnk_last_error_string().decode())
        return False


def _ptr(a):
    if a is None:
        return None, L.MNK_HOST
    if isinstance(a, np.ndarray):
        return C.c_void_p(a.ctypes.data), L.MNK_HOST
    return C.c_void_p(a.data_ptr()), (L.MNK_DEVICE if a.is_cuda else L.MNK_HOST)


@dataclass
class HipSolverOptions:
    lapack_algorithm: str = BUNCHKAUFMAN
    pivot_tol: float = 0.0
    outer_block: int = 0
    lookahead: bool = True
    share: int = 1
    small_tiles: int = 400
    persistent_solve: bool = True
    single_rows: int = 2560
    panel_algo: int = 5


class HipLinearSolver:

    _algorithms = _HIP_LINEAR_SOLVER_ALGOS

    def __init__(self, A, ctx: HipContext | None = None, opt: HipSolverOptions | None = None):
        self.opt = opt or HipSolverOptions()
        if self.opt.lapack_algorithm not in self._algorithms:
            hint = " (LU: HipLUSolver)" if self.opt.lapack_algorithm == LU else ""
            raise SymbolicException(
                f"algorithm {self.opt.lapack_algorithm} is not served by {type(self).__name__} "
                f"({', '.join(self._algorithms)}){hint}")
        self.A = A
        self.ctx = ctx or getattr(A, "ctx", None) or HipContext()
        self.n = _order_of(A)
        self._h = C.c_void_p()
        rc = L.lib().mnk_ls_create(self.ctx.handle, self.n, _ALGO[self.opt.lapack_algorithm], C.byref(self._h))
        if rc:
            raise SymbolicException(L.lib().mnk_last_error_string().decode())
        settings = [("pivot_tol", self.opt.pivot_tol), ("outer_block", self.opt.outer_block),
                    ("lookahead", float(self.opt.lookahead)), ("share", float(self.opt.share)),
                    ("small_tiles", float(self.opt.small_tiles)), ("persistent_solve", float(self.opt.persistent_solve)),
                    ("single_rows", float(self.opt.single_rows)), ("panel_algo", float(self.opt.panel_algo))]
        for key, val in settings:
            L.check(L.lib().mnk_ls_set_option(self._h, key.encode(), float(val)), "mnk_ls_set_option")
        self.info = 0
        _LIVE_OBJECTS.add(self)

    def introduce(self) -> str:
        return f"HIP-MI355X ({self.opt.lapack_algorithm})"

    def improve(self) -> bool:
        return False

    @staticmethod
    def input_type() -> str:
        return "dense"

    @staticmethod
    def default_options():
        return HipSolverOptions()

    @staticmethod
    def is_supported(dtype) -> bool:
        return np.dtype(dtype) == np.float64

    def is_inertia(self) -> bool:
        return self.opt.lapack_algorithm not in _NO_INERTIA

    def factorize(self):
        lib = L.lib()
        info = C.c_int(0)
        A = self.A
        if isinstance(A, DeviceCSC):
            rc = lib.mnk_ls_factorize_sc(self._h, A.owner_handle, C.byref(info))
        elif isinstance(A, DeviceDense):
            rc = lib.mnk_ls_factorize_dc(self._h, A.owner_handle, C.byref(info))
        elif isinstance(A, tuple):
            colptr, rowval, nzval = (np.ascontiguousarray(A[0], dtype=np.int32),
                                     np.ascontiguousarray(A[1], dtype=np.int32),
                                     np.ascontiguousarray(A[2], dtype=np.float64))
            rc = lib.mnk_ls_factorize_csc(self._h, colptr.ctypes.data, rowval.ctypes.data, nzval.ctypes.data, 0,
                                          C.byref(info))
        else:
            p, loc = _ptr(A)
            lda = A.shape[0] if isinstance(A, np.ndarray) else max(A.stride())
            if isinstance(A, np.ndarray) and not A.flags.f_contiguous:
                raise FactorizationException("dense matrices must be column-major (order='F')")
            rc = lib.mnk_ls_factorize_dense(self._h, p, lda, loc, C.byref(info))
        if rc:
            raise FactorizationException(lib.mnk_last_error_string().decode())
        self.info = info.value
        return self

    def factorize_async(self):
        lib = L.lib()
        A = self.A
        if isinstance(A, DeviceCSC):
            rc = lib.mnk_ls_factorize_sc_async(self._h, A.owner_handle)
        elif isinstance(A, DeviceDense):
            rc = lib.mnk_ls_factorize_dc_async(self._h, A.owner_handle)
        else:
            raise FactorizationException("factorize_async needs a device-resident matrix")
        if rc:
            raise FactorizationException(lib.mnk_last_error_string().decode())
        return self

    def inertia(self):
        if not self.is_inertia():
            raise InertiaException(f"{self.opt.lapack_algorithm} reveals no inertia")
        p, z, n = C.c_int64(), C.c_int64(), C.c_int64()
        rc = L.lib().mnk_ls_inertia(self._h, C.byref(p), C.byref(z), C.byref(n))
        if rc:
            raise InertiaException(L.lib().mnk_last_error_string().decode())
        return (p.value, z.value, n.value)

    def solve_linear_system(self, x):
        p, loc = _ptr(x)
        if isinstance(x, np.ndarray):
            if x.ndim == 2:
                if not x.flags.f_contiguous:
                    raise SolveException("matrix right-hand sides must be column-major")
                nrhs, ldx = x.shape[1], x.shape[0]
            else:
                if not x.flags.c_contiguous:
                    raise SolveException("x must be contiguous")
                nrhs, ldx = 1, x.shape[0]
        else:
            nrhs, ldx = (1, x.shape[0]) if x.dim() == 1 else (x.shape[1], x.stride(1))
        if ldx < self.n:
            raise SolveException("right-hand side is shorter than the system order")
        rc = L.lib().mnk_ls_solve(self._h, p, nrhs, ldx, loc)
        if rc:
            raise SolveException(L.lib().mnk_last_error_string().decode())
        return x

    def check_solve(self):
        rc = L.lib().mnk_ls_check_solve(self._h)
        if rc:
            raise SolveException(L.lib().mnk_last_error_string().decode())

    def bk_info(self):
        act, cnt = C.c_int(0), C.c_int(0)
        L.check(L.lib().mnk_ls_bk_info(self._h, C.byref(act), C.byref(cnt), None, None), "mnk_ls_bk_info")
        if not act.value:
            return False, cnt.value, None, None
        perm = np.zeros(self.n, dtype=np.int32)
        doff = np.zeros(self.n)
        L.check(L.lib().mnk_ls_bk_info(self._h, C.byref(act), C.byref(cnt), perm.ctypes.data, doff.ctypes.data),
                "mnk_ls_bk_info")
        return True, cnt.value, perm, doff

    def get_stat(self, key: str) -> float:
        v = C.c_double(0.0)
        L.check(L.lib().mnk_ls_get_stat(self._h, key.encode(), C.byref(v)), "mnk_ls_get_stat")
        return v.value

    def set_option(self, key: str, value: float):
        L.check(L.lib().mnk_ls_set_option(self._h, key.encode(), float(value)), "mnk_ls_set_option")

    def get_factor(self):
        Lm = np.zeros((self.n, self.n), order="F")
        D = np.zeros(self.n)
        L.check(L.lib().mnk_ls_get_factor(self._h, Lm.ctypes.data, D.ctypes.data, L.MNK_HOST), "mnk_ls_get_factor")
        return Lm, D

    def get_pivots(self):
        ipiv = np.zeros(self.n, dtype=np.int64)
        L.check(L.lib().mnk_ls_get_pivots(self._h, ipiv.ctypes.data, L.MNK_HOST), "mnk_ls_get_pivots")
        return ipiv

    def get_factor_device(self):
        import torch
        dev = torch.device("cuda", self.ctx.device)
        Lt = torch.empty((self.n, self.n), dtype=torch.float64, device=dev)
        D = torch.empty(self.n, dtype=torch.float64, device=dev)
        L.check(L.lib().mnk_ls_get_factor(self._h, C.c_void_p(Lt.data_ptr()), C.c_void_p(D.data_ptr()), L.MNK_DEVICE),
                "mnk_ls_get_factor")
        return Lt.T, D

    def close(self):
        if self._h:
            rc = L.lib().mnk_ls_destroy(self._h)
            if rc:
                raise RuntimeError("HipLinearSolver.close: " + L.lib().mnk_last_error_string().decode())
            self._h = C.c_void_p()

    def __del__(self):
        try:
            self.close()
        except Exception:
            pass


class HipLUSolver(HipLinearSolver):
    _algorithms = (LU,)

    def __init__(self, A, ctx: HipContext | None = None, opt: HipSolverOptions | None = None):
        super().__init__(A, ctx=ctx, opt=opt or HipSolverOptions(lapack_algorithm=LU))


class DeviceCSC:

    def __init__(self, owner, n, colptr, rowval):
        self.owner = owner
        self.ctx = owner.ctx
        self.m = self.n = n
        self.colptr, self.rowval = colptr, rowval

    @property
    def owner_handle(self):
        return self.owner._h

    @property
    def nzval(self):
        return self.owner._values(L.MNK_SC_AUG, len(self.rowval))

    def to_dense(self):
        d = np.zeros((self.n, self.n), order="F")
        ci = np.repeat(np.arange(self.n), np.diff(self.colptr))
        d[self.rowval, ci] = self.nzval
        return d

    def nzval_host(self):
        return self.nzval

    def to_scipy(self):
        import scipy.sparse as sp
        return sp.csc_matrix((self.nzval, np.asarray(self.rowval), np.asarray(self.colptr)), shape=(self.n, self.n))


class DeviceDense:

    def __init__(self, owner, order):
        self.owner = owner
        self.ctx = owner.ctx
        self.order = order
        self.shape = (order, order)

    @property
    def owner_handle(self):
        return self.owner._h

    def to_host(self):
        out = np.zeros((self.order, self.order), order="F")
        L.check(L.lib().mnk_dc_get_aug(self.owner._h, out.ctypes.data, L.MNK_HOST), "mnk_dc_get_aug")
        return out


class LeadingBlock(DeviceCSC):

    def __init__(self, full: DeviceCSC, m: int):
        keep = np.repeat(np.arange(full.n), np.diff(full.colptr)) < m
        keep &= np.asarray(full.rowval) < m
        colptr = np.concatenate(([0], np.cumsum(np.bincount(np.repeat(np.arange(full.n), np.diff(full.colptr))[keep], minlength=full.n)[:m])))
        super().__init__(full.owner, m, colptr.astype(np.int64), np.asarray(full.rowval)[keep])
        self._keep = keep
        self._full = full

    @property
    def nzval(self):
        return self._full.nzval[self._keep]


def _order_of(A):
    if isinstance(A, DeviceCSC):
        return A.n
    if isinstance(A, DeviceDense):
        return A.order
    if isinstance(A, tuple):
        return len(A[0]) - 1
    if A.shape[0] != A.shape[1]:
        raise SymbolicException("matrix must be square")
    return A.shape[0]
```

Before: 108.4 it/s.

## Add one-hop persistent solve using precomputed W blocks and LDS-staged inverses

Adds a persistent triangular-solve kernel that uses precomputed per-block W matrices (combined inverse and off-diagonal products) built after factorization. This shortens the critical dependency chain in forward and backward substitution from two inter-workgroup publish/gather hops per block to one. Diagonal inverse blocks are also staged into LDS through global_load_lds ahead of use. The cost is an extra W-block build kernel in the factorize path, more memory for wfwd/wbwd, and a larger dynamic LDS request that may lower occupancy. It is on by default through solve_hops=1.

```diff
diff --git a/madnlp.jl_amd/csrc/dag.hip b/madnlp.jl_amd/csrc/dag.hip
--- a/madnlp.jl_amd/csrc/dag.hip
+++ b/madnlp.jl_amd/csrc/dag.hip
@@ -1299,6 +1299,7 @@
                 for (int i = 0; i < k; ++i) {
                     mnk_ls* ls = g[r0 + i];
                     ls->inv_done = nsc;
+                    ls->w_done = ls->w_in_rec ? nsc : 0;
                     if (!ls->ev_info) MNK_HIP(hipEventCreateWithFlags(&ls->ev_info, hipEventDisableTiming));
                     MNK_HIP(hipEventRecord(ls->ev_info, h));
                     ls->ev_info_recorded = true;
diff --git a/madnlp.jl_amd/csrc/factor.hip b/madnlp.jl_amd/csrc/factor.hip
--- a/madnlp.jl_amd/csrc/factor.hip
+++ b/madnlp.jl_amd/csrc/factor.hip
@@ -1220,6 +1220,9 @@
     rec->info = ls->info_dev.p;
     rec->F = ls->fact.p; rec->ld = ls->ld; rec->dblk = ls->dblk.p; rec->linv = ls->linv.p;
     rec->linv256 = ls->linv256.p; rec->linv256t = ls->linv256t.p; rec->Np = ls->Np;
+    const bool w = mnk_ls_w_wanted(ls);
+    rec->wf = w ? ls->wfwd.p : nullptr; rec->wb = w ? ls->wbwd.p : nullptr;
+    ls->w_in_rec = w;
     rec->dvec = ls->dvec.p; rec->ninertia = lmode ? ls->N : 0; rec->pin_dev = ls->pin_dev;
     rec->amax = mnk_ls_growth_word(ls) != nullptr ? ls->amax_dev.p : nullptr;
 }
diff --git a/madnlp.jl_amd/csrc/ls.h b/madnlp.jl_amd/csrc/ls.h
--- a/madnlp.jl_amd/csrc/ls.h
+++ b/madnlp.jl_amd/csrc/ls.h
@@ -130,6 +130,10 @@
     int64_t dag_max_rows = 30720;
     int panel_algo = 5;
     int persistent_solve = 1;
+    int solve_hops = 1;
+    mnk::DevBuf<double> wfwd, wbwd;
+    int64_t w_done = 0;
+    bool w_in_rec = false;
     int solve512 = 0;
     int64_t solve512_min_rows = 4096;
     int dag_chain_inline = 1;
@@ -239,6 +243,8 @@
 int mnk_ls_run_solve(mnk_ls* ls, double* xdev , double* xuser = nullptr );
 int mnk_ls_build_inverses(mnk_ls* ls, hipStream_t s, int64_t sc0, int64_t sc1);
 int mnk_ls_invert_blocks(mnk_ls* ls, hipStream_t s, int64_t sc0, int64_t sc1);
+bool mnk_ls_w_wanted(mnk_ls* ls);
+int mnk_ls_build_wblocks(mnk_ls* ls, hipStream_t s, int64_t sc0, int64_t sc1);
 int mnk_ls_right_trsm_rows(mnk_ls* ls, hipStream_t s, int64_t j0, double* Xrows, double* Vrows, int64_t ldr, int64_t nrows);
 int mnk_ls_run_bunchkaufman(mnk_ls* ls);
 long mnk_ls_dag_spin_limit(const mnk_ls* ls);
@@ -246,6 +252,7 @@
 struct SmallSysRec {
     int* flags; int64_t nflags; int* info;
     double* F; int64_t ld; const double* dblk; double* linv; double* linv256; double* linv256t; int64_t Np;
+    double* wf; double* wb;
     const double* dvec; int64_t ninertia; unsigned long long* pin_dev; const unsigned long long* amax;
 };
 }
diff --git a/madnlp.jl_amd/csrc/ls.hip b/madnlp.jl_amd/csrc/ls.hip
--- a/madnlp.jl_amd/csrc/ls.hip
+++ b/madnlp.jl_amd/csrc/ls.hip
@@ -757,6 +757,11 @@
         return 0;
     }
     if (!strcmp(key, "persistent_solve")) { ls->persistent_solve = value != 0.0; return 0; }
+    if (!strcmp(key, "solve_hops")) {
+        MNK_REQUIRE(value == 1.0 || value == 2.0, "solve_hops must be 1 or 2");
+        ls->solve_hops = (int)value;
+        return 0;
+    }
     if (!strcmp(key, "ps_spin_limit")) {
         MNK_REQUIRE(value >= 1024.0, "ps_spin_limit must be at least 1024");
         ls->ps_spin_limit = (long)value;
diff --git a/madnlp.jl_amd/csrc/solve.hip b/madnlp.jl_amd/csrc/solve.hip
--- a/madnlp.jl_amd/csrc/solve.hip
+++ b/madnlp.jl_amd/csrc/solve.hip
@@ -265,6 +265,7 @@
 constexpr int PS_MAXOWN = 12;
 constexpr int PS_NEAR = 3;
 constexpr int PS_DAHEAD = 3;
+constexpr int PS_INV_LDS_BYTES = 256 * 64 * 8;
 
 __device__ __forceinline__ void ps_publish(double* p, double v) {
     __hip_atomic_store(reinterpret_cast<unsigned long long*>(p), (unsigned long long)__double_as_longlong(v),
@@ -559,6 +560,335 @@
                                spin_limit, missing_wg, (int)gridDim.x, (int)blockIdx.x);
 }
 
+template <bool LDL>
+__device__ __forceinline__ void persistent_solve1_body(
+    const double* __restrict__ F, int64_t ld, const double* __restrict__ Inv, const double* __restrict__ InvT,
+    const double* __restrict__ Wf, const double* __restrict__ Wb,
+    const double* __restrict__ dinv, const double* xin, double* xout, int64_t N,
+    double* __restrict__ pub , double* __restrict__ pub_other,
+    int64_t Np, int* abort_flag, const int* __restrict__ info, unsigned long long* __restrict__ trace ,
+    int near_steps, int nap, long spin_limit, int missing_wg, const int G, const int g) {
+#define PS_STAMP(blk, slot) do { if (trace != nullptr && t == 0) trace[(int64_t)(blk) * 8 + (slot)] = wall_clock64(); } while (0)
+    __shared__ double run[PS_MAXOWN][64];
+    __shared__ double ysol[PS_MAXOWN][64];
+    __shared__ double xs[256];
+    __shared__ double part[PS_NQ][64];
+    __shared__ int s_bad;
+    extern __shared__ __attribute__((aligned(16))) double inv_s[];
+    const int t = threadIdx.x, r = t & 63, q = t >> 6;
+    const int qu = __builtin_amdgcn_readfirstlane(q);
+    const int nb = (int)(Np / 64);
+    const int nsteps = (nb + 3) / 4;
+    const int nown = g < nb ? (nb - g + G - 1) / G : 0;
+    if (pub_other != nullptr)
+        for (int e = t; e < nown * 256; e += PS_NT) {
+            const int m = e >> 8, arr = (e >> 6) & 3;
+            reinterpret_cast<unsigned long long*>(pub_other)[(int64_t)arr * Np + (int64_t)(g + m * G) * 64 + (e & 63)] = ~0ull;
+        }
+    if (*info != 0) return;
+    if (nown == 0) return;
+    if (g == missing_wg) return;
+    double* rfin = pub;
+    double* ypub = pub + Np;
+    double* zfin = pub + 2 * Np;
+    double* xpub = pub + 3 * Np;
+    for (int e = t; e < nown * 64; e += PS_NT) {
+        const int64_t row = (int64_t)(g + (e >> 6) * G) * 64 + (e & 63);
+        run[e >> 6][e & 63] = row < N ? xin[row] : 0.0;
+    }
+    if (t == 0) s_bad = 0;
+    __syncthreads();
+
+    double a[PS_CW];
+    double d[PS_CW];
+    auto dot_chunk = [&](const double (&v)[PS_CW], bool active) {
+        double s0 = 0.0, s1 = 0.0, s2 = 0.0, s3 = 0.0;
+        if (active) {
+            const double* xq = xs + q * PS_CW;
+#pragma unroll
+            for (int j = 0; j < PS_CW; j += 4) {
+                s0 = fma(v[j], xq[j], s0);
+                s1 = fma(v[j + 1], xq[j + 1], s1);
+                s2 = fma(v[j + 2], xq[j + 2], s2);
+                s3 = fma(v[j + 3], xq[j + 3], s3);
+            }
+        }
+        part[q][r] = (s0 + s1) + (s2 + s3);
+    };
+    auto reduce_parts = [&](int c) {
+        double sm = 0.0;
+#pragma unroll
+        for (int u = 0; u < PS_NQ; ++u) sm += part[u][c];
+        return sm;
+    };
+    const int qb = (qu * PS_CW) >> 6;
+    const unsigned ru = (unsigned)r;
+    auto load_sq = [&](const double* __restrict__ M, int k, int li, double (&dst)[PS_CW], bool active) {
+        const double* Mk = M + (int64_t)k * (SB * SB) + li * 64 + (int64_t)(qu * PS_CW) * SB;
+        if (active) {
+#pragma unroll
+            for (int j = 0; j < PS_CW; ++j) dst[j] = (Mk + (int64_t)j * SB)[ru];
+        }
+    };
+
+    auto dma_sq = [&](const double* __restrict__ M, int k, int li, int c0, int c1) {
+        const unsigned ln = (unsigned)(t & 63), lo = (ln & 31) * 2 + (ln >> 5) * SB;
+        const double* Mk = M + (int64_t)k * (SB * SB) + li * 64;
+        for (int c = c0 + 2 * qu; c < c1; c += 2 * PS_NQ)
+            __builtin_amdgcn_global_load_lds((const __attribute__((address_space(1))) void*)(Mk + (int64_t)c * SB + lo),
+                                             (__attribute__((address_space(3))) void*)(inv_s + c * 64), 16, 0, 0);
+    };
+    auto dot_lds = [&](bool active) {
+        double s0 = 0.0, s1 = 0.0, s2 = 0.0, s3 = 0.0;
+        if (active) {
+            const double* xq = xs + q * PS_CW;
+            const double* vq = inv_s + (q * PS_CW) * 64 + r;
+#pragma nounroll
+            for (int j = 0; j < PS_CW; j += 4) {
+                s0 = fma(vq[j * 64], xq[j], s0);
+                s1 = fma(vq[(j + 1) * 64], xq[j + 1], s1);
+                s2 = fma(vq[(j + 2) * 64], xq[j + 2], s2);
+                s3 = fma(vq[(j + 3) * 64], xq[j + 3], s3);
+            }
+        }
+        part[q][r] = (s0 + s1) + (s2 + s3);
+    };
+
+    int m0 = 0;
+    int mc = 0;
+    bool have_inv = false;
+    bool have_w = false;
+    bool a_next = false;
+    auto form_c = [&](int m, int i) -> bool {
+        const int li = i & 3;
+        if (!have_inv) dma_sq(Inv, i >> 2, li, 0, 64 * (li + 1));
+        if (t < 64) xs[li * 64 + t] = run[m][t];
+        asm volatile("s_waitcnt vmcnt(0)" ::: "memory");
+        if (!ps_gather(rfin + (int64_t)(i - li) * 64, li * 64, xs, abort_flag, spin_limit, false, 6, &s_bad)) return false;
+        PS_STAMP(i, 3);
+        dot_lds(qb <= li);
+        ps_barrier();
+        if (t < 64) run[m][t] = reduce_parts(t);
+        have_inv = false;
+        return true;
+    };
+    for (int m = 0; m < nown && ((g + m * G) >> 2) <= 1; ++m)
+        if (t < 64) ps_publish(rfin + (int64_t)(g + m * G) * 64 + t, run[m][t]);
+    for (; mc < nown && ((g + mc * G) >> 2) <= 1; ++mc) {
+        const int i = g + mc * G;
+        if (!form_c(mc, i)) return;
+        if ((i >> 2) == 0) {
+            if (t < 64) {
+                const double v = run[mc][t];
+                ps_publish(ypub + (int64_t)i * 64 + t, v);
+                ysol[mc][t] = v;
+            }
+            PS_STAMP(i, 4);
+            m0 = mc + 1;
+        }
+        ps_barrier();
+    }
+    for (int k = 0; k + 1 < nsteps && m0 < nown; ++k) {
+        const int b0 = 4 * k;
+        const int i = g + m0 * G;
+        const bool crit = (i >> 2) == k + 1;
+        if (!crit && !a_next) {
+            const double* Fs = F + (int64_t)i * 64 + ((int64_t)b0 * 64 + qu * PS_CW) * ld;
+#pragma unroll
+            for (int j = 0; j < PS_CW; ++j) a[j] = (Fs + (int64_t)j * ld)[ru];
+        }
+        if (!have_w && (i >> 2) <= k + 1 + PS_DAHEAD) {
+            load_sq(Wf, i >> 2, i & 3, d, true);
+            have_w = true;
+        }
+        if (!have_inv && mc < nown) {
+            const int ic = g + mc * G;
+            if ((ic >> 2) <= k + 2 + PS_DAHEAD) {
+                dma_sq(Inv, ic >> 2, ic & 3, 0, 64 * ((ic & 3) + 1));
+                have_inv = true;
+            }
+        }
+        if (crit) PS_STAMP(i, 0);
+        if (!ps_gather(ypub + (int64_t)b0 * 64, 256, xs, abort_flag, spin_limit, (i >> 2) > k + near_steps, nap, &s_bad)) return;
+        if (crit) {
+            PS_STAMP(i, 1);
+            dot_chunk(d, true);
+            ps_barrier();
+            if (t < 64) {
+                const double v = run[m0][t] - reduce_parts(t);
+                ps_publish(ypub + (int64_t)i * 64 + t, v);
+                ysol[m0][t] = v;
+            }
+            PS_STAMP(i, 4);
+            have_w = false;
+            ++m0;
+            if (m0 >= nown) break;
+            ps_barrier();
+        }
+        for (int m = m0; m < nown; ++m) {
+            const int im = g + m * G;
+            if (crit || m > m0) {
+                const double* Fs = F + (int64_t)im * 64 + ((int64_t)b0 * 64 + qu * PS_CW) * ld;
+#pragma unroll
+                for (int j = 0; j < PS_CW; ++j) a[j] = (Fs + (int64_t)j * ld)[ru];
+            }
+            dot_chunk(a, true);
+            a_next = nown - m0 == 1 && (im >> 2) >= k + 3;
+            if (a_next) {
+                const double* Fs = F + (int64_t)im * 64 + ((int64_t)(b0 + 4) * 64 + qu * PS_CW) * ld;
+#pragma unroll
+                for (int j = 0; j < PS_CW; ++j) a[j] = (Fs + (int64_t)j * ld)[ru];
+            }
+            ps_barrier();
+            const bool fin = (im >> 2) == k + 2;
+            if (t < 64) {
+                const double v = run[m][t] - reduce_parts(t);
+                run[m][t] = v;
+                if (fin) ps_publish(rfin + (int64_t)im * 64 + t, v);
+            }
+            if (fin) PS_STAMP(im, 2);
+            if (m + 1 < nown) ps_barrier();
+        }
+        if (mc < nown && ((g + mc * G) >> 2) == k + 2) {
+            const int ic = g + mc * G;
+            if (!form_c(mc, ic)) return;
+            ++mc;
+        }
+    }
+
+    __syncthreads();
+    for (int e = t; e < nown * 64; e += PS_NT) {
+        const int m = e >> 6, c = e & 63;
+        const double y = ysol[m][c];
+        run[m][c] = LDL ? y * dinv[(int64_t)(g + m * G) * 64 + c] : y;
+    }
+    __syncthreads();
+    const int lane = t & 63, sub = lane & 15, colq = lane >> 4, rc = qu & 3, cg = qu >> 2;
+    const int K = nsteps - 1;
+    auto nbk_of = [&](int k) { return nb - 4 * k < 4 ? nb - 4 * k : 4; };
+    int m1 = nown - 1;
+    int mb = nown - 1;
+    have_inv = false;
+    have_w = false;
+    a_next = false;
+    auto form_cb = [&](int m, int i) -> bool {
+        const int li = i & 3, nbk = nbk_of(i >> 2);
+        if (!have_inv) dma_sq(InvT, i >> 2, li, 64 * li, 256);
+        if (t < 64) xs[li * 64 + t] = run[m][t];
+        asm volatile("s_waitcnt vmcnt(0)" ::: "memory");
+        if (!ps_gather(zfin + (int64_t)(i + 1) * 64, (nbk - 1 - li) * 64, xs + (li + 1) * 64, abort_flag, spin_limit, false, 6, &s_bad)) return false;
+        dot_lds(qb >= li && qb < nbk);
+        ps_barrier();
+        if (t < 64) run[m][t] = reduce_parts(t);
+        have_inv = false;
+        return true;
+    };
+    const unsigned so = (unsigned)(4 * sub) + (unsigned)colq * (unsigned)ld;
+    auto load_slice = [&](int im, double (&dst)[PS_CW], int bs) {
+        const double* Fs = F + ((int64_t)bs * 64 + 64 * (qu & 3)) + ((int64_t)im * 64 + (qu >> 2) * 16) * ld;
+#pragma unroll
+        for (int p = 0; p < 4; ++p) {
+            const v2d lo = *reinterpret_cast<const v2d*>(Fs + (int64_t)(4 * p) * ld + so);
+            const v2d hi = *reinterpret_cast<const v2d*>(Fs + (int64_t)(4 * p) * ld + 2 + so);
+            dst[4 * p] = lo[0];
+            dst[4 * p + 1] = lo[1];
+            dst[4 * p + 2] = hi[0];
+            dst[4 * p + 3] = hi[1];
+        }
+    };
+    for (int m = nown - 1; m >= 0 && ((g + m * G) >> 2) >= K - 1; --m)
+        if (t < 64) ps_publish(zfin + (int64_t)(g + m * G) * 64 + t, run[m][t]);
+    for (; mb >= 0 && ((g + mb * G) >> 2) >= K - 1; --mb) {
+        const int i = g + mb * G;
+        if (!form_cb(mb, i)) return;
+        if ((i >> 2) == K) {
+            if (t < 64) {
+                const double v = run[mb][t];
+                ps_publish(xpub + (int64_t)i * 64 + t, v);
+                if ((int64_t)i * 64 + t < N) xout[(int64_t)i * 64 + t] = v;
+            }
+            m1 = mb - 1;
+        }
+        ps_barrier();
+    }
+    for (int k = K; k >= 1 && m1 >= 0; --k) {
+        const int b0 = 4 * k, nbk = nbk_of(k);
+        const int i = g + m1 * G;
+        const bool crit = (i >> 2) == k - 1;
+        if (!crit && !a_next && rc < nbk) load_slice(i, a, b0);
+        if (!have_w && (i >> 2) >= k - 1 - PS_DAHEAD) {
+            load_sq(Wb, i >> 2, i & 3, d, qb < nbk_of((i >> 2) + 1));
+            have_w = true;
+        }
+        if (!have_inv && mb >= 0) {
+            const int ic = g + mb * G;
+            if ((ic >> 2) >= k - 2 - PS_DAHEAD) {
+                dma_sq(InvT, ic >> 2, ic & 3, 64 * (ic & 3), 256);
+                have_inv = true;
+            }
+        }
+        if (!ps_gather(xpub + (int64_t)b0 * 64, nbk * 64, xs, abort_flag, spin_limit, (i >> 2) < k - near_steps, nap, &s_bad)) return;
+        if (crit) {
+            dot_chunk(d, qb < nbk);
+            ps_barrier();
+            if (t < 64) {
+                const double v = run[m1][t] - reduce_parts(t);
+                ps_publish(xpub + (int64_t)i * 64 + t, v);
+                if ((int64_t)i * 64 + t < N) xout[(int64_t)i * 64 + t] = v;
+            }
+            have_w = false;
+            --m1;
+            if (m1 < 0) break;
+            ps_barrier();
+        }
+        for (int m = m1; m >= 0; --m) {
+            const int im = g + m * G;
+            if ((crit || m < m1) && rc < nbk) load_slice(im, a, b0);
+            if (rc < nbk) {
+                const double x0 = xs[64 * rc + 4 * sub], x1 = xs[64 * rc + 4 * sub + 1],
+                             x2 = xs[64 * rc + 4 * sub + 2], x3 = xs[64 * rc + 4 * sub + 3];
+#pragma unroll
+                for (int p = 0; p < 4; ++p) {
+                    double sp = (a[4 * p] * x0 + a[4 * p + 1] * x1) + (a[4 * p + 2] * x2 + a[4 * p + 3] * x3);
+                    sp += __shfl_xor(sp, 1);
+                    sp += __shfl_xor(sp, 2);
+                    if ((sub & 3) == 0) part[rc * 4 + (sub >> 2)][cg * 16 + 4 * p + colq] = sp;
+                }
+            } else if (lane < 16) {
+#pragma unroll
+                for (int u = 0; u < 4; ++u) part[rc * 4 + u][cg * 16 + lane] = 0.0;
+            }
+            a_next = m1 == 0 && (im >> 2) <= k - 3;
+            if (a_next) load_slice(im, a, b0 - 4);
+            ps_barrier();
+            const bool fin = (im >> 2) == k - 2;
+            if (t < 64) {
+                const double v = run[m][t] - reduce_parts(t);
+                run[m][t] = v;
+                if (fin) ps_publish(zfin + (int64_t)im * 64 + t, v);
+            }
+            if (m > 0) ps_barrier();
+        }
+        if (mb >= 0 && ((g + mb * G) >> 2) == k - 2) {
+            const int ic = g + mb * G;
+            if (!form_cb(mb, ic)) return;
+            --mb;
+        }
+    }
+#undef PS_STAMP
+}
+
+template <bool LDL>
+__global__ __launch_bounds__(PS_NT) void persistent_solve1_kernel(
+    const double* __restrict__ F, int64_t ld, const double* __restrict__ Inv, const double* __restrict__ InvT,
+    const double* __restrict__ Wf, const double* __restrict__ Wb,
+    const double* __restrict__ dinv, const double* xin, double* xout, int64_t N, double* __restrict__ pub,
+    double* __restrict__ pub_other, int64_t Np, int* abort_flag, const int* __restrict__ info,
+    unsigned long long* __restrict__ trace, int near_steps, int nap, long spin_limit, int missing_wg) {
+    persistent_solve1_body<LDL>(F, ld, Inv, InvT, Wf, Wb, dinv, xin, xout, N, pub, pub_other, Np, abort_flag, info, trace, near_steps,
+                                nap, spin_limit, missing_wg, (int)gridDim.x, (int)blockIdx.x);
+}
+
 struct PsSys {
     const double* F;
     int64_t ld;
@@ -572,16 +902,22 @@
     double* pub_other;
     int* abort_flag;
     const int* info;
+    const double* Wf;
+    const double* Wb;
 };
 typedef const PsSys __attribute__((address_space(4))) * PsSysP;
 
-template <bool LDL>
+template <bool LDL, int HOPS>
 __global__ __launch_bounds__(PS_NT) void persistent_solve_multi_kernel(const PsSys* __restrict__ sys, int G, int64_t Np, int near_steps,
                                                                       int nap, long spin_limit) {
     const int isys = (int)blockIdx.x / G, g = (int)blockIdx.x % G;
     const PsSysP y = (PsSysP)(uintptr_t)(sys + isys);
-    persistent_solve_body<LDL>(y->F, y->ld, y->Inv, y->InvT, y->dinv, y->xin, y->xout, y->N, y->pub, y->pub_other, Np, y->abort_flag,
-                               y->info, nullptr, near_steps, nap, spin_limit, -1, G, g);
+    if (HOPS == 1)
+        persistent_solve1_body<LDL>(y->F, y->ld, y->Inv, y->InvT, y->Wf, y->Wb, y->dinv, y->xin, y->xout, y->N, y->pub, y->pub_other, Np,
+                                    y->abort_flag, y->info, nullptr, near_steps, nap, spin_limit, -1, G, g);
+    else
+        persistent_solve_body<LDL>(y->F, y->ld, y->Inv, y->InvT, y->dinv, y->xin, y->xout, y->N, y->pub, y->pub_other, Np, y->abort_flag,
+                                   y->info, nullptr, near_steps, nap, spin_limit, -1, G, g);
 }
 
 __global__ void ps_set_sys_kernel(PsSys rec, PsSys* __restrict__ dst) { *dst = rec; }
@@ -831,9 +1167,92 @@
     }
 }
 
+__global__ __launch_bounds__(256) void wblocks_kernel(const double* __restrict__ F, int64_t ld, const double* __restrict__ Inv,
+                                                      const double* __restrict__ InvT, double* __restrict__ Wf,
+                                                      double* __restrict__ Wb, int64_t Np, const int* __restrict__ info, int blk0,
+                                                      const mnk::SmallSysRec* __restrict__ recs = nullptr) {
+    int dir = blockIdx.z;
+    if (recs != nullptr) {
+        const mnk::SmallSysRec r = recs[blockIdx.z >> 1];
+        F = r.F; ld = r.ld; Inv = r.linv256; InvT = r.linv256t; Wf = r.wf; Wb = r.wb; Np = r.Np; info = r.info;
+        dir = blockIdx.z & 1;
+        if (Wf == nullptr) return;
+    }
+    if (*info != 0) return;
+    const int64_t k = (int64_t)blockIdx.x + blk0;
+    const int64_t nsc = (Np + SB - 1) / SB;
+    if (k >= nsc || (dir == 0 ? k < 1 : k + 1 >= nsc)) return;
+    const int tm = blockIdx.y & 1, tn = blockIdx.y >> 1;
+    const int tid = threadIdx.x, lane = tid & 63, w = __builtin_amdgcn_readfirstlane(tid >> 6);
+    const int l15 = lane & 15, l4 = lane >> 4;
+    const int m0 = 128 * tm + 32 * w, n0 = 64 * tn;
+    const int rows_k = (int)(Np - k * SB < SB ? Np - k * SB : SB);
+    const int rows_n = (int)(Np - (k + 1) * SB < SB ? Np - (k + 1) * SB : SB);
+    const double* A = (dir == 0 ? Inv : InvT) + k * (int64_t)(SB * SB) + (m0 + l15) + (int64_t)l4 * SB;
+    const double* B = dir == 0 ? F + (k * SB + l4) + ((k - 1) * SB + n0 + l15) * ld
+                               : F + ((k + 1) * SB + n0 + l15) + (k * SB + l4) * ld;
+    const int64_t bsc = dir == 0 ? 1 : ld;
+    const int64_t bsn = dir == 0 ? ld : 1;
+    const int c_lo = dir == 0 ? 0 : 128 * tm;
+    const int c_hi = dir == 0 ? (128 * (tm + 1) < rows_k ? 128 * (tm + 1) : rows_k) : SB;
+    v4f64 acc[2][4];
+#pragma unroll
+    for (int mi = 0; mi < 2; ++mi)
+#pragma unroll
+        for (int ni = 0; ni < 4; ++ni) acc[mi][ni] = v4f64{0.0, 0.0, 0.0, 0.0};
+    bool bok[4];
+#pragma unroll
+    for (int ni = 0; ni < 4; ++ni) bok[ni] = dir == 0 || n0 + 16 * ni + l15 < rows_n;
+    for (int cc = c_lo; cc < c_hi; cc += 16)
+#pragma unroll
+    for (int c = cc; c < cc + 16; c += 4) {
+        double af[2], bf[4];
+#pragma unroll
+        for (int mi = 0; mi < 2; ++mi) af[mi] = A[16 * mi + (int64_t)c * SB];
+#pragma unroll
+        for (int ni = 0; ni < 4; ++ni) bf[ni] = bok[ni] ? B[(int64_t)(16 * ni) * bsn + (int64_t)c * bsc] : 0.0;
+#pragma unroll
+        for (int mi = 0; mi < 2; ++mi)
+#pragma unroll
+            for (int ni = 0; ni < 4; ++ni) acc[mi][ni] = __builtin_amdgcn_mfma_f64_16x16x4f64(bf[ni], af[mi], acc[mi][ni], 0, 0, 0);
+    }
+    double* out = (dir == 0 ? Wf : Wb) + k * (int64_t)(SB * SB);
+#pragma unroll
+    for (int mi = 0; mi < 2; ++mi)
+#pragma unroll
+        for (int ni = 0; ni < 4; ++ni)
+#pragma unroll
+            for (int r = 0; r < 4; ++r) out[(m0 + 16 * mi + l15) + (int64_t)(n0 + 16 * ni + l4 + 4 * r) * SB] = acc[mi][ni][r];
+}
+
 }
 
 using namespace mnk;
+
+bool mnk_ls_w_wanted(mnk_ls* ls) {
+    if (ls->solve_hops != 1 || !ls->persistent_solve || ls->bk_active || (ls->algo != MNK_LDL && ls->algo != MNK_CHOLESKY)) return false;
+    if (ls->Np <= SB) return false;
+    if (!ls->wfwd.p) {
+        const size_t cnt = (size_t)((ls->Np + SB - 1) / SB) * (SB * SB);
+        if (ls->wfwd.alloc(cnt) || ls->wbwd.alloc(cnt)) {
+            (void)hipGetLastError();
+            ls->wfwd.release(); ls->wbwd.release();
+            ls->solve_hops = 2;
+            return false;
+        }
+    }
+    return true;
+}
+
+int mnk_ls_build_wblocks(mnk_ls* ls, hipStream_t s, int64_t sc0, int64_t sc1) {
+    const int64_t nsc = (ls->Np + SB - 1) / SB;
+    sc1 = std::min(sc1, nsc);
+    if (sc1 <= sc0) return 0;
+    hipLaunchKernelGGL(wblocks_kernel, dim3((unsigned)(sc1 - sc0), 8, 2), dim3(256), 0, s, ls->fact.p, ls->ld, ls->linv256.p,
+                       ls->linv256t.p, ls->wfwd.p, ls->wbwd.p, ls->Np, ls->info_dev.p, (int)sc0);
+    MNK_HIP(hipGetLastError());
+    return 0;
+}
 
 int mnk_ls_build_inverses(mnk_ls* ls, hipStream_t s, int64_t sc0, int64_t sc1) {
     const int64_t nblk = std::min<int64_t>(sc1, (ls->Np + SB - 1) / SB) - sc0;
@@ -875,6 +1294,12 @@
         }
     }
     MNK_HIP(hipGetLastError());
+    if (sc0 == 0) ls->w_done = 0;
+    if (ls->w_done == sc0 && mnk_ls_w_wanted(ls)) {
+        int rc = mnk_ls_build_wblocks(ls, s, sc0, sc1);
+        if (rc) return rc;
+        ls->w_done = std::min<int64_t>(sc1, (ls->Np + SB - 1) / SB);
+    }
     return 0;
 }
 
@@ -882,6 +1307,10 @@
     const unsigned nblk = (unsigned)((Np + SB - 1) / SB);
     hipLaunchKernelGGL(linv256_mfma_kernel, dim3(nblk, 4, (unsigned)n), dim3(256), 0, s, (const double*)nullptr, (int64_t)0,
                        (const double*)nullptr, (double*)nullptr, (double*)nullptr, (int64_t)0, (const int*)nullptr, 0, recs_dev);
+    if (nblk >= 2)
+        hipLaunchKernelGGL(wblocks_kernel, dim3(nblk, 8, 2 * (unsigned)n), dim3(256), 0, s, (const double*)nullptr, (int64_t)0,
+                           (const double*)nullptr, (const double*)nullptr, (double*)nullptr, (double*)nullptr, (int64_t)0,
+                           (const int*)nullptr, 0, recs_dev);
     MNK_HIP(hipGetLastError());
     return 0;
 }
@@ -896,6 +1325,19 @@
     hipLaunchKernelGGL(linv256_mfma_kernel, dim3(1, 4), dim3(256), 0, s, (const double*)nullptr, (int64_t)0, (const double*)nullptr,
                        (double*)nullptr, (double*)nullptr, (int64_t)256, one.p, 0);
     MNK_HIP(hipGetLastError());
+    return 0;
+}
+
+static int ps1_allow_lds() {
+    static std::atomic<uint64_t> attr_devs{0};
+    int dev = 0;
+    MNK_HIP(hipGetDevice(&dev));
+    if (attr_devs.load(std::memory_order_relaxed) >> (dev & 63) & 1) return 0;
+    MNK_HIP(hipFuncSetAttribute((const void*)persistent_solve1_kernel<true>, hipFuncAttributeMaxDynamicSharedMemorySize, PS_INV_LDS_BYTES));
+    MNK_HIP(hipFuncSetAttribute((const void*)persistent_solve1_kernel<false>, hipFuncAttributeMaxDynamicSharedMemorySize, PS_INV_LDS_BYTES));
+    MNK_HIP(hipFuncSetAttribute((const void*)persistent_solve_multi_kernel<true, 1>, hipFuncAttributeMaxDynamicSharedMemorySize, PS_INV_LDS_BYTES));
+    MNK_HIP(hipFuncSetAttribute((const void*)persistent_solve_multi_kernel<false, 1>, hipFuncAttributeMaxDynamicSharedMemorySize, PS_INV_LDS_BYTES));
+    attr_devs.fetch_or(1ull << (dev & 63), std::memory_order_relaxed);
     return 0;
 }
 
@@ -962,7 +1404,27 @@
         const double* xin = xuser != nullptr ? xuser : xdev;
         double* xout = xuser != nullptr ? xuser : xdev;
         const int64_t nio = xuser != nullptr ? N : Np;
-        if (ldl)
+        bool one_hop = ls->solve_hops == 1 && (Np <= SB || mnk_ls_w_wanted(ls));
+        if (one_hop && Np > SB && ls->w_done < (Np + SB - 1) / SB) {
+            rc = mnk_ls_build_wblocks(ls, s, ls->w_done, (Np + SB - 1) / SB);
+            if (rc) return mnk_persist_end(ls->ctx, s, rc);
+            ls->w_done = (Np + SB - 1) / SB;
+        }
+        if (one_hop) {
+            rc = ps1_allow_lds();
+            if (rc) return mnk_persist_end(ls->ctx, s, rc);
+        }
+        if (one_hop && ldl)
+            hipLaunchKernelGGL(persistent_solve1_kernel<true>, dim3(G), dim3(PS_NT), PS_INV_LDS_BYTES, s, ls->fact.p, ld, ls->linv256.p,
+                               ls->linv256t.p, ls->wfwd.p, ls->wbwd.p, ls->dinv.p, xin, xout, nio, pubs[cur], pubs[oth], Np,
+                               ls->solve_abort, ls->info_dev.p, ls->solve_trace.p, ps_near, ps_nap, ls->ps_spin_limit,
+                               ls->debug_ps_missing);
+        else if (one_hop)
+            hipLaunchKernelGGL(persistent_solve1_kernel<false>, dim3(G), dim3(PS_NT), PS_INV_LDS_BYTES, s, ls->fact.p, ld, ls->linv256.p,
+                               ls->linv256t.p, ls->wfwd.p, ls->wbwd.p, ls->dinv.p, xin, xout, nio, pubs[cur], pubs[oth], Np,
+                               ls->solve_abort, ls->info_dev.p, ls->solve_trace.p, ps_near, ps_nap, ls->ps_spin_limit,
+                               ls->debug_ps_missing);
+        else if (ldl)
             hipLaunchKernelGGL(persistent_solve_kernel<true>, dim3(G), dim3(PS_NT), 0, s, ls->fact.p, ld, ls->linv256.p,
                                ls->linv256t.p, ls->dinv.p, xin, xout, nio, pubs[cur], pubs[oth], Np, ls->solve_abort, ls->info_dev.p,
                                ls->solve_trace.p, ps_near, ps_nap, ls->ps_spin_limit, ls->debug_ps_missing);
@@ -1027,7 +1489,8 @@
     const int G = (int)std::min<int64_t>(nb64, ls->ctx->num_cu);
     return !ls->bk_active && ls->persistent_solve && !(ls->solve512 && ls->linv512.p) && !ls->ctx->partitioned &&
            (nb64 + G - 1) / G <= PS_MAXOWN && (G >= 4 || nb64 <= G) && !(ls->solve_abort && *ls->solve_abort != 0) &&
-           ls->debug_ps_missing < 0 && !ls->solve_trace.p;
+           ls->debug_ps_missing < 0 && !ls->solve_trace.p &&
+           (ls->solve_hops != 1 || ls->Np <= SB || (ls->wfwd.p && ls->w_done >= (ls->Np + SB - 1) / SB));
 }
 
 bool mnk_solve_defer(mnk_ls* ls, double* xuser) {
@@ -1063,17 +1526,23 @@
                 hipLaunchKernelGGL(ps_reset_kernel, dim3((unsigned)((4 * Np + 255) / 256)), dim3(256), 0, h,
                                    reinterpret_cast<unsigned long long*>(pubs[cur]), 4 * Np);
             PsSys rec{ls->fact.p, ls->ld, ls->linv256.p, ls->linv256t.p, ls->dinv.p, v[i].x, v[i].x, ls->N, pubs[cur], pubs[oth],
-                      ls->solve_abort, ls->info_dev.p};
+                      ls->solve_abort, ls->info_dev.p, ls->wfwd.p, ls->wbwd.p};
             hipLaunchKernelGGL(ps_set_sys_kernel, dim3(1), dim3(1), 0, h, rec, dsys + i);
             ls->pub_clean[cur] = false;
             ls->pub_clean[oth] = true;
             ls->pub_next = oth;
         }
         const bool ldl = l0->algo == MNK_LDL;
-        if (ldl)
-            hipLaunchKernelGGL(persistent_solve_multi_kernel<true>, dim3((unsigned)(q * G)), dim3(PS_NT), 0, h, dsys, G, Np, PS_NEAR, 6, l0->ps_spin_limit);
+        const bool one_hop = l0->solve_hops == 1;
+        if (one_hop) { int rl = ps1_allow_lds(); if (rl) return rl; }
+        if (ldl && one_hop)
+            hipLaunchKernelGGL((persistent_solve_multi_kernel<true, 1>), dim3((unsigned)(q * G)), dim3(PS_NT), PS_INV_LDS_BYTES, h, dsys, G, Np, PS_NEAR, 6, l0->ps_spin_limit);
+        else if (one_hop)
+            hipLaunchKernelGGL((persistent_solve_multi_kernel<false, 1>), dim3((unsigned)(q * G)), dim3(PS_NT), PS_INV_LDS_BYTES, h, dsys, G, Np, PS_NEAR, 6, l0->ps_spin_limit);
+        else if (ldl)
+            hipLaunchKernelGGL((persistent_solve_multi_kernel<true, 2>), dim3((unsigned)(q * G)), dim3(PS_NT), 0, h, dsys, G, Np, PS_NEAR, 6, l0->ps_spin_limit);
         else
-            hipLaunchKernelGGL(persistent_solve_multi_kernel<false>, dim3((unsigned)(q * G)), dim3(PS_NT), 0, h, dsys, G, Np, PS_NEAR, 6, l0->ps_spin_limit);
+            hipLaunchKernelGGL((persistent_solve_multi_kernel<false, 2>), dim3((unsigned)(q * G)), dim3(PS_NT), 0, h, dsys, G, Np, PS_NEAR, 6, l0->ps_spin_limit);
         MNK_HIP(hipGetLastError());
         return 0;
     };
@@ -1102,7 +1571,8 @@
         const int maxq = envq > 0 ? envq : std::max(1, std::min(PS_BATCH_MAXQ, l0->ctx->num_cu / g4));
         std::vector<SolveReq> g, rest;
         for (const SolveReq& r : pend) {
-            bool take = (int)g.size() < maxq && r.ls->ctx->device == l0->ctx->device && r.ls->Np == l0->Np && r.ls->algo == l0->algo;
+            bool take = (int)g.size() < maxq && r.ls->ctx->device == l0->ctx->device && r.ls->Np == l0->Np && r.ls->algo == l0->algo &&
+                        r.ls->solve_hops == l0->solve_hops;
             for (const SolveReq& t : g) take = take && t.ls != r.ls;
             for (const SolveReq& t : rest) take = take && t.ls != r.ls;
             if (take) {
diff --git a/madnlp.jl_amd/linear_solver.py b/madnlp.jl_amd/linear_solver.py
--- a/madnlp.jl_amd/linear_solver.py
+++ b/madnlp.jl_amd/linear_solver.py
@@ -131,6 +131,7 @@
     share: int = 1
     small_tiles: int = 400
     persistent_solve: bool = True
+    solve_hops: int = 1
     single_rows: int = 2560
     panel_algo: int = 5
 
@@ -156,7 +157,8 @@
         settings = [("pivot_tol", self.opt.pivot_tol), ("outer_block", self.opt.outer_block),
                     ("lookahead", float(self.opt.lookahead)), ("share", float(self.opt.share)),
                     ("small_tiles", float(self.opt.small_tiles)), ("persistent_solve", float(self.opt.persistent_solve)),
-                    ("single_rows", float(self.opt.single_rows)), ("panel_algo", float(self.opt.panel_algo))]
+                    ("single_rows", float(self.opt.single_rows)), ("panel_algo", float(self.opt.panel_algo)),
+                    ("solve_hops", float(self.opt.solve_hops))]
         for key, val in settings:
             L.check(L.lib().mnk_ls_set_option(self._h, key.encode(), float(val)), "mnk_ls_set_option")
         self.info = 0
```

Measured after the change: 107.2 it/s. -1.1%, worse.
